# ShifuML/shifu-tensorflow

Measured on NVIDIA H100. Metric: rows/sec tabular-DNN train, higher is better.
Workload: dtype bf16

## Files before the change

include/shifu_b200.h:

```cpp
#ifndef SHIFU_B200_H
#define SHIFU_B200_H

#include <stdint.h>

#ifdef __cplusplus
extern "C" {
#endif

#define SB_MAX_HIDDEN 32

typedef enum {
  SB_OK = 0,
  SB_ERR_INVALID = -1,
  SB_ERR_CUDA = -2,
  SB_ERR_NCCL = -3,
  SB_ERR_IO = -4,
  SB_ERR_STATE = -5,
  SB_ERR_FORMAT = -6
} sb_status;

typedef enum { SB_ACT_SIGMOID = 0, SB_ACT_TANH = 1, SB_ACT_RELU = 2, SB_ACT_LEAKYRELU = 3, SB_ACT_NONE = -1 } sb_act;
typedef enum { SB_LOSS_MSE = 0, SB_LOSS_SIGMOID_CE = 1 } sb_loss;
typedef enum { SB_OPT_ADADELTA = 0, SB_OPT_ADAM = 1, SB_OPT_SGD = 2, SB_OPT_MOMENTUM = 3 } sb_optimizer;
typedef enum { SB_PREC_FP32 = 0, SB_PREC_BF16 = 1, SB_PREC_FP32_TC = 2, SB_PREC_BF16X2 = 3 } sb_precision;

typedef struct {
  int32_t n_features;
  int32_t n_hidden;
  int32_t hidden[SB_MAX_HIDDEN];
  int32_t acts[SB_MAX_HIDDEN];
  int32_t loss;
  int32_t optimizer;
  float learning_rate;
  float rho;
  float epsilon;
  float beta1, beta2;
  float momentum;
  int32_t max_batch;
  int32_t precision;
} sb_net_desc;

typedef struct sb_trainer sb_trainer_t;
typedef struct sb_model sb_model_t;

const char* sb_version(void);
const char* sb_last_error(void);
int sb_device_count(void);
int sb_host_alloc(void** ptr, uint64_t bytes);
int sb_host_free(void* ptr);

#define SB_NCCL_ID_BYTES 128
int sb_nccl_unique_id(void* out128);

int sb_trainer_create(const sb_net_desc* desc, int device, const void* nccl_id, int rank, int world,
                      sb_trainer_t** out);
int sb_trainer_destroy(sb_trainer_t* t);
#define SB_IPC_HANDLE_BYTES 64
int sb_trainer_ipc_handle(sb_trainer_t* t, void* out64);
int sb_trainer_set_peer_handles(sb_trainer_t* t, const void* handles , int32_t n_handles);
int sb_trainer_clear_peer_handles(sb_trainer_t* t);
void* sb_trainer_exchange_base(sb_trainer_t* t);
int sb_trainer_set_peer_pointers(sb_trainer_t* t, void* const* bases, int32_t n);
int64_t sb_trainer_param_count(const sb_trainer_t* t);
int sb_trainer_set_params(sb_trainer_t* t, const float* flat, int64_t n);
int sb_trainer_get_params(sb_trainer_t* t, float* flat, int64_t n);
int sb_trainer_init_xavier(sb_trainer_t* t, uint64_t seed);
int sb_trainer_get_grads(sb_trainer_t* t, float* flat, int64_t n);

int sb_trainer_step(sb_trainer_t* t, const float* X, const float* y, const float* w, int32_t rows,
                    float* loss_out);

int sb_trainer_set_sparse(sb_trainer_t* t, int32_t n_dense, int32_t n_onehot, int32_t n_cat);
int sb_trainer_step_sparse(sb_trainer_t* t, const float* Xd, const int32_t* idx, const float* y, const float* w,
                           int32_t rows, float* loss_out);
int sb_trainer_predict_sparse(sb_trainer_t* t, const float* Xd, const int32_t* idx, int64_t rows, float* out);
int sb_trainer_eval_loss_sparse(sb_trainer_t* t, const float* Xd, const int32_t* idx, const float* y, const float* w,
                                int64_t rows, float* loss_out);

int sb_trainer_step_async(sb_trainer_t* t, const float* X, const float* y, const float* w, int32_t rows);

int sb_trainer_accumulate(sb_trainer_t* t, const float* X, const float* y, const float* w, int32_t rows,
                          float* loss_out);
int sb_trainer_apply_accumulated(sb_trainer_t* t);
int sb_trainer_apply_accumulated_mean(sb_trainer_t* t, int64_t total_pushes);

int sb_trainer_load_dataset(sb_trainer_t* t, const float* X, const float* y, const float* w, int64_t n_rows);
int sb_trainer_step_resident(sb_trainer_t* t, int64_t row_offset, int32_t rows, float* loss_out);
int sb_trainer_step_resident_async(sb_trainer_t* t, int64_t row_offset, int32_t rows);
int sb_trainer_run_resident(sb_trainer_t* t, const int64_t* row_offsets, int32_t n_steps, int32_t rows);
int sb_trainer_accumulate_resident(sb_trainer_t* t, int64_t row_offset, int32_t rows, float* loss_out);
int sb_trainer_loss_resident(sb_trainer_t* t, int64_t row_offset, int32_t rows, float* loss_out);
int sb_trainer_last_loss(sb_trainer_t* t, float* loss_out);
int sb_trainer_loss_history(sb_trainer_t* t, int64_t first_step, int32_t n, float* out);
int sb_trainer_sync(sb_trainer_t* t);
int sb_trainer_broadcast_state(sb_trainer_t* t, int32_t root);
void* sb_trainer_stream(sb_trainer_t* t);
int sb_trainer_kernels_per_step(sb_trainer_t* t, int32_t rows);

int sb_trainer_eval_loss(sb_trainer_t* t, const float* X, const float* y, const float* w, int64_t rows,
                         float* loss_out);
int sb_trainer_predict(sb_trainer_t* t, const float* X, int64_t rows, float* out);

int sb_trainer_save_checkpoint(sb_trainer_t* t, const char* path);
int sb_trainer_load_checkpoint(sb_trainer_t* t, const char* path);
int64_t sb_trainer_global_step(const sb_trainer_t* t);

int sb_trainer_export_savedmodel(sb_trainer_t* t, const char* export_dir);

int sb_model_load(const char* saved_model_dir, const char* input_name, const char* output_name,
                  const char* tag, int device, int precision, sb_model_t** out);
int sb_model_create(const sb_net_desc* desc, const float* flat_params, int64_t n, int device, sb_model_t** out);
int sb_model_destroy(sb_model_t* m);
int32_t sb_model_n_features(const sb_model_t* m);
int32_t sb_model_n_layers(const sb_model_t* m);
int sb_model_score(sb_model_t* m, const float* X, int64_t rows, float* out);
int sb_model_score_row_f64(sb_model_t* m, const double* row, int32_t n, double* out);
int sb_model_score_device(sb_model_t* m, const float* dX, int64_t rows, float* dOut);
int sb_model_sync(sb_model_t* m);
void* sb_model_stream(sb_model_t* m);

#define SB_COL_SKIP (-1)
#define SB_COL_TARGET (-2)
#define SB_COL_WEIGHT (-3)
typedef struct { int64_t row; int32_t slot; int32_t len; int64_t offset; } sb_cell_flag;
int sb_text_parse(const char* text, int64_t n_bytes, char delim, const int32_t* col_map, int32_t n_map, int32_t n_feat,
                  float* X, float* y, float* w, int64_t max_rows, int64_t* n_rows_out, sb_cell_flag* flags,
                  int64_t flag_cap, int64_t* n_flags_out, int device);
int sb_text_parse_device(const char* text, int64_t n_bytes, char delim, const int32_t* col_map, int32_t n_map, int32_t n_feat,
                         float** dX, float** dy, float** dw, int64_t* n_rows_out, sb_cell_flag* flags, int64_t flag_cap,
                         int64_t* n_flags_out, int device, float* kernel_ms_out);
int sb_device_alloc_f32(float** out, int64_t n, int device);
int sb_device_free(void* p);
int sb_device_patch_f32(float* d_base, int64_t index, float value);
int sb_device_read_f32(const float* d_src, int64_t n, float* host_out);
int sb_device_gather_rows(const float* d_src, int32_t n_cols, const int64_t* rows_host, int64_t n, float* d_dst, int device);

int sb_debug_text_parse_host(const char* text, int64_t n_bytes, char delim, const int32_t* col_map, int32_t n_map,
                             int32_t n_feat, float* X, float* y, float* w, int64_t max_rows, int64_t* n_rows_out,
                             sb_cell_flag* flags, int64_t flag_cap, int64_t* n_flags_out);

int sb_savedmodel_write(const char* export_dir, const sb_net_desc* desc, const float* flat_params, int64_t n);
int sb_savedmodel_read(const char* saved_model_dir, const char* input_name, const char* output_name,
                       const char* tag, sb_net_desc* desc_out, int32_t* out_act, float* flat, int64_t flat_cap,
                       int64_t* n_params);

int sb_debug_gemm_bf16_cfg(const float* A, const float* B, float* D, int32_t M, int32_t N, int32_t K,
                           int32_t split_k, int32_t a_mn, int32_t b_mn, int32_t cfg_cg, int32_t cfg_bn, int device);

int sb_debug_gemm_layer(int32_t kind, int32_t precision, const float* A, const float* W, const float* bias, const float* aux,
                        const float* addend, float* out, float* colsum, float* grad, int32_t* guard, char* route,
                        int32_t route_cap, int32_t M, int32_t N, int32_t K, int32_t a_rows, int32_t row0, int32_t act,
                        int32_t r0, int32_t r1, int32_t sms, int64_t clear_n4, int device);

int sb_debug_step_trace(sb_trainer_t* t, uint64_t* stamps, int32_t cap_kernels, char* names, int32_t names_cap, int32_t* n_kernels);
int sb_debug_gemm_bench(const float* A, const float* B, float* D, int32_t M, int32_t N, int32_t K, int32_t split_k,
                        int32_t a_mn, int32_t b_mn, int32_t cfg_cg, int32_t cfg_bn, int device, int32_t iters,
                        float* ms_out);

int sb_debug_gemm_epilogue(const float* A, const float* W, const float* bias, const float* aux, float* out, float* colsum,
                           int32_t M, int32_t N, int32_t K, int32_t da, int32_t act, int32_t bm_wg, int device,
                           int32_t iters, float* ms_out);

int sb_debug_gemm_fwd_out(const float* A, const float* W, const float* bias, const float* wo, float bo, const float* y,
                          const float* w, float* dZ, float* g_bL, float* g_wo, float* g_bo, float* loss_sum, int32_t* guard,
                          int32_t M, int32_t N, int32_t K, int32_t a_rows, int32_t row0, int32_t act, int32_t loss,
                          int32_t np, int32_t grid, int device);

#ifdef __cplusplus
}
#endif
#endif
```

shifu-tensorflow_b200/_capi.py:

```python
from __future__ import annotations

import ctypes as C
import os
from typing import Optional, Sequence

import numpy as np

os.environ.setdefault("CUDA_DEVICE_MAX_CONNECTIONS", "32")

_HERE = os.path.dirname(os.path.abspath(__file__))
LIB_PATH = os.path.join(_HERE, "lib", "libshifu_b200.so")

SB_MAX_HIDDEN = 32
SB_NCCL_ID_BYTES = 128
ACT_SIGMOID, ACT_TANH, ACT_RELU, ACT_LEAKYRELU, ACT_NONE = 0, 1, 2, 3, -1
LOSS_MSE, LOSS_SIGMOID_CE = 0, 1
OPT_ADADELTA, OPT_ADAM, OPT_SGD, OPT_MOMENTUM = 0, 1, 2, 3
PREC_FP32, PREC_BF16, PREC_FP32_TC, PREC_BF16X2 = 0, 1, 2, 3
SB_OK, SB_ERR_INVALID, SB_ERR_CUDA, SB_ERR_NCCL, SB_ERR_IO, SB_ERR_STATE, SB_ERR_FORMAT = 0, -1, -2, -3, -4, -5, -6


class NetDesc(C.Structure):
    _fields_ = [
        ("n_features", C.c_int32), ("n_hidden", C.c_int32),
        ("hidden", C.c_int32 * SB_MAX_HIDDEN), ("acts", C.c_int32 * SB_MAX_HIDDEN),
        ("loss", C.c_int32), ("optimizer", C.c_int32),
        ("learning_rate", C.c_float), ("rho", C.c_float), ("epsilon", C.c_float),
        ("beta1", C.c_float), ("beta2", C.c_float), ("momentum", C.c_float),
        ("max_batch", C.c_int32), ("precision", C.c_int32),
    ]


def make_desc(n_features: int, hidden: Sequence[int], acts: Sequence[int], loss: int = LOSS_MSE,
              optimizer: int = OPT_ADADELTA, learning_rate: float = 0.001, rho: float = 0.95, epsilon: float = 1e-8,
              beta1: float = 0.9, beta2: float = 0.999, momentum: float = 0.9, max_batch: int = 128,
              precision: int = PREC_FP32) -> NetDesc:
    if len(hidden) != len(acts):
        raise ValueError("hidden and acts must have the same length")
    if len(hidden) > SB_MAX_HIDDEN:
        raise ValueError("at most %d hidden layers" % SB_MAX_HIDDEN)
    d = NetDesc()
    d.n_features, d.n_hidden = int(n_features), len(hidden)
    for i, (h, a) in enumerate(zip(hidden, acts)):
        d.hidden[i], d.acts[i] = int(h), int(a)
    d.loss, d.optimizer = int(loss), int(optimizer)
    d.learning_rate, d.rho, d.epsilon = learning_rate, rho, epsilon
    d.beta1, d.beta2, d.momentum = beta1, beta2, momentum
    d.max_batch, d.precision = int(max_batch), int(precision)
    return d


class CellFlag(C.Structure):
    _fields_ = [("row", C.c_int64), ("slot", C.c_int32), ("len", C.c_int32), ("offset", C.c_int64)]


COL_SKIP, COL_TARGET, COL_WEIGHT = -1, -2, -3


class ShifuB200Error(RuntimeError):
    def __init__(self, code: int, msg: str):
        super().__init__("[%d] %s" % (code, msg))
        self.code = code


_lib = None

_P = C.POINTER
_f32p, _f64p, _vp, _cp = _P(C.c_float), _P(C.c_double), C.c_void_p, C.c_char_p
PROTOTYPES = {
    "sb_version": (C.c_char_p, []),
    "sb_last_error": (C.c_char_p, []),
    "sb_device_count": (C.c_int, []),
    "sb_host_alloc": (C.c_int, [_P(_vp), C.c_uint64]),
    "sb_host_free": (C.c_int, [_vp]),
    "sb_nccl_unique_id": (C.c_int, [_vp]),
    "sb_trainer_create": (C.c_int, [_P(NetDesc), C.c_int, _vp, C.c_int, C.c_int, _P(_vp)]),
    "sb_trainer_destroy": (C.c_int, [_vp]),
    "sb_trainer_ipc_handle": (C.c_int, [_vp, _vp]),
    "sb_trainer_set_peer_handles": (C.c_int, [_vp, _vp, C.c_int32]),
    "sb_trainer_clear_peer_handles": (C.c_int, [_vp]),
    "sb_trainer_exchange_base": (C.c_void_p, [_vp]),
    "sb_trainer_set_peer_pointers": (C.c_int, [_vp, _P(_vp), C.c_int32]),
    "sb_trainer_param_count": (C.c_int64, [_vp]),
    "sb_trainer_set_params": (C.c_int, [_vp, _f32p, C.c_int64]),
    "sb_trainer_get_params": (C.c_int, [_vp, _f32p, C.c_int64]),
    "sb_trainer_init_xavier": (C.c_int, [_vp, C.c_uint64]),
    "sb_trainer_get_grads": (C.c_int, [_vp, _f32p, C.c_int64]),
    "sb_trainer_step": (C.c_int, [_vp, _f32p, _f32p, _f32p, C.c_int32, _f32p]),
    "sb_trainer_set_sparse": (C.c_int, [_vp, C.c_int32, C.c_int32, C.c_int32]),
    "sb_trainer_step_sparse": (C.c_int, [_vp, _f32p, _P(C.c_int32), _f32p, _f32p, C.c_int32, _f32p]),
    "sb_trainer_predict_sparse": (C.c_int, [_vp, _f32p, _P(C.c_int32), C.c_int64, _f32p]),
    "sb_trainer_eval_loss_sparse": (C.c_int, [_vp, _f32p, _P(C.c_int32), _f32p, _f32p, C.c_int64, _f32p]),
    "sb_trainer_step_async": (C.c_int, [_vp, _f32p, _f32p, _f32p, C.c_int32]),
    "sb_trainer_accumulate": (C.c_int, [_vp, _f32p, _f32p, _f32p, C.c_int32, _f32p]),
    "sb_trainer_apply_accumulated": (C.c_int, [_vp]),
    "sb_trainer_apply_accumulated_mean": (C.c_int, [_vp, C.c_int64]),
    "sb_trainer_loss_resident": (C.c_int, [_vp, C.c_int64, C.c_int32, _f32p]),
    "sb_trainer_broadcast_state": (C.c_int, [_vp, C.c_int32]),
    "sb_trainer_load_dataset": (C.c_int, [_vp, _f32p, _f32p, _f32p, C.c_int64]),
    "sb_trainer_step_resident": (C.c_int, [_vp, C.c_int64, C.c_int32, _f32p]),
    "sb_trainer_step_resident_async": (C.c_int, [_vp, C.c_int64, C.c_int32]),
    "sb_trainer_run_resident": (C.c_int, [_vp, C.POINTER(C.c_int64), C.c_int32, C.c_int32]),
    "sb_trainer_accumulate_resident": (C.c_int, [_vp, C.c_int64, C.c_int32, _f32p]),
    "sb_trainer_last_loss": (C.c_int, [_vp, _f32p]),
    "sb_trainer_loss_history": (C.c_int, [_vp, C.c_int64, C.c_int32, _f32p]),
    "sb_trainer_sync": (C.c_int, [_vp]),
    "sb_trainer_stream": (C.c_void_p, [_vp]),
    "sb_trainer_kernels_per_step": (C.c_int, [_vp, C.c_int32]),
    "sb_trainer_eval_loss": (C.c_int, [_vp, _f32p, _f32p, _f32p, C.c_int64, _f32p]),
    "sb_trainer_predict": (C.c_int, [_vp, _f32p, C.c_int64, _f32p]),
    "sb_trainer_save_checkpoint": (C.c_int, [_vp, _cp]),
    "sb_trainer_load_checkpoint": (C.c_int, [_vp, _cp]),
    "sb_trainer_global_step": (C.c_int64, [_vp]),
    "sb_trainer_export_savedmodel": (C.c_int, [_vp, _cp]),
    "sb_model_load": (C.c_int, [_cp, _cp, _cp, _cp, C.c_int, C.c_int, _P(_vp)]),
    "sb_model_create": (C.c_int, [_P(NetDesc), _f32p, C.c_int64, C.c_int, _P(_vp)]),
    "sb_model_destroy": (C.c_int, [_vp]),
    "sb_model_n_features": (C.c_int32, [_vp]),
    "sb_model_n_layers": (C.c_int32, [_vp]),
    "sb_model_score": (C.c_int, [_vp, _f32p, C.c_int64, _f32p]),
    "sb_model_score_row_f64": (C.c_int, [_vp, _f64p, C.c_int32, _f64p]),
    "sb_model_score_device": (C.c_int, [_vp, _vp, C.c_int64, _vp]),
    "sb_model_sync": (C.c_int, [_vp]),
    "sb_model_stream": (C.c_void_p, [_vp]),
    "sb_text_parse": (C.c_int, [_cp, C.c_int64, C.c_char, _P(C.c_int32), C.c_int32, C.c_int32, _f32p, _f32p, _f32p, C.c_int64,
                                _P(C.c_int64), _P(CellFlag), C.c_int64, _P(C.c_int64), C.c_int]),
    "sb_text_parse_device": (C.c_int, [_cp, C.c_int64, C.c_char, _P(C.c_int32), C.c_int32, C.c_int32, _P(_f32p), _P(_f32p), _P(_f32p),
                                       _P(C.c_int64), _P(CellFlag), C.c_int64, _P(C.c_int64), C.c_int, _f32p]),
    "sb_device_alloc_f32": (C.c_int, [_P(_f32p), C.c_int64, C.c_int]),
    "sb_device_free": (C.c_int, [_vp]),
    "sb_device_patch_f32": (C.c_int, [_f32p, C.c_int64, C.c_float]),
    "sb_device_read_f32": (C.c_int, [_f32p, C.c_int64, _f32p]),
    "sb_device_gather_rows": (C.c_int, [_f32p, C.c_int32, _P(C.c_int64), C.c_int64, _f32p, C.c_int]),
    "sb_debug_text_parse_host": (C.c_int, [_cp, C.c_int64, C.c_char, _P(C.c_int32), C.c_int32, C.c_int32, _f32p, _f32p, _f32p,
                                           C.c_int64, _P(C.c_int64), _P(CellFlag), C.c_int64, _P(C.c_int64)]),
    "sb_savedmodel_write": (C.c_int, [_cp, _P(NetDesc), _f32p, C.c_int64]),
    "sb_savedmodel_read": (C.c_int, [_cp, _cp, _cp, _cp, _P(NetDesc), _P(C.c_int32), _f32p, C.c_int64, _P(C.c_int64)]),
    "sb_debug_gemm_layer": (C.c_int, [C.c_int32, C.c_int32, _f32p, _f32p, _f32p, _f32p, _f32p, _f32p, _f32p, _f32p, _P(C.c_int32),
                                      C.c_char_p, C.c_int32, C.c_int32, C.c_int32, C.c_int32, C.c_int32, C.c_int32, C.c_int32,
                                      C.c_int32, C.c_int32, C.c_int32, C.c_int64, C.c_int]),
    "sb_debug_step_trace": (C.c_int, [_vp, C.POINTER(C.c_uint64), C.c_int32, C.c_char_p, C.c_int32, C.POINTER(C.c_int32)]),
    "sb_debug_gemm_bench": (C.c_int, [_f32p, _f32p, _f32p, C.c_int32, C.c_int32, C.c_int32, C.c_int32, C.c_int32, C.c_int32,
                                      C.c_int32, C.c_int32, C.c_int, C.c_int32, _f32p]),
    "sb_debug_gemm_bf16_cfg": (C.c_int, [_f32p, _f32p, _f32p, C.c_int32, C.c_int32, C.c_int32, C.c_int32, C.c_int32, C.c_int32,
                                         C.c_int32, C.c_int32, C.c_int]),
    "sb_debug_gemm_epilogue": (C.c_int, [_f32p, _f32p, _f32p, _f32p, _f32p, _f32p, C.c_int32, C.c_int32, C.c_int32, C.c_int32,
                                         C.c_int32, C.c_int32, C.c_int, C.c_int32, _f32p]),
    "sb_debug_gemm_fwd_out": (C.c_int, [_f32p, _f32p, _f32p, _f32p, C.c_float, _f32p, _f32p, _f32p, _f32p, _f32p, _f32p, _f32p,
                                        _P(C.c_int32), C.c_int32, C.c_int32, C.c_int32, C.c_int32, C.c_int32, C.c_int32,
                                        C.c_int32, C.c_int32, C.c_int32, C.c_int]),
}


def lib():
    global _lib
    if _lib is not None:
        return _lib
    if not os.path.exists(LIB_PATH):
        raise ImportError(
            "libshifu_b200.so is missing (%s). Build it with `python -c 'import __graft_entry__ as g; g.build()'` "
            "or `python shifu-tensorflow_b200/build.py`. There is no CPU fallback." % LIB_PATH)
    L = C.CDLL(LIB_PATH, mode=C.RTLD_GLOBAL)
    for name, (res, args) in PROTOTYPES.items():
        fn = getattr(L, name)
        fn.restype, fn.argtypes = res, args
    _lib = L
    return L


def check(status: int) -> None:
    if status != SB_OK:
        raise ShifuB200Error(status, lib().sb_last_error().decode("utf-8", "replace"))


def _f32(a, shape=None) -> np.ndarray:
    a = np.ascontiguousarray(a, dtype=np.float32)
    if shape is not None and a.shape != shape:
        a = a.reshape(shape)
    return a


def _ptr(a):
    if a is None:
        return None
    if hasattr(a, "ptr") and not isinstance(a, np.ndarray):
        return a.ptr
    return a.ctypes.data_as(_f32p)


class DeviceArray:

    def __init__(self, ptr, shape, device: int = 0, owner: bool = True):
        self.ptr, self.shape, self.device, self._own = ptr, tuple(shape), device, owner

    @classmethod
    def empty(cls, shape, device: int = 0) -> "DeviceArray":
        p = _f32p()
        n = int(np.prod(shape))
        check(lib().sb_device_alloc_f32(C.byref(p), max(n, 1), device))
        return cls(p, shape, device)

    def __len__(self):
        return self.shape[0]

    @property
    def size(self) -> int:
        return int(np.prod(self.shape))

    def numpy(self) -> np.ndarray:
        out = np.empty(self.shape, np.float32)
        if self.size:
            check(lib().sb_device_read_f32(self.ptr, self.size, _ptr(out)))
        return out

    def patch(self, flat_index: int, value: float):
        check(lib().sb_device_patch_f32(self.ptr, int(flat_index), float(value)))

    def take_rows(self, rows) -> "DeviceArray":
        rows = np.ascontiguousarray(rows, dtype=np.int64)
        n_cols = int(np.prod(self.shape[1:])) if len(self.shape) > 1 else 1
        out = DeviceArray.empty((len(rows),) + self.shape[1:], self.device)
        check(lib().sb_device_gather_rows(self.ptr, n_cols, rows.ctypes.data_as(_P(C.c_int64)), len(rows), out.ptr, self.device))
        return out

    def free(self):
        if self._own and self.ptr:
            lib().sb_device_free(C.cast(self.ptr, _vp))
        self.ptr = None

    __del__ = free


class Trainer:

    def __init__(self, desc: NetDesc, device: int = 0, nccl_id: Optional[bytes] = None, rank: int = 0, world: int = 1):
        self._h = C.c_void_p()
        self.desc = desc
        idbuf = None
        if nccl_id is not None:
            if len(nccl_id) != SB_NCCL_ID_BYTES:
                raise ValueError("nccl_id must be %d bytes" % SB_NCCL_ID_BYTES)
            idbuf = C.create_string_buffer(bytes(nccl_id), SB_NCCL_ID_BYTES)
        check(lib().sb_trainer_create(C.byref(desc), device, C.cast(idbuf, _vp) if idbuf is not None else None,
                                      rank, world, C.byref(self._h)))
        self.n_params = int(lib().sb_trainer_param_count(self._h))
        self.n_features = int(desc.n_features)

    def close(self):
        if getattr(self, "_h", None) is not None and self._h:
            lib().sb_trainer_destroy(self._h)
            self._h = None

    __del__ = close

    def __enter__(self):
        return self

    def __exit__(self, *exc):
        self.close()

    def ipc_handle(self) -> bytes:
        buf = C.create_string_buffer(64)
        check(lib().sb_trainer_ipc_handle(self._h, C.cast(buf, _vp)))
        return buf.raw

    def set_peer_handles(self, handles: Sequence[bytes]):
        blob = b"".join(handles)
        buf = C.create_string_buffer(blob, len(blob))
        check(lib().sb_trainer_set_peer_handles(self._h, C.cast(buf, _vp), len(handles)))

    def clear_peer_handles(self):
        check(lib().sb_trainer_clear_peer_handles(self._h))

    @property
    def exchange_base(self) -> int:
        return int(lib().sb_trainer_exchange_base(self._h) or 0)

    def set_peer_pointers(self, bases: Sequence[int]):
        arr = (C.c_void_p * len(bases))(*[C.c_void_p(int(b)) for b in bases])
        check(lib().sb_trainer_set_peer_pointers(self._h, arr, len(bases)))

    def set_params(self, flat):
        flat = _f32(flat).reshape(-1)
        check(lib().sb_trainer_set_params(self._h, _ptr(flat), flat.size))

    def get_params(self) -> np.ndarray:
        out = np.empty(self.n_params, np.float32)
        check(lib().sb_trainer_get_params(self._h, _ptr(out), out.size))
        return out

    def get_grads(self) -> np.ndarray:
        out = np.empty(self.n_params, np.float32)
        check(lib().sb_trainer_get_grads(self._h, _ptr(out), out.size))
        return out

    def init_xavier(self, seed: int):
        check(lib().sb_trainer_init_xavier(self._h, seed))

    def _xyw(self, X, y, w):
        if isinstance(X, DeviceArray):
# ... 110 lines not shown
        return out

    def sync(self):
        check(lib().sb_trainer_sync(self._h))

    @property
    def stream(self) -> int:
        return int(lib().sb_trainer_stream(self._h) or 0)

    def kernels_per_step(self, rows: int) -> int:
        n = lib().sb_trainer_kernels_per_step(self._h, rows)
        if n < 0:
            check(n)
        return n

    def eval_loss(self, X, y, w=None) -> float:
        X, y, w, rows = self._xyw(X, y, w)
        loss = C.c_float()
        check(lib().sb_trainer_eval_loss(self._h, _ptr(X), _ptr(y), _ptr(w), rows, C.byref(loss)))
        return float(loss.value)

    def predict(self, X) -> np.ndarray:
        X = _f32(X)
        out = np.empty(X.shape[0], np.float32)
        check(lib().sb_trainer_predict(self._h, _ptr(X), X.shape[0], _ptr(out)))
        return out

    def debug_step_trace(self):
        buf = np.zeros((32, 16), np.uint64)
        names = C.create_string_buffer(4096)
        k = C.c_int32()
        check(lib().sb_debug_step_trace(self._h, buf.ctypes.data_as(C.POINTER(C.c_uint64)), 32, names, 4096, C.byref(k)))
        return names.value.decode().split(","), buf[:k.value].copy()

    @property
    def global_step(self) -> int:
        return int(lib().sb_trainer_global_step(self._h))

    def save_checkpoint(self, path: str):
        check(lib().sb_trainer_save_checkpoint(self._h, path.encode()))

    def load_checkpoint(self, path: str):
        check(lib().sb_trainer_load_checkpoint(self._h, path.encode()))

    def export_savedmodel(self, export_dir: str):
        check(lib().sb_trainer_export_savedmodel(self._h, export_dir.encode()))


class Model:

    def __init__(self, handle):
        self._h = handle
        self.n_features = int(lib().sb_model_n_features(self._h))

    @classmethod
    def load(cls, saved_model_dir: str, input_name: str, output_name: str, tag: str = "serve", device: int = 0,
             precision: int = PREC_FP32) -> "Model":
        h = C.c_void_p()
        enc = lambda s: None if s is None else s.encode()
        check(lib().sb_model_load(enc(saved_model_dir), enc(input_name), enc(output_name), enc(tag), device, precision,
                                  C.byref(h)))
        return cls(h)

    @classmethod
    def create(cls, desc: NetDesc, flat_params, device: int = 0) -> "Model":
        h = C.c_void_p()
        flat = _f32(flat_params).reshape(-1)
        check(lib().sb_model_create(C.byref(desc), _ptr(flat), flat.size, device, C.byref(h)))
        return cls(h)

    def close(self):
        if getattr(self, "_h", None) is not None and self._h:
            lib().sb_model_destroy(self._h)
            self._h = None

    __del__ = close

    def __enter__(self):
        return self

    def __exit__(self, *exc):
        self.close()

    def score(self, X) -> np.ndarray:
        X = _f32(X)
        if X.ndim != 2 or X.shape[1] != self.n_features:
            raise ValueError("X must be [rows, %d]" % self.n_features)
        out = np.empty(X.shape[0], np.float32)
        check(lib().sb_model_score(self._h, _ptr(X), X.shape[0], _ptr(out)))
        return out

    def score_row_f64(self, row) -> float:
        row = np.ascontiguousarray(row, dtype=np.float64).reshape(-1)
        out = C.c_double()
        check(lib().sb_model_score_row_f64(self._h, row.ctypes.data_as(_f64p), row.size, C.byref(out)))
        return float(out.value)

    def score_device(self, dX_ptr: int, rows: int, dOut_ptr: int):
        check(lib().sb_model_score_device(self._h, C.c_void_p(dX_ptr), rows, C.c_void_p(dOut_ptr)))

    def sync(self):
        check(lib().sb_model_sync(self._h))

    @property
    def stream(self) -> int:
        return int(lib().sb_model_stream(self._h) or 0)


def nccl_unique_id() -> bytes:
    buf = C.create_string_buffer(SB_NCCL_ID_BYTES)
    check(lib().sb_nccl_unique_id(C.cast(buf, _vp)))
    return buf.raw


def device_count() -> int:
    return int(lib().sb_device_count())


def savedmodel_write(export_dir: str, desc: NetDesc, flat_params) -> None:
    flat = _f32(flat_params).reshape(-1)
    check(lib().sb_savedmodel_write(export_dir.encode(), C.byref(desc), _ptr(flat), flat.size))


def savedmodel_read(saved_model_dir: str, input_name: str, output_name: str, tag: str = "serve"):
    d = NetDesc()
    out_act = C.c_int32(0)
    n = C.c_int64(0)
    args = (saved_model_dir.encode(), input_name.encode(), output_name.encode(), tag.encode())
    check(lib().sb_savedmodel_read(*args, C.byref(d), C.byref(out_act), None, 0, C.byref(n)))
    flat = np.empty(n.value, np.float32)
    check(lib().sb_savedmodel_read(*args, C.byref(d), C.byref(out_act), _ptr(flat), flat.size, C.byref(n)))
    return int(d.n_features), [int(d.hidden[i]) for i in range(d.n_hidden)], [int(d.acts[i]) for i in range(d.n_hidden)], \
        int(out_act.value), flat


def debug_gemm_bf16(A: np.ndarray, B: np.ndarray, split_k: int = 1, device: int = 0, a_mn: bool = False,
                    b_mn: bool = False, cg: int = 0, bn: int = 0) -> np.ndarray:
    A, B = _f32(A), _f32(B)
    (K, M) = A.shape if a_mn else A.shape[::-1]
    (K2, N) = B.shape if b_mn else B.shape[::-1]
    assert K == K2
    D = np.zeros((M, N), np.float32)
    check(lib().sb_debug_gemm_bf16_cfg(_ptr(A), _ptr(B), _ptr(D), M, N, K, split_k, int(a_mn), int(b_mn), cg, bn, device))
    return D


GEMM_FWD, GEMM_DA, GEMM_DW = 0, 1, 2
PARTS = {PREC_FP32: 1, PREC_BF16: 1, PREC_FP32_TC: 3, PREC_BF16X2: 2}


def debug_gemm_layer(kind: int, precision: int, A: np.ndarray, W: np.ndarray, act: int = ACT_NONE,
                     bias: Optional[np.ndarray] = None, aux: Optional[np.ndarray] = None, addend: Optional[np.ndarray] = None,
                     colsum: Optional[np.ndarray] = None, grad: Optional[np.ndarray] = None, M: Optional[int] = None,
                     row0: int = 0, r0: int = 0, r1: Optional[int] = None, sms: int = 0, clear_n4: int = 0, device: int = 0):
    A, W = _f32(A), _f32(W)
    nparts = PARTS[precision]
    out = cs = g = None
    if kind == GEMM_DW:
        a_rows, Mx = A.shape
        K, N = W.shape
        if row0 + K > a_rows:
            raise ValueError("the batch of K = %d rows at row0 = %d runs past A" % (K, row0))
        g = np.zeros((Mx, N), np.float32) if grad is None else _f32(grad).copy()
        a_rows_arg, M = a_rows, Mx
    elif kind == GEMM_DA:
        M, K = A.shape
        N = W.shape[0]
        assert W.shape == (N, K) and np.shape(aux) == (M, N)
        cs = np.zeros(N, np.float32) if colsum is None else _f32(colsum).copy()
        a_rows_arg = M
    else:
        a_rows_arg, K = A.shape
        N = W.shape[1]
        M = a_rows_arg - row0 if M is None else M
    if kind != GEMM_DW:
        out = np.zeros((nparts, M, N), np.float32)
    bias = None if bias is None else _f32(bias)
    aux = None if aux is None else _f32(aux)
    addend = None if addend is None else _f32(addend)
    guard = C.c_int32(-1)
    route = C.create_string_buffer(64)
    check(lib().sb_debug_gemm_layer(kind, precision, _ptr(A), _ptr(W), _ptr(bias), _ptr(aux), _ptr(addend), _ptr(out), _ptr(cs),
                                    _ptr(g), C.byref(guard), route, 64, M, N, K, a_rows_arg, row0, act, r0,
                                    M if r1 is None else r1, sms, clear_n4, device))
    return out, cs, g, int(guard.value), route.value.decode()


def debug_gemm_split(A: np.ndarray, B: np.ndarray, np_parts: int, device: int = 0) -> np.ndarray:
    prec = {1: PREC_BF16, 2: PREC_BF16X2, 3: PREC_FP32_TC}.get(np_parts)
    if prec is None:
        raise ShifuB200Error(SB_ERR_INVALID, "np_parts=%r outside 1..3" % (np_parts,))
    A, B = _f32(A), _f32(B)
    assert A.shape[1] == B.shape[1]
    out, _, _, guard, _ = debug_gemm_layer(GEMM_FWD, prec, A, B.T.copy(), ACT_NONE, bias=np.zeros(B.shape[0], np.float32),
                                           device=device)
    if guard != 0:
        raise ShifuB200Error(SB_ERR_STATE, "%d sentinel elements around the output changed" % guard)
    return out.astype(np.float64).sum(axis=0)


def debug_gemm_bench(M: int, N: int, K: int, split_k: int = 1, a_mn: bool = False, b_mn: bool = False, cg: int = 0,
                     bn: int = 0, iters: int = 50, device: int = 0) -> float:
    rng = np.random.default_rng(0)
    A = rng.standard_normal((K, M) if a_mn else (M, K), dtype=np.float32)
    B = rng.standard_normal((K, N) if b_mn else (N, K), dtype=np.float32)
    D = np.zeros((M, N), np.float32)
    ms = C.c_float()
    check(lib().sb_debug_gemm_bench(_ptr(A), _ptr(B), _ptr(D), M, N, K, split_k, int(a_mn), int(b_mn), cg, bn, device,
                                    iters, C.byref(ms)))
    return float(ms.value)


def debug_gemm_epilogue(A: np.ndarray, W: np.ndarray, act: int, bias: Optional[np.ndarray] = None,
                        aux: Optional[np.ndarray] = None, bm_wg: int = 0, iters: int = 0, device: int = 0):
    A, W = _f32(A), _f32(W)
    M, K = A.shape
    da = aux is not None
    N = W.shape[0] if da else W.shape[1]
    assert W.shape == ((N, K) if da else (K, N))
    bias = _f32(bias) if bias is not None else None
    aux = _f32(aux) if da else None
    out = np.zeros((M, N), np.float32)
    cs = np.zeros(N, np.float32) if da else None
    ms = C.c_float()
    check(lib().sb_debug_gemm_epilogue(_ptr(A), _ptr(W), _ptr(bias) if bias is not None else None,
                                       _ptr(aux) if da else None, _ptr(out), _ptr(cs) if da else None, M, N, K, int(da),
                                       act, bm_wg, device, iters, C.byref(ms)))
    return out, cs, (float(ms.value) if iters > 0 else None)


def debug_gemm_fwd_out(A: np.ndarray, W: np.ndarray, bias: np.ndarray, wo: np.ndarray, bo: float, y: np.ndarray,
                       w: np.ndarray, act: int, loss: int, np_parts: int = 1, row0: int = 0, M: Optional[int] = None,
                       grid: int = 0, g_bL: Optional[np.ndarray] = None, g_wo: Optional[np.ndarray] = None, g_bo: float = 0.0,
                       loss_sum: float = 0.0, device: int = 0):
    A, W, bias, wo = _f32(A), _f32(W), _f32(bias), _f32(wo)
    a_rows, K = A.shape
    K2, N = W.shape
    assert K == K2
    M = a_rows - row0 if M is None else M
    y, w = _f32(y).reshape(-1), _f32(w).reshape(-1)
    assert y.size == M and w.size == M
    g_bL = _f32(g_bL).copy() if g_bL is not None else np.zeros(N, np.float32)
    g_wo = _f32(g_wo).copy() if g_wo is not None else np.zeros(N, np.float32)
    gbo, ls, guard = C.c_float(g_bo), C.c_float(loss_sum), C.c_int32(-1)
    dZ = np.zeros((max(np_parts, 1), max(M, 0), N), np.float32)
    check(lib().sb_debug_gemm_fwd_out(_ptr(A), _ptr(W), _ptr(bias), _ptr(wo), float(bo), _ptr(y), _ptr(w), _ptr(dZ),
                                      _ptr(g_bL), _ptr(g_wo), C.byref(gbo), C.byref(ls), C.byref(guard), M, N, K, a_rows, row0,
                                      act, loss, np_parts, grid, device))
    return dZ, g_bL, g_wo, float(gbo.value), float(ls.value), int(guard.value)


def text_parse_device(text: bytes, col_map: Sequence[int], n_feat: int, delim: str = "|", device: int = 0, flag_cap: int = 65536):
    if not text.endswith(b"\n"):
        text = text + b"\n"
    cm = (C.c_int32 * len(col_map))(*[int(c) for c in col_map])
    dX, dy, dw = _f32p(), _f32p(), _f32p()
    flags = (CellFlag * flag_cap)()
    n_rows, n_flags, kms = C.c_int64(0), C.c_int64(0), C.c_float(0)
    check(lib().sb_text_parse_device(text, len(text), delim.encode()[:1], cm, len(col_map), n_feat, C.byref(dX), C.byref(dy), C.byref(dw),
                                     C.byref(n_rows), flags, flag_cap, C.byref(n_flags), device, C.byref(kms)))
    if n_flags.value > flag_cap:
        raise ShifuB200Error(SB_ERR_FORMAT, "%d cells need the slow path, more than flag_cap=%d" % (n_flags.value, flag_cap))
    fl = [(int(flags[i].row), int(flags[i].slot), int(flags[i].offset), int(flags[i].len)) for i in range(n_flags.value)]
    n = n_rows.value
    return DeviceArray(dX, (n, n_feat), device), DeviceArray(dy, (n,), device), DeviceArray(dw, (n,), device), fl, text, float(kms.value)


def text_parse(text: bytes, col_map: Sequence[int], n_feat: int, delim: str = "|", device: int = 0, host_debug: bool = False,
               flag_cap: int = 65536):
    if not text.endswith(b"\n"):
        text = text + b"\n"
    max_rows = text.count(b"\n")
    cm = (C.c_int32 * len(col_map))(*[int(c) for c in col_map])
    X = np.zeros((max_rows, n_feat), np.float32)
    y = np.zeros(max_rows, np.float32)
    w = np.ones(max_rows, np.float32)
    flags = (CellFlag * flag_cap)()
    n_rows, n_flags = C.c_int64(0), C.c_int64(0)
    args = [text, len(text), delim.encode()[:1], cm, len(col_map), n_feat, _ptr(X), _ptr(y), _ptr(w), max_rows, C.byref(n_rows),
            flags, flag_cap, C.byref(n_flags)]
    if host_debug:
        check(lib().sb_debug_text_parse_host(*args))
    else:
        check(lib().sb_text_parse(*args, device))
    if n_flags.value > flag_cap:
        raise ShifuB200Error(SB_ERR_FORMAT, "%d cells need the slow path, more than flag_cap=%d" % (n_flags.value, flag_cap))
    fl = [(int(flags[i].row), int(flags[i].slot), int(flags[i].offset), int(flags[i].len)) for i in range(n_flags.value)]
    n = n_rows.value
    return X[:n], y[:n], w[:n], fl, text
```

shifu-tensorflow_b200/csrc/capi.cu:

```cuda
#include <math.h>
#include <stdlib.h>
#include <string.h>
#include <algorithm>
#include <memory>
#include <random>
#include "net.cuh"
#include "savedmodel.h"
#include "xchg_p2p.cuh"

using namespace sb;

enum { G_STEP = 0, G_ACC = 1, G_KINDS = 2 };

struct sb_trainer {
  Net net;
  sb_net_desc desc;
  OptHyper hyper;
  float lr = 0.f;
  int rank = 0, world = 1;
  NcclComm comm = nullptr;
  float *grad = nullptr, *s1 = nullptr, *s2 = nullptr, *acc = nullptr;
  int n_acc = 0;
  float grad_out_scale = 1.f;
  long long global_step = 0;
// ... 114 lines not shown
}

static int enqueue_allreduce(sb_trainer* t, float* buf) {
  if (t->world <= 1) return SB_OK;
  NcclApi* api = nccl_api();
  SB_CHECK(api && t->comm, SB_ERR_NCCL, "no gradient exchange configured: world = %d but neither an NCCL communicator (nccl_id) nor a "
           "peer table (sb_trainer_set_peer_handles / _pointers) exists", t->world);
  int r = api->AllReduce(buf, buf, static_cast<size_t>(t->net.n_params), NCCL_FLOAT32, NCCL_SUM, t->comm, t->net.stream);
  SB_CHECK(r == 0, SB_ERR_NCCL, "ncclAllReduce failed: %s", api->GetErrorString(r));
  return SB_OK;
}

static int enqueue_optimizer(sb_trainer* t, const StepIn& in, const float* g, int w0 = 0, int w1 = -1, cudaStream_t st = nullptr,
                             bool publish_scalars = false, bool pdl = false) {
  Net& n = t->net;
  if (w1 < 0) w1 = n.n_work;
  if (!st) st = n.stream;
  if (w1 <= w0) return SB_OK;
  SB_TRY(launch_kernel(optimizer_kernel, dim3(static_cast<unsigned>(w1 - w0)), dim3(256), 0, st, pdl, n.work + w0, in.desc, t->hyper,
                       n.theta, g, n.s1, n.s2, in.scal, publish_scalars ? t->d_hscal : static_cast<float*>(nullptr),
                       n.next_trace(st == n.stream ? "opt" : "opt_side")));
  n.mark("optimizer");
  return SB_OK;
}

enum { XSEG_A = 1 };
static int xseg_all(const sb_trainer* t) { return (1 << t->x_slots) - 1; }

static XchgParams xchg_params(sb_trainer* t, const BatchDesc* desc) {
  Net& n = t->net;
  XchgParams p;
  memset(&p, 0, sizeof(p));
  p.peers = t->d_peers;
  p.rank = t->rank; p.world = t->world;
  p.s1_off = static_cast<long long>(n.s1_off); p.s2_off = static_cast<long long>(n.s2_off);
  p.grad_off = t->grad_off; p.flags_off = t->flags_off;
  p.work = n.work;
  p.n_slots = t->x_slots;
  for (int sl = 0; sl < t->x_slots; ++sl) { p.slot_begin[sl] = t->x_begin[sl]; p.slot_end[sl] = t->x_end[sl]; }
  p.desc = desc;
  p.hyper = t->hyper;
  p.host_err = t->d_herr;
  p.timeout_ns = t->xchg_timeout_ns;
  static const bool fence_sys = getenv("SB_XCHG_FENCE_SYS") != nullptr;
  p.fence_gpu = fence_sys ? 0 : 1;
  return p;
}

static int enqueue_xchg(sb_trainer* t, const StepIn& in, int slot_mask, cudaStream_t st, bool publish_scalars, bool pdl,
                        bool alone = false) {
  Net& n = t->net;
  XchgParams p = xchg_params(t, in.desc);
  p.slot_mask = slot_mask;
  p.scal = publish_scalars ? in.scal : nullptr;
  p.host_scal = publish_scalars ? t->d_hscal : nullptr;
  char nm[24];
  if (slot_mask == XSEG_A) snprintf(nm, sizeof(nm), "xchg_A");
  else if ((slot_mask & (slot_mask - 1)) == 0) snprintf(nm, sizeof(nm), "xchg_B%d", __builtin_ctz(slot_mask) - 1);
  else snprintf(nm, sizeof(nm), "xchg");
  p.trace = n.next_trace(nm);
  int runs = 0, all_runs = 0;
  for (int sl = 0; sl < t->x_slots; ++sl)
    if ((slot_mask >> sl) & 1) {
      runs += (p.slot_end[sl] - p.slot_begin[sl] + t->world - 1) / t->world;
      all_runs += p.slot_end[sl] - p.slot_begin[sl];
    }
  const int U = t->world <= 2 ? 2 : 1;
  const int want = std::max((runs + U - 1) / U, (all_runs - runs + 3) / 4);
  int grid = t->xchg_blocks > 0 ? t->xchg_blocks : (alone ? 2 : 1) * n.num_sms;
  if (t->peers_share_device && grid > 32) grid = 32;
  if (grid > want) grid = want;
  if (grid < 1) grid = 1;
  const dim3 g(static_cast<unsigned>(grid)), b(256);
  if (t->ll_ready) {
    LLParams lp;
    lp.x = p; lp.llg_off = t->llg_off; lp.lls_off = t->lls_off; lp.n4 = t->xch_n4;
    if (t->world <= 2) SB_TRY(launch_kernel(xchg_ll_kernel<2>, g, b, 0, st, pdl, lp));
    else if (t->world <= 4) SB_TRY(launch_kernel(xchg_ll_kernel<4>, g, b, 0, st, pdl, lp));
    else if (t->world <= 8) SB_TRY(launch_kernel(xchg_ll_kernel<8>, g, b, 0, st, pdl, lp));
    else SB_TRY(launch_kernel(xchg_ll_kernel<16>, g, b, 0, st, pdl, lp));
  } else
  if (t->world <= 2) SB_TRY(launch_kernel(xchg_update_kernel<2>, g, b, 0, st, pdl, p));
  else if (t->world <= 4) SB_TRY(launch_kernel(xchg_update_kernel<4>, g, b, 0, st, pdl, p));
  else if (t->world <= 8) SB_TRY(launch_kernel(xchg_update_kernel<8>, g, b, 0, st, pdl, p));
  else SB_TRY(launch_kernel(xchg_update_kernel<16>, g, b, 0, st, pdl, p));
  n.mark("xchg_update");
  t->master_stale = true;
  t->grad_sharded = true;
  return SB_OK;
}

static int gather_master(sb_trainer* t) {
  if (!t->p2p_ready || !t->master_stale || t->world <= 1) return SB_OK;
  Net& n = t->net;
  SB_CUDA(cudaStreamSynchronize(n.stream));
  XchgParams p = xchg_params(t, n.desc);
  gather_master_kernel<<<n.n_work, 256, 0, n.stream>>>(p, 0);
  SB_CUDA(cudaGetLastError());
  SB_CUDA(cudaStreamSynchronize(n.stream));
  t->master_stale = false;
  return SB_OK;
}

static int join_streams(cudaStream_t to, cudaStream_t from, cudaEvent_t e) {
  SB_CUDA(cudaEventRecord(e, from));
  SB_CUDA(cudaStreamWaitEvent(to, e, 0));
  return SB_OK;
}

enum Dw1At { DW1_BESIDE, DW1_FRONT, DW1_BEHIND };
struct Dw1Plan {
  Dw1At at;
  int sms[2];
};

static Dw1Plan plan_dw1(const sb_trainer* t, int rows, bool split_tail, bool xsched) {
  const Net& n = t->net;
  const int S = n.num_sms;
  Dw1Plan d = {DW1_BESIDE, {S, S}};
  if (xsched) {
    d.at = t->peers_share_device ? DW1_BEHIND : DW1_FRONT;
    return d;
  }
  const Layer& l0 = n.layers[0];
  const Layer& l1 = n.layers[1];
  const int kx = round_up(rows, 64) * pairs_of(n.nparts);
  const GemmPlan n0 = plan_gemm(l0.in, l0.out, kx, S, true);
  const GemmPlan n1 = plan_gemm(l1.in, l1.out, kx, S, true);
  if (n0.grid + n1.grid <= S) return d;
  if (split_tail && (n0.grid == S || n0.bn == 256)) {
    d.at = DW1_FRONT;
    return d;
  }
  const GemmPlan b1 = plan_gemm(l1.in, l1.out, kx, S / 3, true);
  const GemmPlan b0 = plan_gemm(l0.in, l0.out, kx, S - b1.grid, true);
  auto waves = [&](const GemmPlan& pl, const Layer& ly, int sms) {
    const int tiles = ((ly.in + 127) / 128) * ((ly.out + pl.bn - 1) / pl.bn) * pl.split_k;
    return ((tiles + sms - 1) / sms) * pl.kb_per_split;
  };
  const int t_nat = waves(n0, l0, S) + waves(n1, l1, S);
  const int t0 = waves(b0, l0, S - b1.grid);
  const int t1 = waves(b1, l1, S / 3);
  if ((t0 > t1 ? t0 : t1) < t_nat) { d.sms[1] = S / 3; d.sms[0] = S - b1.grid; }
  return d;
}

static int enqueue_step_backward(sb_trainer* t, const StepIn& in, int rows, int kind) {
  Net& n = t->net;
  float* g = t->grad;
  const int L = n.L, S = n.num_sms;
  if (!n.tc()) {
    for (int l = L - 1; l >= 0; --l) {
      SB_TRY(n.enqueue_dw(in, l, rows, g, n.stream, false, S));
      if (l > 0) SB_TRY(n.enqueue_da(l, rows, g));
    }
  } else {
    const bool split_tail = kind == G_STEP && (t->world == 1 || t->p2p_ready) && L > 1;
    const bool xsched = split_tail && t->world > 1;
    const Dw1Plan d1 = L > 1 ? plan_dw1(t, rows, split_tail, xsched) : Dw1Plan{DW1_BESIDE, {S, S}};
    for (int l = L - 1; l >= 1; --l) {
      if (l > 1 || d1.at == DW1_BESIDE) {
        SB_TRY(join_streams(t->side, n.stream, t->ev_dz[l]));
        SB_TRY(n.enqueue_dw(in, l, rows, g, t->side, false, l == 1 ? d1.sms[1] : S));
      }
      SB_TRY(n.enqueue_da(l, rows, g));
    }
    if (split_tail) SB_CUDA(cudaEventRecord(t->ev_da_done, n.stream));
    if (L == 1) {
      SB_TRY(join_streams(t->side, n.stream, t->ev_dz[0]));
      SB_TRY(n.enqueue_dw(in, 0, rows, g, t->side, false, S));
    } else {
      if (d1.at == DW1_FRONT) {
        SB_TRY(n.enqueue_dw(in, 1, rows, g, n.stream, true, d1.sms[1]));
        SB_TRY(join_streams(t->side, n.stream, t->ev_c[0]));
        if (xsched) {
          SB_TRY(enqueue_xchg(t, in, XSEG_A, t->side, false, false));
          SB_CUDA(cudaEventRecord(t->ev_x[0], t->side));
        }
      }
      if (xsched && !in.sparse) {
        for (int c = 0; c < t->x_chunks; ++c) {
          const int r0 = c * t->x_chunk_rows, r1 = std::min(r0 + t->x_chunk_rows, n.layers[0].in);
          SB_TRY(n.enqueue_dw(in, 0, rows, g, n.stream, true, d1.sms[0], r0, r1, t->x_chunks > 1 ? c : -1));
          cudaStream_t cs = t->xstream[c & 1];
          SB_TRY(join_streams(cs, n.stream, t->ev_c[1 + c]));
          const bool last = c == t->x_chunks - 1;
          SB_TRY(enqueue_xchg(t, in, 1 << (1 + c), cs, last, false, last && d1.at != DW1_BEHIND));
          SB_CUDA(cudaEventRecord(t->ev_x[1 + c], cs));
        }
      } else {
        SB_TRY(n.enqueue_dw(in, 0, rows, g, n.stream, true, d1.sms[0]));
      }
      if (d1.at == DW1_BEHIND) {
        SB_TRY(n.enqueue_dw(in, 1, rows, g, n.stream, true, d1.sms[1]));
        SB_TRY(join_streams(t->side, n.stream, t->ev_c[0]));
        SB_TRY(enqueue_xchg(t, in, XSEG_A, t->side, false, false));
        SB_CUDA(cudaEventRecord(t->ev_x[0], t->side));
      }
    }
    if (xsched) {
      if (in.sparse) SB_TRY(enqueue_xchg(t, in, xseg_all(t) & ~XSEG_A, n.stream, true, false));
      else
        for (int c = 0; c < t->x_chunks; ++c) SB_CUDA(cudaStreamWaitEvent(n.stream, t->ev_x[1 + c], 0));
      SB_CUDA(cudaStreamWaitEvent(n.stream, t->ev_x[0], 0));
      return SB_OK;
    }
    if (split_tail) {
      SB_TRY(enqueue_optimizer(t, in, g, n.work_begin[0], n.work_end[0], n.stream, true, true));
      SB_CUDA(cudaStreamWaitEvent(t->side, t->ev_da_done, 0));
      SB_TRY(enqueue_optimizer(t, in, g, n.work_end[0], n.n_work, t->side));
      return join_streams(n.stream, t->side, t->ev_join);
    }
    SB_TRY(join_streams(n.stream, t->side, t->ev_join));
  }
  if (kind == G_STEP) {
    if (t->world > 1 && t->p2p_ready) {
      SB_TRY(enqueue_xchg(t, in, xseg_all(t), n.stream, true, false));
    } else {
      SB_TRY(enqueue_allreduce(t, g));
      SB_TRY(enqueue_optimizer(t, in, g, 0, -1, nullptr, true, false));
    }
  } else {
    const long long np = n.n_params;
    axpy_kernel<<<static_cast<unsigned>((np + 255) / 256), 256, 0, n.stream>>>(t->acc, g, np, in.scal, t->d_hscal);
    SB_CUDA(cudaGetLastError());
    n.mark("accumulate");
  }
  return SB_OK;
}

static int enqueue_step_body(sb_trainer* t, const StepIn& in, int rows, int kind) {
  Net& n = t->net;
  n.trace_k = 0;
  float4* clear = nullptr;
  long long clear_n4 = 0;
  if (in.resident) {
    if (n.L > 1) {
      clear = reinterpret_cast<float4*>(t->grad);
      clear_n4 = t->xch_n4;
    } else {
      SB_CUDA(cudaMemsetAsync(t->grad, 0, sizeof(float) * n.n_params, n.stream));
    }
  } else {
    SB_TRY(n.enqueue_load(in, rows, t->grad, n.n_params));
  }
  bool fused_out = false;
  SB_TRY(n.enqueue_hidden_forward(in, rows, t->grad, &fused_out, clear, clear_n4));
  if (!fused_out) SB_TRY(n.enqueue_out(in, rows, true, true, nullptr, t->grad));
  return enqueue_step_backward(t, in, rows, kind);
}

static int get_graph(sb_trainer* t, const StepIn& in, int rows, int kind, int pair, cudaGraphExec_t* out) {
  auto key = std::make_pair(rows, kind * 8 + (in.sparse ? 4 : 0) + (in.resident ? 2 : 0) + pair);
  auto it = t->graphs.find(key);
  if (it != t->graphs.end()) { *out = it->second; return SB_OK; }
  Net& n = t->net;
  n.launches = 0;
  cudaGraph_t g = nullptr;
  SB_CUDA(cudaStreamBeginCapture(n.stream, cudaStreamCaptureModeThreadLocal));
  int s = enqueue_step_body(t, in, rows, kind);
  cudaError_t e = cudaStreamEndCapture(n.stream, &g);
  if (s != SB_OK) { if (g) cudaGraphDestroy(g); return s; }
  SB_CHECK(e == cudaSuccess, SB_ERR_CUDA, "cudaStreamEndCapture failed: %s", cudaGetErrorString(e));
  cudaGraphExec_t ge = nullptr;
  SB_CUDA(cudaGraphInstantiate(&ge, g, 0));
  cudaGraphDestroy(g);
  t->graphs[key] = ge;
  if (kind == G_STEP && !in.sparse && (in.resident || !t->dsXb)) t->kernels_per_step[rows] = n.launches + 1;
  *out = ge;
  return SB_OK;
}

static int run_step(sb_trainer* t, const float* X, const float* y, const float* w, int rows, int kind, long long resident_row0 = -1,
                    bool sparse = false) {
  Net& n = t->net;
  SB_CHECK(rows > 0 && rows <= n.max_batch, SB_ERR_INVALID, "rows=%d outside (0, max_batch=%d]", rows, n.max_batch);
  SB_CUDA(cudaSetDevice(n.device));
  const bool resident = resident_row0 >= 0 && t->dsXb != nullptr;
  const bool prep = resident && t->prep != nullptr;
  const int pair = prep ? static_cast<int>(t->prep_steps & 1) : 0;
  const StepIn in{t->descs[pair], t->scals[pair], resident, sparse};
  t->last_pair = pair;
  cudaGraphExec_t ge = nullptr;
  SB_TRY(get_graph(t, in, rows, kind, pair, &ge));
  float lr_t = t->lr, gscale = 1.f / static_cast<float>(t->world);
  if (kind == G_STEP) {
    ++t->global_step;
    lr_t = lr_for_step(t, t->global_step);
  }
  if (kind == G_STEP) ++t->epoch;
  if (prep) {
    if (!t->have_pos) SB_CUDA(cudaEventRecord(t->ev_pos[pair ^ 1], n.stream));
    SB_CUDA(cudaStreamWaitEvent(t->prep, t->ev_pos[pair ^ 1], 0));
    set_batch_kernel<<<1, 1, 0, t->prep>>>(in.desc, nullptr, y, w, lr_t, gscale, t->epoch, static_cast<int>(resident_row0), t->dsP, rows, in.scal,
                                           kind == G_STEP ? t->hist_slot(t->global_step) : nullptr);
    SB_CUDA(cudaGetLastError());
    SB_CUDA(cudaEventRecord(t->ev_prep[pair], t->prep));
    SB_CUDA(cudaEventRecord(t->ev_pos[pair], n.stream));
    SB_CUDA(cudaStreamWaitEvent(n.stream, t->ev_prep[pair], 0));
    t->have_pos = true;
    ++t->prep_steps;
  } else {
    t->have_pos = false;
    if (resident)
      set_batch_kernel<<<1, 1, 0, n.stream>>>(in.desc, nullptr, y, w, lr_t, gscale, t->epoch, static_cast<int>(resident_row0), t->dsP, rows, in.scal,
                                               kind == G_STEP ? t->hist_slot(t->global_step) : nullptr);
    else
      set_batch_kernel<<<1, 1, 0, n.stream>>>(in.desc, X, y, w ? w : n.ones, lr_t, gscale, t->epoch, 0, nullptr, 0, nullptr,
                                               kind == G_STEP ? t->hist_slot(t->global_step) : nullptr);
  }
  SB_CUDA(cudaGetLastError());
  SB_CUDA(cudaGraphLaunch(ge, n.stream));
  if (kind == G_ACC) ++t->n_acc;
  t->grad_out_scale = (kind == G_STEP) ? gscale : 1.f;
  return SB_OK;
}

static int poll_nccl(sb_trainer* t) {
// ... 968 lines not shown
```

shifu-tensorflow_b200/csrc/common.cuh:

```cuda
#pragma once
#include <cuda_runtime.h>
#include <cuda_bf16.h>
#include <stdint.h>
#include <stdio.h>
#include <string>
#include <type_traits>
#include <utility>

#include "../../include/shifu_b200.h"

namespace sb {

std::string& last_error_ref();
int set_error(int code, const char* fmt, ...);

#define SB_CUDA(call)                                                                                       \
  do {                                                                                                      \
    cudaError_t _e = (call);                                                                                \
    if (_e != cudaSuccess)                                                                                  \
      return ::sb::set_error(SB_ERR_CUDA, "%s failed: %s (%s:%d)", #call, cudaGetErrorString(_e), __FILE__, \
                             __LINE__);                                                                     \
  } while (0)

#define SB_CHECK(cond, code, ...)                          \
  do {                                                     \
    if (!(cond)) return ::sb::set_error(code, __VA_ARGS__); \
  } while (0)

#define SB_TRY(expr)          \
  do {                        \
    int _s = (expr);          \
    if (_s != SB_OK) return _s; \
  } while (0)

template <typename T>
struct DevBuf {
  T* p = nullptr;
  DevBuf() = default;
  DevBuf(const DevBuf&) = delete;
  DevBuf& operator=(const DevBuf&) = delete;
  DevBuf(DevBuf&& o) noexcept : p(o.p) { o.p = nullptr; }
  DevBuf& operator=(DevBuf&& o) noexcept { std::swap(p, o.p); return *this; }
  ~DevBuf() { if (p) cudaFree(p); }
  int alloc(size_t n) {
    SB_CHECK(p == nullptr, SB_ERR_STATE, "DevBuf allocated twice");
    void* q = nullptr;
    SB_CUDA(cudaMalloc(&q, n * sizeof(T)));
    p = static_cast<T*>(q);
    return SB_OK;
  }
};

inline int round_up(int x, int m) { return (x + m - 1) / m * m; }
inline int64_t ceil_div64(int64_t a, int64_t b) { return (a + b - 1) / b; }

template <typename... KArgs, typename... Args>
int launch_kernel(void (*kernel)(KArgs...), dim3 grid, dim3 block, size_t smem, cudaStream_t st, bool pdl, Args... args) {
  cudaLaunchConfig_t cfg = {};
  cfg.gridDim = grid; cfg.blockDim = block; cfg.dynamicSmemBytes = smem; cfg.stream = st;
  cudaLaunchAttribute at[1];
  at[0].id = cudaLaunchAttributeProgrammaticStreamSerialization;
  at[0].val.programmaticStreamSerializationAllowed = 1;
  cfg.attrs = at; cfg.numAttrs = pdl ? 1 : 0;
  SB_CUDA(cudaLaunchKernelEx(&cfg, kernel, static_cast<KArgs>(args)...));
  return SB_OK;
}

template <typename... KArgs>
int set_max_smem(void (*kernel)(KArgs...), int bytes) {
  SB_CUDA(cudaFuncSetAttribute(kernel, cudaFuncAttributeMaxDynamicSharedMemorySize, bytes));
  return SB_OK;
}

template <typename F>
int with_act(int act, F&& f) {
  switch (act) {
    case SB_ACT_SIGMOID: return f(std::integral_constant<int, SB_ACT_SIGMOID>());
    case SB_ACT_TANH: return f(std::integral_constant<int, SB_ACT_TANH>());
    case SB_ACT_RELU: return f(std::integral_constant<int, SB_ACT_RELU>());
    case SB_ACT_LEAKYRELU: return f(std::integral_constant<int, SB_ACT_LEAKYRELU>());
    default: return f(std::integral_constant<int, SB_ACT_NONE>());
  }
}

#define SB_LEAKY_ALPHA 0.2f

__device__ __forceinline__ float sigmoidf_stable(float z) {
  if (z >= 0.f) return 1.f / (1.f + expf(-z));
  float e = expf(z);
  return e / (1.f + e);
}

__device__ __forceinline__ float act_apply(float z, int act) {
  switch (act) {
    case SB_ACT_SIGMOID: return sigmoidf_stable(z);
    case SB_ACT_TANH: return tanhf(z);
    case SB_ACT_RELU: return fmaxf(z, 0.f);
    case SB_ACT_LEAKYRELU: return z > 0.f ? z : z * SB_LEAKY_ALPHA;
    default: return z;
  }
}
__device__ __forceinline__ float act_grad_from_out(float a, int act) {
  switch (act) {
    case SB_ACT_SIGMOID: return a * (1.f - a);
    case SB_ACT_TANH: return 1.f - a * a;
    case SB_ACT_RELU: return a > 0.f ? 1.f : 0.f;
    case SB_ACT_LEAKYRELU: return a > 0.f ? 1.f : SB_LEAKY_ALPHA;
    default: return 1.f;
  }
}

__device__ __forceinline__ float warp_sum(float v) {
#pragma unroll
  for (int o = 16; o > 0; o >>= 1) v += __shfl_xor_sync(0xffffffffu, v, o);
  return v;
}

__device__ __forceinline__ float warp_colsum_32x32(float (&v)[32], int lane) {
#pragma unroll
  for (int half = 16; half >= 1; half >>= 1) {
    const bool upper = (lane & half) != 0;
#pragma unroll
    for (int i = 0; i < half; ++i) {
      float send = upper ? v[i] : v[i + half];
      float keep = upper ? v[i + half] : v[i];
      v[i] = keep + __shfl_xor_sync(0xffffffffu, send, half);
    }
  }
  return v[0];
}

template <int LEN, int N_>
__device__ __forceinline__ void colsum_halve(float (&v)[N_], int lane, int m) {
  const bool upper = (lane & m) != 0;
#pragma unroll
  for (int i = 0; i < LEN; ++i) {
    const float send = upper ? v[i] : v[i + LEN];
    const float keep = upper ? v[i + LEN] : v[i];
    v[i] = keep + __shfl_xor_sync(0xffffffffu, send, m);
  }
}
template <int N_>
__device__ __forceinline__ void colsum_row_groups(float (&v)[N_], int lane) {
  static_assert(N_ % 8 == 0, "three halving rounds");
  colsum_halve<N_ / 2>(v, lane, 16);
  colsum_halve<N_ / 4>(v, lane, 8);
  colsum_halve<N_ / 8>(v, lane, 4);
}

}
```

shifu-tensorflow_b200/csrc/gemm_pp.cuh:

```cuda
#pragma once
#include "gemm_tc.cuh"

namespace sb {

struct PpTmaps {
  CUtensorMap a;
  CUtensorMap b;
  CUtensorMap o;
  CUtensorMap x;
};

template <int BM_WG, int BN>
struct GemmPpCfg : RingCfg<BM_WG * 64 * 2, BN * 64 * 2, 1024 + 256 + 2 * BN * 4 + 16 * BN * 4 + 2 * BM_WG * BN * 2> {
  static_assert(BM_WG == 64 || BM_WG == 128, "warpgroup tile rows");
  static_assert(BN == 64 || BN == 128, "tile N");
  static_assert(GemmPpCfg::STAGES >= 4, "operand ring");
  static constexpr int X_TILE = BM_WG * 128;
  static constexpr int X_BYTES = X_TILE * (BN / 64);
};

template <int BM_WG, int BN, int EPI, int ACT>
__global__ void __launch_bounds__(GemmPpCfg<BM_WG, BN>::THREADS, 1)
gemm_pp_kernel(const __grid_constant__ PpTmaps tms, const GemmTcParams p) {
  static_assert(EPI == EPI_FWD || EPI == EPI_DA, "forward or dA");
  using Cfg = GemmPpCfg<BM_WG, BN>;
  constexpr int BK = Cfg::BK, MI = BM_WG / 64;
  constexpr bool B_MN = EPI == EPI_FWD;

  extern __shared__ uint8_t smem_raw[];
  const Ring<Cfg> ring(smem_raw, 2 * Cfg::X_BYTES);
  const uint32_t xs_base = ring.end();
  const uint32_t sm_bias = ring.bars + 256u;
  const uint32_t sm_col = sm_bias + 2u * BN * 4u;
  auto aux_bar = [&](int g) { return ring.bar(g); };

  const int warp = threadIdx.x >> 5;
  const int lane = threadIdx.x & 31;
  const bool tracing = ring_enter(ring, 1, 2, &tms.a, &tms.b, p);

  const int tiles_m = (p.M + BM_WG - 1) / BM_WG;
  const int tiles_n = (p.N + BN - 1) / BN;
  const int n_tiles = tiles_m * tiles_n;
  const int kb_n = (p.K + BK - 1) / BK;

  if (warp >= Cfg::PRODUCER_WARP) {
    asm volatile("setmaxnreg.dec.sync.aligned.u32 %0;" ::"n"(Cfg::PRODUCER_REGS));
    if (warp == Cfg::PRODUCER_WARP && lane == 0) {
      RingPos<Cfg::STAGES> pos;
      const int a_row0 = (p.a_rows != nullptr) ? p.a_rows->row0 : 0;
      for (int t = blockIdx.x; t < n_tiles; t += gridDim.x) {
        const int m0 = (t / tiles_n) * BM_WG, n0 = (t % tiles_n) * BN;
        for (int kb = 0; kb < kb_n; ++kb) {
          ring_issue(ring, pos, [&](uint32_t fb, uint32_t sa, uint32_t sb) {
            tma_load_2d(sa, &tms.a, fb, kb * BK, m0 + a_row0);
            if constexpr (B_MN) {
#pragma unroll
              for (int j = 0; j < BN / 64; ++j) tma_load_2d(sb + j * 8192, &tms.b, fb, n0 + j * 64, kb * BK);
            } else {
              tma_load_2d(sb, &tms.b, fb, kb * BK, n0);
            }
          });
          if (kb == 0 && t == static_cast<int>(blockIdx.x)) ring_stamp(p, tracing, 3);
        }
      }
    }
    ring_producer_tail<Cfg>(p);
  } else {
    asm volatile("setmaxnreg.inc.sync.aligned.u32 %0;" ::"n"(Cfg::CONSUMER_REGS));
    const int g = warp >> 2;
    const int gt = static_cast<int>(threadIdx.x) & 127;
    const bool xthread = gt == 0;
    auto bar_wg = [&]() { asm volatile("bar.sync %0, 128;" ::"r"(2 + g) : "memory"); };
    const uint32_t xs = xs_base + static_cast<uint32_t>(g) * Cfg::X_BYTES;
    const uint32_t bias_s = sm_bias + static_cast<uint32_t>(g) * BN * 4u;
    const uint32_t col_w = sm_col + static_cast<uint32_t>(g * 8 + (warp & 3)) * BN * 4u;
    const int r0 = (warp & 3) * 16 + (lane >> 2);
    const int c0 = 2 * (lane & 3);
    auto xaddr = [&](int r, int c) {
      return xs + static_cast<uint32_t>((c >> 6) * Cfg::X_TILE + r * 128 + ((((c & 63) >> 3) ^ (r & 7)) << 4) + (c & 7) * 2);
    };
    const bool do_cols = EPI == EPI_DA && p.colsum != nullptr;

    float acc[MI][BN / 2];
    for (int lt = g;; lt += 2) {
      const int t = static_cast<int>(blockIdx.x) + lt * static_cast<int>(gridDim.x);
      if (t >= n_tiles) break;
      const int it = lt >> 1;
      const int m0 = (t / tiles_n) * BM_WG, n0 = (t % tiles_n) * BN;
      const int nx = min(BN / 64, (p.N - n0 + 63) / 64);

      if (xthread) tma_store_wait_read<0>();
      if constexpr (EPI == EPI_FWD) {
        for (int j = gt; j < BN; j += 128) {
          const float bv = (n0 + j < p.N) ? __ldg(p.bias + n0 + j) : 0.f;
          asm volatile("st.shared.f32 [%0], %1;" ::"r"(bias_s + j * 4u), "f"(bv) : "memory");
        }
        bar_wg();
      } else {
        if (xthread) {
          mbar_arrive_expect_tx(aux_bar(g), static_cast<uint32_t>(nx * Cfg::X_TILE));
          for (int x = 0; x < nx; ++x) tma_load_2d(xs + x * Cfg::X_TILE, &tms.x, aux_bar(g), n0 + x * 64, m0);
        }
      }

      if (lt >= 1) asm volatile("bar.sync %0, 256;" ::"r"(4 + g) : "memory");
      RingPos<Cfg::STAGES> pos = RingPos<Cfg::STAGES>::at(lt * kb_n);
      ring_mma<BN, false, B_MN>(ring, pos, kb_n, acc, 0u, 0u, xthread, lt == 0, p, tracing, [&] {
        if (t + static_cast<int>(gridDim.x) < n_tiles) asm volatile("bar.arrive %0, 256;" ::"r"(4 + (g ^ 1)) : "memory");
      });

      if constexpr (EPI == EPI_FWD) {
#pragma unroll
        for (int i = 0; i < BN / 8; ++i) {
          const int c = c0 + 8 * i;
          float2 b;
          asm volatile("ld.shared.v2.f32 {%0, %1}, [%2];" : "=f"(b.x), "=f"(b.y) : "r"(bias_s + c * 4u) : "memory");
#pragma unroll
          for (int mi = 0; mi < MI; ++mi) {
#pragma unroll
            for (int h = 0; h < 2; ++h) {
              const float v0 = act_apply(acc[mi][4 * i + 2 * h] + b.x, ACT);
              const float v1 = act_apply(acc[mi][4 * i + 2 * h + 1] + b.y, ACT);
              asm volatile("st.shared.b32 [%0], %1;" ::"r"(xaddr(64 * mi + r0 + 8 * h, c)), "r"(pack_bf16x2(v0, v1)) : "memory");
            }
          }
        }
      } else {
        mbar_wait(aux_bar(g), static_cast<uint32_t>(it) & 1u);
        const uint32_t cb = col_w + static_cast<uint32_t>(it & 1) * 4u * BN * 4u;
#pragma unroll
        for (int x = 0; x < BN / 64; ++x) {
          float cs[16];
#pragma unroll
          for (int i = 0; i < 8; ++i) {
            const int c = 64 * x + c0 + 8 * i;
            float s0 = 0.f, s1 = 0.f;
#pragma unroll
            for (int mi = 0; mi < MI; ++mi) {
#pragma unroll
              for (int h = 0; h < 2; ++h) {
                const uint32_t a = xaddr(64 * mi + r0 + 8 * h, c);
                uint32_t raw;
                asm volatile("ld.shared.b32 %0, [%1];" : "=r"(raw) : "r"(a) : "memory");
                const float x0 = __uint_as_float(raw << 16), x1 = __uint_as_float(raw & 0xFFFF0000u);
                const float v0 = acc[mi][32 * x + 4 * i + 2 * h] * act_grad_from_out(x0, ACT);
                const float v1 = acc[mi][32 * x + 4 * i + 2 * h + 1] * act_grad_from_out(x1, ACT);
                asm volatile("st.shared.b32 [%0], %1;" ::"r"(a), "r"(pack_bf16x2(v0, v1)) : "memory");
                s0 += v0;
                s1 += v1;
              }
            }
            cs[2 * i] = s0;
            cs[2 * i + 1] = s1;
          }
          if (do_cols) {
            colsum_row_groups(cs, lane);
            const uint32_t col = static_cast<uint32_t>(64 * x + c0 + 8 * (lane >> 2));
            asm volatile("st.shared.v2.f32 [%0], {%1, %2};" ::"r"(cb + col * 4u), "f"(cs[0]), "f"(cs[1]) : "memory");
          }
        }
      }
      fence_proxy_async();
      bar_wg();
      if (xthread) {
        for (int x = 0; x < nx; ++x) tma_store_2d(&tms.o, xs + x * Cfg::X_TILE, n0 + x * 64, m0);
        tma_store_commit();
      }
      if (do_cols) {
        const uint32_t cb = col_w + static_cast<uint32_t>((it & 1) * 4 - (warp & 3)) * BN * 4u;
        for (int j = gt; j < BN; j += 128) {
          float v = 0.f;
#pragma unroll
          for (int w = 0; w < 4; ++w) {
            float x;
            asm volatile("ld.shared.f32 %0, [%1];" : "=f"(x) : "r"(cb + (w * BN + j) * 4u) : "memory");
            v += x;
          }
          if (n0 + j < p.N && v != 0.f) red_add_f32(p.colsum + n0 + j, v);
        }
      }
      if (lt == 0 && threadIdx.x == 0) ring_stamp(p, tracing, 7);
    }
    if (xthread) asm volatile("cp.async.bulk.wait_group 0;" ::: "memory");
  }
  ring_exit(p, tracing);
}

struct PpPlan {
  int bm_wg;
  int bn;
  int grid;
};

constexpr int PP_TILE_WIDE = 256;

static inline PpPlan plan_gemm_pp(int M, int N, int K, int num_sms, bool fwd, int tile = 0) {
  PpPlan pl = {};
  const int tiles_m = (M + 127) / 128, kb = (K + 63) / 64;
  const int wide_tiles = tiles_m * ((N + 255) / 256), narrow_tiles = tiles_m * ((N + 127) / 128);
  const bool wide = fwd && N > 128 && 8 * wide_tiles >= 7 * num_sms && kb >= 16 &&
                    2 * ((wide_tiles + num_sms - 1) / num_sms) <= (narrow_tiles + num_sms - 1) / num_sms;
  if (tile == PP_TILE_WIDE || (tile == 0 && wide)) {
    pl.bm_wg = 128;
    pl.bn = 256;
    pl.grid = wide_tiles < num_sms ? wide_tiles : num_sms;
    return pl;
  }
  pl.bn = N <= 64 ? 64 : 128;
  const int tiles_n = (N + pl.bn - 1) / pl.bn;
  const int tiles128 = tiles_m * tiles_n;
  const bool tall = tiles128 > num_sms || (8 * tiles128 >= 7 * num_sms && kb >= 8);
  pl.bm_wg = tile > 0 ? tile : (tall ? 128 : 64);
  const int tiles = ((M + pl.bm_wg - 1) / pl.bm_wg) * tiles_n;
  pl.grid = tiles < num_sms ? tiles : num_sms;
  return pl;
}

template <typename F>
static int with_pp_shape(int bm_wg, int bn, F&& f) {
  using std::integral_constant;
  if (bm_wg == 128 && bn == 128) return f(integral_constant<int, 128>(), integral_constant<int, 128>());
  if (bm_wg == 128 && bn == 64) return f(integral_constant<int, 128>(), integral_constant<int, 64>());
  if (bm_wg == 64 && bn == 128) return f(integral_constant<int, 64>(), integral_constant<int, 128>());
  if (bm_wg == 64 && bn == 64) return f(integral_constant<int, 64>(), integral_constant<int, 64>());
  return set_error(SB_ERR_INVALID, "no gemm_pp instantiation for bm_wg=%d bn=%d", bm_wg, bn);
}

template <int EPI>
static int launch_gemm_pp(const PpPlan& pl, const PpTmaps& tms, const GemmTcParams& p, cudaStream_t st, bool pdl) {
  return with_pp_shape(pl.bm_wg, pl.bn, [&](auto BM_WG, auto BN) {
    return with_act(p.act, [&](auto ACT) {
      using Cfg = GemmPpCfg<BM_WG, BN>;
      return launch_kernel(gemm_pp_kernel<BM_WG, BN, EPI, ACT>, pl.grid, Cfg::THREADS, Cfg::SMEM_BYTES, st, pdl, tms, p);
    });
  });
}

static int set_gemm_pp_attrs() {
  for (int bm_wg : {64, 128})
    for (int bn : {64, 128})
      for (int act = SB_ACT_NONE; act <= SB_ACT_LEAKYRELU; ++act)
        SB_TRY(with_pp_shape(bm_wg, bn, [&](auto BM_WG, auto BN) {
          return with_act(act, [&](auto ACT) {
            const int bytes = GemmPpCfg<BM_WG, BN>::SMEM_BYTES;
            SB_TRY(set_max_smem(gemm_pp_kernel<BM_WG, BN, EPI_FWD, ACT>, bytes));
            return set_max_smem(gemm_pp_kernel<BM_WG, BN, EPI_DA, ACT>, bytes);
          });
        }));
  return SB_OK;
}

}
```

shifu-tensorflow_b200/csrc/gemm_ring.cuh:

```cuda
#pragma once
#include <cuda.h>
#include "common.cuh"
#include "ptx.cuh"
#include "kernels.cuh"

namespace sb {

struct GemmTcParams {
  int M, N, K;
  int kb_per_split;
  int split_k;
  const float* bias;
  int act;
  __nv_bfloat16* out;
  int ld_out;
  const __nv_bfloat16* aux;
  int ld_aux;
  float* colsum;
  float* accum;
  int ld_acc;
  int acc_vec4;
  const float* wo;
  const float* bo;
  const BatchDesc* desc;
  float* scal;
  int loss;
  float *g_wo, *g_bo, *g_bL;
  const BatchDesc* a_rows;
  float4* zero_buf;
  long long zero_n4;
  unsigned long long* trace;
  int np;
  int n_pairs;
  unsigned char pair_a[6], pair_b[6];
  long long out_ps, aux_ps;
  const float* addend;
  int ld_add;
};

template <int A_BYTES_, int B_BYTES_, int FIXED_BYTES_>
struct RingCfg {
  static constexpr int BK = 64;
  static constexpr int THREADS = 384;
  static constexpr int PRODUCER_WARP = 8;
  static constexpr int CONSUMER_REGS = 232;
  static constexpr int PRODUCER_REGS = 40;
  static constexpr int A_BYTES = A_BYTES_, B_BYTES = B_BYTES_, FIXED_BYTES = FIXED_BYTES_;
  static constexpr int STAGE_BYTES = A_BYTES + B_BYTES;
  static constexpr int RING_BUDGET = 232448 - FIXED_BYTES;
  static constexpr int STAGES = RING_BUDGET / STAGE_BYTES > 8 ? 8 : RING_BUDGET / STAGE_BYTES;
  static constexpr int SMEM_BYTES = STAGES * STAGE_BYTES + FIXED_BYTES;
};

template <class Cfg>
struct Ring {
  uint32_t base, bars;
  __device__ __forceinline__ Ring(const uint8_t* smem, uint32_t bar_offset)
      : base((smem_u32(smem) + 1023u) & ~1023u), bars(base + Cfg::STAGES * Cfg::STAGE_BYTES + bar_offset) {}
  __device__ __forceinline__ uint32_t end() const { return base + Cfg::STAGES * Cfg::STAGE_BYTES; }
  __device__ __forceinline__ uint32_t a(int s) const { return base + s * Cfg::STAGE_BYTES; }
  __device__ __forceinline__ uint32_t b(int s) const { return a(s) + Cfg::A_BYTES; }
  __device__ __forceinline__ uint32_t full(int s) const { return bars + 8u * s; }
  __device__ __forceinline__ uint32_t empty(int s) const { return bars + 8u * (Cfg::STAGES + s); }
  __device__ __forceinline__ uint32_t bar(int i) const { return bars + 8u * (2 * Cfg::STAGES + i); }
};

template <int STAGES>
struct RingPos {
  int stage = 0;
  uint32_t phase = 0;
  __device__ __forceinline__ void advance() {
    if (++stage == STAGES) { stage = 0; phase ^= 1u; }
  }
  __device__ __forceinline__ static RingPos at(int n) {
    RingPos r;
    r.stage = n % STAGES;
    r.phase = static_cast<uint32_t>(n / STAGES) & 1u;
    return r;
  }
};

__device__ __forceinline__ void ring_stamp(const GemmTcParams& p, bool tracing, int slot) {
  if (tracing) p.trace[slot] = globaltimer_ns();
}

template <class Cfg>
__device__ __forceinline__ bool ring_enter(const Ring<Cfg>& ring, uint32_t empty_arrivals, int n_own_bars, const void* tm_a,
                                           const void* tm_b, const GemmTcParams& p) {
  const bool tracing = p.trace != nullptr && blockIdx.x == 0;
  if (threadIdx.x == 0) ring_stamp(p, tracing, 0);
  if (threadIdx.x == 0) {
    tma_prefetch_desc(tm_a);
    tma_prefetch_desc(tm_b);
    for (int s = 0; s < Cfg::STAGES; ++s) {
      mbar_init(ring.full(s), 1);
      mbar_init(ring.empty(s), empty_arrivals);
    }
    for (int i = 0; i < n_own_bars; ++i) mbar_init(ring.bar(i), 1);
    fence_barrier_init();
  }
  __syncthreads();
  if (threadIdx.x == 0) ring_stamp(p, tracing, 1);
  pdl_wait();
  pdl_launch_dependents();
  if (threadIdx.x == 0) ring_stamp(p, tracing, 2);
  return tracing;
}

__device__ __forceinline__ void ring_exit(const GemmTcParams& p, bool tracing) {
  __syncthreads();
  if (threadIdx.x == 0) {
    ring_stamp(p, tracing, 8);
    if (p.trace != nullptr) atomicMax(p.trace + 10, static_cast<unsigned long long>(globaltimer_ns()));
  }
}

template <class Cfg, class Boxes>
__device__ __forceinline__ void ring_issue(const Ring<Cfg>& ring, RingPos<Cfg::STAGES>& pos, Boxes&& boxes) {
  mbar_wait(ring.empty(pos.stage), pos.phase ^ 1u);
  const uint32_t fb = ring.full(pos.stage);
  mbar_arrive_expect_tx(fb, Cfg::STAGE_BYTES);
  boxes(fb, ring.a(pos.stage), ring.b(pos.stage));
  pos.advance();
}

template <class Cfg>
__device__ __forceinline__ void ring_producer_tail(const GemmTcParams& p) {
  if ((threadIdx.x >> 5) > Cfg::PRODUCER_WARP && p.zero_buf != nullptr) {
    const float4 z4 = make_float4(0.f, 0.f, 0.f, 0.f);
    const long long zt = static_cast<long long>(threadIdx.x) - 32 * (Cfg::PRODUCER_WARP + 1), zn = 32 * 3;
    for (long long i = static_cast<long long>(blockIdx.x) * zn + zt; i < p.zero_n4; i += static_cast<long long>(gridDim.x) * zn)
      p.zero_buf[i] = z4;
  }
  __syncwarp();
}

struct RingNoOp {
  __device__ __forceinline__ void operator()() const {}
};

template <int N, bool A_MN, bool B_MN, class Cfg, int MI, class Issued = RingNoOp>
__device__ __forceinline__ void ring_mma(const Ring<Cfg>& ring, RingPos<Cfg::STAGES>& pos, int n_kb, float (&acc)[MI][N / 2],
                                         uint32_t a_off, uint32_t b_off, bool releaser, bool first_tile,
                                         const GemmTcParams& p, bool tracing, Issued&& issued = Issued()) {
  constexpr uint32_t a_kstep = A_MN ? (2048u >> 4) : (32u >> 4);
  constexpr uint32_t b_kstep = B_MN ? (2048u >> 4) : (32u >> 4);
  int prev_stage = -1;
  for (int kb = 0; kb < n_kb; ++kb) {
    mbar_wait(ring.full(pos.stage), pos.phase);
    if (kb == 0 && first_tile && threadIdx.x == 0) ring_stamp(p, tracing, 4);
    const uint32_t sa = ring.a(pos.stage) + a_off, sb = ring.b(pos.stage) + b_off;
    const uint64_t da = A_MN ? make_mnmajor_sw128_desc(sa, 8192u) : make_kmajor_sw128_desc(sa);
    const uint64_t db = B_MN ? make_mnmajor_sw128_desc(sb, 8192u) : make_kmajor_sw128_desc(sb);
    wgmma_fence();
#pragma unroll
    for (int k = 0; k < Cfg::BK / 16; ++k) {
#pragma unroll
      for (int mi = 0; mi < MI; ++mi)
        wgmma_bf16<N, A_MN ? 1 : 0, B_MN ? 1 : 0>(acc[mi], da + (8192u >> 4) * mi + a_kstep * k, db + b_kstep * k,
                                                  (kb > 0 || k > 0) ? 1u : 0u);
    }
    wgmma_commit();
    wgmma_wait<1>();
    if (prev_stage >= 0 && releaser) mbar_arrive(ring.empty(prev_stage));
    prev_stage = pos.stage;
    pos.advance();
  }
  issued();
  wgmma_wait<0>();
  if (prev_stage >= 0 && releaser) mbar_arrive(ring.empty(prev_stage));
  if (first_tile && threadIdx.x == 0) { ring_stamp(p, tracing, 5); ring_stamp(p, tracing, 6); }
// ... 4 lines not shown
```

shifu-tensorflow_b200/csrc/gemm_wide.cuh:

```cuda
#pragma once
#include "gemm_pp.cuh"

namespace sb {

struct GemmWideCfg : RingCfg<128 * 64 * 2, 256 * 64 * 2, 1024 + 256 + 256 * 4 + 128 * 256 * 2> {
  static constexpr int BM = 128, BN = 256;
  static constexpr int X_TILE = BM * 128;
};
static_assert(GemmWideCfg::STAGES >= 3, "operand ring");

template <int ACT>
__global__ void __launch_bounds__(GemmWideCfg::THREADS, 1)
gemm_wide_kernel(const __grid_constant__ PpTmaps tms, const GemmTcParams p) {
  using Cfg = GemmWideCfg;
  constexpr int BM = Cfg::BM, BN = Cfg::BN, BK = Cfg::BK;

  extern __shared__ uint8_t smem_raw[];
  const Ring<Cfg> ring(smem_raw, Cfg::BN * Cfg::BM * 2);
  const uint32_t xs = ring.end();
  const uint32_t bias_s = ring.bars + 256u;

  const int warp = threadIdx.x >> 5;
  const int lane = threadIdx.x & 31;
  const bool tracing = ring_enter(ring, 2, 0, &tms.a, &tms.b, p);

  const int tiles_m = (p.M + BM - 1) / BM;
  const int tiles_n = (p.N + BN - 1) / BN;
  const int n_tiles = tiles_m * tiles_n;
  const int kb_n = (p.K + BK - 1) / BK;

  if (warp >= Cfg::PRODUCER_WARP) {
    asm volatile("setmaxnreg.dec.sync.aligned.u32 %0;" ::"n"(Cfg::PRODUCER_REGS));
    if (warp == Cfg::PRODUCER_WARP && lane == 0) {
      RingPos<Cfg::STAGES> pos;
      const int a_row0 = (p.a_rows != nullptr) ? p.a_rows->row0 : 0;
      for (int t = blockIdx.x; t < n_tiles; t += gridDim.x) {
        const int m0 = (t / tiles_n) * BM, n0 = (t % tiles_n) * BN;
        for (int kb = 0; kb < kb_n; ++kb) {
          ring_issue(ring, pos, [&](uint32_t fb, uint32_t sa, uint32_t sb) {
            tma_load_2d(sa, &tms.a, fb, kb * BK, m0 + a_row0);
#pragma unroll
            for (int j = 0; j < BN / 64; ++j) tma_load_2d(sb + j * 8192, &tms.b, fb, n0 + j * 64, kb * BK);
          });
          if (kb == 0 && t == static_cast<int>(blockIdx.x)) ring_stamp(p, tracing, 3);
        }
      }
    }
    ring_producer_tail<Cfg>(p);
  } else {
    asm volatile("setmaxnreg.inc.sync.aligned.u32 %0;" ::"n"(Cfg::CONSUMER_REGS));
    const int g = warp >> 2;
    const int ct = static_cast<int>(threadIdx.x);
    auto bar_consumers = [&]() { asm volatile("bar.sync 2, 256;" ::: "memory"); };
    const int r0 = 64 * g + (warp & 3) * 16 + (lane >> 2);
    const int c0 = 2 * (lane & 3);
    auto xaddr = [&](int r, int c) {
      return xs + static_cast<uint32_t>((c >> 6) * Cfg::X_TILE + r * 128 + ((((c & 63) >> 3) ^ (r & 7)) << 4) + (c & 7) * 2);
    };

    float acc_mi[1][BN / 2];
    float (&acc)[BN / 2] = acc_mi[0];
    RingPos<Cfg::STAGES> pos;
    for (int t = blockIdx.x; t < n_tiles; t += gridDim.x) {
      const bool first = t == static_cast<int>(blockIdx.x);
      const int m0 = (t / tiles_n) * BM, n0 = (t % tiles_n) * BN;
      const int nx = min(BN / 64, (p.N - n0 + 63) / 64);
      const float bv = (n0 + ct < p.N) ? __ldg(p.bias + n0 + ct) : 0.f;

      ring_mma<BN, false, true>(ring, pos, kb_n, acc_mi, static_cast<uint32_t>(g) * 8192u, 0u, (ct & 127) == 0, first, p,
                                tracing);

      asm volatile("st.shared.f32 [%0], %1;" ::"r"(bias_s + ct * 4u), "f"(bv) : "memory");
      if (ct == 0) tma_store_wait_read<0>();
      bar_consumers();
#pragma unroll
      for (int i = 0; i < BN / 8; ++i) {
        const int c = c0 + 8 * i;
        float2 b;
        asm volatile("ld.shared.v2.f32 {%0, %1}, [%2];" : "=f"(b.x), "=f"(b.y) : "r"(bias_s + c * 4u) : "memory");
#pragma unroll
        for (int h = 0; h < 2; ++h) {
          const float v0 = act_apply(acc[4 * i + 2 * h] + b.x, ACT);
          const float v1 = act_apply(acc[4 * i + 2 * h + 1] + b.y, ACT);
          asm volatile("st.shared.b32 [%0], %1;" ::"r"(xaddr(r0 + 8 * h, c)), "r"(pack_bf16x2(v0, v1)) : "memory");
        }
      }
      fence_proxy_async();
      bar_consumers();
      if (ct == 0) {
        for (int x = 0; x < nx; ++x) tma_store_2d(&tms.o, xs + x * Cfg::X_TILE, n0 + x * 64, m0);
        tma_store_commit();
      }
      if (first && ct == 0) ring_stamp(p, tracing, 7);
    }
    if (ct == 0) asm volatile("cp.async.bulk.wait_group 0;" ::: "memory");
  }
  ring_exit(p, tracing);
}

static int launch_gemm_wide(const PpPlan& pl, const PpTmaps& tms, const GemmTcParams& p, cudaStream_t st, bool pdl) {
  if (pl.bm_wg != GemmWideCfg::BM || pl.bn != GemmWideCfg::BN)
    return set_error(SB_ERR_INVALID, "gemm_wide has 128 x 256 tiles only (bm_wg=%d bn=%d)", pl.bm_wg, pl.bn);
  return with_act(p.act, [&](auto ACT) {
    return launch_kernel(gemm_wide_kernel<ACT>, pl.grid, GemmWideCfg::THREADS, GemmWideCfg::SMEM_BYTES, st, pdl, tms, p);
  });
}

static int set_gemm_wide_attrs() {
  for (int act = SB_ACT_NONE; act <= SB_ACT_LEAKYRELU; ++act)
    SB_TRY(with_act(act, [&](auto ACT) { return set_max_smem(gemm_wide_kernel<ACT>, GemmWideCfg::SMEM_BYTES); }));
  return SB_OK;
}

}
```

shifu-tensorflow_b200/csrc/net.cu:

```cuda
#include <stdarg.h>
#include <stdlib.h>
#include <string.h>
#include <algorithm>
#include "net.cuh"
#include "gemm_dw.cuh"
#include "gemm_fwd_out.cuh"
#include "gemm_pp.cuh"
#include "gemm_wide.cuh"

namespace sb {

std::string& last_error_ref() {
  thread_local std::string e;
  return e;
}
int set_error(int code, const char* fmt, ...) {
  char buf[1024];
  va_list ap;
  va_start(ap, fmt);
  vsnprintf(buf, sizeof(buf), fmt, ap);
  va_end(ap);
  last_error_ref() = buf;
  return code;
}
// ... 34 lines not shown
  cuuint32_t box[2] = {64u, static_cast<cuuint32_t>(box_rows)};
  cuuint32_t estr[2] = {1u, 1u};
  CUresult r = enc(out, CU_TENSOR_MAP_DATA_TYPE_BFLOAT16, 2, const_cast<void*>(base), gdim, gstr, box, estr,
                   CU_TENSOR_MAP_INTERLEAVE_NONE, CU_TENSOR_MAP_SWIZZLE_128B, CU_TENSOR_MAP_L2_PROMOTION_L2_256B,
                   CU_TENSOR_MAP_FLOAT_OOB_FILL_NONE);
  SB_CHECK(r == CUDA_SUCCESS, SB_ERR_CUDA, "cuTensorMapEncodeTiled failed (%d) rows=%d cols=%d ld=%d box_rows=%d",
           static_cast<int>(r), rows, cols, ld, box_rows);
  return SB_OK;
}

GemmPlan plan_gemm(int M, int N, int K, int num_sms, bool allow_split) {
  const int total_kb = (K + 63) / 64;
  auto tiles_of = [&](int bn) { return ((M + 127) / 128) * ((N + bn - 1) / bn); };
  auto plan = [&](int bn) {
    const int tiles = tiles_of(bn);
    int split = 1;
    if (allow_split) {
      split = num_sms / tiles;
      const int cap = total_kb / 8;
      if (split > cap) split = cap;
      if (split < 1) split = 1;
    }
    if (split > total_kb) split = total_kb;
    GemmPlan pl = {};
    pl.bn = bn;
    pl.kb_per_split = (total_kb + split - 1) / split;
    pl.split_k = (total_kb + pl.kb_per_split - 1) / pl.kb_per_split;
    const int work = tiles * pl.split_k;
    pl.grid = work < num_sms ? work : num_sms;
    return pl;
  };
  auto cost = [&](const GemmPlan& pl) {
    const long long work = static_cast<long long>(tiles_of(pl.bn)) * pl.split_k;
    return (work + pl.grid - 1) / pl.grid * pl.kb_per_split * pl.bn;
  };
  const GemmPlan pl = plan(N <= 64 ? 64 : 128);
  if (allow_split && N > 128) {
    const GemmPlan wide = plan(256);
    if (wide.grid == pl.grid && cost(wide) <= cost(pl) && wide.kb_per_split >= 32) return wide;
  }
  return pl;
}

int validate_desc(const sb_net_desc* d) {
  SB_CHECK(d != nullptr, SB_ERR_INVALID, "net desc is null");
  SB_CHECK(d->n_features > 0, SB_ERR_INVALID, "n_features must be > 0 (got %d)", d->n_features);
  SB_CHECK(d->n_hidden >= 1 && d->n_hidden <= SB_MAX_HIDDEN, SB_ERR_INVALID, "n_hidden must be in [1,%d] (got %d)",
           SB_MAX_HIDDEN, d->n_hidden);
  for (int l = 0; l < d->n_hidden; ++l) {
    SB_CHECK(d->hidden[l] > 0, SB_ERR_INVALID, "hidden[%d] must be > 0", l);
    SB_CHECK(d->acts[l] >= SB_ACT_NONE && d->acts[l] <= SB_ACT_LEAKYRELU, SB_ERR_INVALID, "acts[%d] invalid", l);
  }
  SB_CHECK(d->max_batch > 0, SB_ERR_INVALID, "max_batch must be > 0");
  SB_CHECK(d->precision >= SB_PREC_FP32 && d->precision <= SB_PREC_BF16X2, SB_ERR_INVALID, "precision invalid");
  SB_CHECK(d->loss == SB_LOSS_MSE || d->loss == SB_LOSS_SIGMOID_CE, SB_ERR_INVALID, "loss invalid");
  SB_CHECK(d->optimizer >= SB_OPT_ADADELTA && d->optimizer <= SB_OPT_MOMENTUM, SB_ERR_INVALID, "optimizer invalid");
  return SB_OK;
}

static int check_device(int device, int* num_sms) {
  int n = 0;
  cudaError_t e = cudaGetDeviceCount(&n);
  SB_CHECK(e == cudaSuccess && n > 0, SB_ERR_CUDA, "no CUDA device available (%s); this library has no CPU fallback",
           cudaGetErrorString(e));
  SB_CHECK(device >= 0 && device < n, SB_ERR_INVALID, "device %d out of range [0,%d)", device, n);
  cudaDeviceProp prop;
  SB_CUDA(cudaGetDeviceProperties(&prop, device));
  SB_CHECK(prop.major == 9 && prop.minor == 0, SB_ERR_CUDA, "device %d is sm_%d%d; this library is built for sm_90a only",
           device, prop.major, prop.minor);
  *num_sms = prop.multiProcessorCount;
  SB_CUDA(cudaSetDevice(device));
  return SB_OK;
}

int Net::init(const sb_net_desc* d, int device_, bool training_) {
  SB_TRY(validate_desc(d));
  SB_TRY(check_device(device_, &num_sms));
  device = device_;
  training = training_;
  const bool want_trace = getenv("SB_STEP_TRACE") != nullptr;
  int prio_least = 0, prio_greatest = 0;
  SB_CUDA(cudaDeviceGetStreamPriorityRange(&prio_least, &prio_greatest));
  SB_CUDA(cudaStreamCreateWithPriority(&stream, cudaStreamNonBlocking, prio_greatest));
  F = d->n_features;
  L = d->n_hidden;
  precision = d->precision;
  nparts = precision == SB_PREC_FP32_TC ? 3 : (precision == SB_PREC_BF16X2 ? 2 : 1);
  loss = d->loss;
  max_batch = d->max_batch;
  ldB = round_up(max_batch, 8);
  ldF = round_up(F, 8);
  layers.resize(L + 1);
  long long off = 0;
  int prev = F;
  for (int l = 0; l <= L; ++l) {
    Layer& ly = layers[l];
    ly.in = prev;
    ly.out = (l < L) ? d->hidden[l] : 1;
    ly.act = (l < L) ? d->acts[l] : SB_ACT_SIGMOID;
    ly.w_off = off; off += static_cast<long long>(ly.in) * ly.out;
    ly.b_off = off; off += ly.out;
    ly.ld_in = round_up(ly.in, 8);
    ly.ld_out = round_up(ly.out, 8);
    prev = ly.out;
  }
  n_params = off;
  const bool bf = tc();
  {
    auto align256 = [](size_t b) { return (b + 255) & ~static_cast<size_t>(255); };
    const size_t vec_bytes = align256(static_cast<size_t>(n_params) * sizeof(float) + 64);
    size_t at = vec_bytes;
    if (training) { s1_off = at; at += vec_bytes; s2_off = at; at += vec_bytes; }
    shadow_off = at;
    std::vector<size_t> wn_off(L, 0);
    Wn_ps.assign(L, 0);
    if (bf)
      for (int l = 0; l < L; ++l) {
        const size_t part = align256(static_cast<size_t>(layers[l].in) * layers[l].ld_out * sizeof(__nv_bfloat16));
        wn_off[l] = at; at += part * nparts;
        Wn_ps[l] = static_cast<long long>(part / sizeof(__nv_bfloat16));
      }
    extra_off = at;
    at += align256(arena_extra_bytes);
    arena_bytes = at;
    void* q = nullptr;
    SB_CUDA(cudaMalloc(&q, arena_bytes));
    allocs.push_back(q);
    SB_CUDA(cudaMemsetAsync(q, 0, arena_bytes, stream));
    arena = static_cast<char*>(q);
    theta = reinterpret_cast<float*>(arena);
    if (training) { s1 = reinterpret_cast<float*>(arena + s1_off); s2 = reinterpret_cast<float*>(arena + s2_off); }
    if (bf)
      for (int l = 0; l < L; ++l) layers[l].Wn = reinterpret_cast<__nv_bfloat16*>(arena + wn_off[l]);
  }
  SB_TRY(dalloc(&scal, SCAL_COUNT));
  SB_TRY(dalloc(&desc, 1));
  if (want_trace) SB_TRY(dalloc(&step_trace, 32 * 16));
  SB_TRY(dalloc(&yhat, max_batch));
  SB_TRY(dalloc(&ones, max_batch));
  SB_TRY(dalloc(&stX, static_cast<size_t>(max_batch) * F));
  SB_TRY(dalloc(&stY, max_batch));
  SB_TRY(dalloc(&stW, max_batch));
  fill_kernel<<<(max_batch + 255) / 256, 256, 0, stream>>>(ones, 1.f, max_batch);

  if (bf) {
    Xb_ps = static_cast<long long>(max_batch) * ldF;
    SB_TRY(dalloc(&Xb, static_cast<size_t>(Xb_ps) * nparts));
    A.assign(L, nullptr); dZ.assign(L, nullptr); A_ps.assign(L, 0);
    for (int l = 0; l < L; ++l) {
      Layer& ly = layers[l];
      A_ps[l] = static_cast<long long>(max_batch) * ly.ld_out;
      SB_TRY(dalloc(&A[l], static_cast<size_t>(A_ps[l]) * nparts));
      if (training) SB_TRY(dalloc(&dZ[l], static_cast<size_t>(A_ps[l]) * nparts));
    }
  } else {
    SB_TRY(dalloc(&Xf, static_cast<size_t>(max_batch) * F));
    Af.assign(L, nullptr); dZf.assign(L, nullptr);
    for (int l = 0; l < L; ++l) {
      SB_TRY(dalloc(&Af[l], static_cast<size_t>(max_batch) * layers[l].out));
      if (training) SB_TRY(dalloc(&dZf[l], static_cast<size_t>(max_batch) * layers[l].out));
    }
  }

  std::vector<OptWork> wk;
  auto add_runs = [&](long long o, long long n, const Layer* mat) {
    for (long long s = 0; s < n; s += 1024) {
      OptWork w = {};
      w.off = o + s; w.count = static_cast<int>(n - s < 1024 ? n - s : 1024);
      w.np = 1;
      if (mat) {
        w.out_dim = mat->out; w.mat_off = mat->w_off; w.Wn = mat->Wn; w.ld_out = mat->ld_out;
        w.np = nparts; w.part_stride = Wn_ps[static_cast<size_t>(mat - layers.data())];
      }
      wk.push_back(w);
    }
  };
  work_begin.assign(L + 1, 0); work_end.assign(L + 1, 0);
  for (int l = 0; l <= L; ++l) {
    Layer& ly = layers[l];
    work_begin[l] = static_cast<int>(wk.size());
    if (bf && l < L) {
      add_runs(ly.w_off, static_cast<long long>(ly.in) * ly.out, &ly);
      add_runs(ly.b_off, ly.out, nullptr);
    } else {
      add_runs(ly.w_off, static_cast<long long>(ly.in) * ly.out + ly.out, nullptr);
    }
    work_end[l] = static_cast<int>(wk.size());
  }
  n_work = static_cast<int>(wk.size());
  SB_TRY(dalloc(&work, wk.size()));
  SB_CUDA(cudaMemcpyAsync(work, wk.data(), wk.size() * sizeof(OptWork), cudaMemcpyHostToDevice, stream));
  SB_CUDA(cudaStreamSynchronize(stream));

  if (bf) {
    SB_TRY((set_gemm_tc_attrs<EPI_FWD, false, true>()));
    SB_TRY(set_gemm_fwd_out_attrs());
    SB_TRY(set_gemm_pp_attrs());
    SB_TRY(set_gemm_wide_attrs());
    SB_TRY((set_gemm_tc_attrs<EPI_DA, false, false>()));
    SB_TRY((set_gemm_tc_attrs<EPI_DW, true, true>()));
    SB_TRY(set_gemm_dw_attrs());
    const int co = cudaSharedmemCarveoutMaxShared;
    cudaFuncSetAttribute(load_batch_kernel<true>, cudaFuncAttributePreferredSharedMemoryCarveout, co);
    cudaFuncSetAttribute(out_layer_kernel<__nv_bfloat16>, cudaFuncAttributePreferredSharedMemoryCarveout, co);
  }
  return SB_OK;
}

Net::~Net() {
  if (!stream && allocs.empty()) return;
  cudaSetDevice(device);
  if (stream) cudaStreamSynchronize(stream);
  for (void* p : allocs) cudaFree(p);
  if (stream) cudaStreamDestroy(stream);
}

int Net::set_sparse(int n_dense_, int n_onehot_, int n_cat_) {
  SB_CHECK(n_dense_ >= 1 && n_onehot_ >= 1 && n_cat_ >= 1, SB_ERR_INVALID, "wide+deep needs >= 1 dense, one-hot and categorical column");
  SB_CHECK(n_dense_ + n_onehot_ == F, SB_ERR_INVALID, "n_dense (%d) + n_onehot (%d) must equal n_features (%d): the sparse path evaluates "
           "the SAME first layer", n_dense_, n_onehot_, F);
  SB_CUDA(cudaSetDevice(device));
  n_dense = n_dense_; n_onehot = n_onehot_; n_cat = n_cat_;
  ldD = round_up(n_dense, 8);
  if (!idx) SB_TRY(dalloc(&idx, static_cast<size_t>(max_batch) * n_cat));
  if (!E) SB_TRY(dalloc(&E, static_cast<size_t>(max_batch) * layers[0].ld_out));
  SB_CUDA(cudaStreamSynchronize(stream));
  return SB_OK;
}

int Net::enqueue_embed(int rows, bool scatter, float* grad, cudaStream_t st) {
  const Layer& l0 = layers[0];
  EmbedParams p = {};
  p.rows = rows; p.n_cat = n_cat; p.H = l0.out;
  p.idx = idx;
  p.np = nparts; p.ldW = tc() ? l0.ld_out : l0.out;
  if (tc()) { p.We = l0.Wn + static_cast<size_t>(n_dense) * l0.ld_out; p.We_ps = Wn_ps[0]; }
  else p.We32 = theta + l0.w_off + static_cast<long long>(n_dense) * l0.out;
  p.E = E; p.ldE = l0.ld_out;
  if (scatter) {
    if (tc()) { p.dZ = dZ[0]; p.dZ_ps = A_ps[0]; p.ld_dZ = l0.ld_out; }
    else { p.dZ32 = dZf[0]; p.ld_dZ = l0.out; }
    p.gWe = grad + l0.w_off + static_cast<long long>(n_dense) * l0.out;
    SB_TRY(launch_kernel(embed_scatter_kernel, dim3((rows + 7) / 8), dim3(256), 0, st, false, p));
    mark("embed_scatter");
  } else {
    SB_TRY(launch_kernel(embed_gather_kernel, dim3((rows + 7) / 8), dim3(256), 0, st, false, p));
    mark("embed_gather");
  }
  return SB_OK;
}

int Net::refresh_shadows() {
  if (!tc()) return SB_OK;
  shadow_refresh_kernel<<<n_work, 256, 0, stream>>>(work, theta);
  SB_CUDA(cudaGetLastError());
  return SB_OK;
}

int Net::enqueue_load(const StepIn& in, int rows, float* clear, long long clear_n) {
  const int Fx = in.sparse ? n_dense : F;
  const int ldx = in.sparse ? ldD : ldF;
  const long long units = static_cast<long long>(rows) * (ldx / 8);
  long long blocks = (units + 255) / 256;
  const long long cap = static_cast<long long>(num_sms) * 16;
  if (blocks > cap) blocks = cap;
  if (blocks < 1) blocks = 1;
  if (tc())
    SB_TRY(launch_kernel(load_batch_kernel<true>, dim3(static_cast<unsigned>(blocks)), dim3(256), 0, stream, true,
                         static_cast<const BatchDesc*>(in.desc), rows, Fx, Xb, ldx, static_cast<float*>(nullptr), in.scal, clear,
                         clear_n, nparts, Xb_ps));
  else
    SB_TRY(launch_kernel(load_batch_kernel<false>, dim3(static_cast<unsigned>(blocks)), dim3(256), 0, stream, true,
                         static_cast<const BatchDesc*>(in.desc), rows, Fx, static_cast<__nv_bfloat16*>(nullptr), ldx, Xf, in.scal,
                         clear, clear_n, 1, 0ll));
  mark("load_batch");
  if (in.sparse) SB_TRY(enqueue_embed(rows, false, nullptr, stream));
  return SB_OK;
}

int Net::enqueue_hidden_forward(const StepIn& in, int rows, float* grad, bool* fused_out, float4* clear, long long clear_n4) {
  if (fused_out) *fused_out = false;
  for (int l = 0; l < L; ++l) {
    Layer& ly = layers[l];
    const bool sp0 = (l == 0) && in.sparse;
    const int k_in = sp0 ? n_dense : ly.in;
    const int ld_k = sp0 ? ldD : ly.ld_in;
    if (tc()) {
      TmapSet tm;
      const bool res0 = (l == 0) && in.resident;
      const __nv_bfloat16* src = (l == 0) ? (res0 ? resident_Xb : Xb) : A[l - 1];
      const long long src_ps = (l == 0) ? (res0 ? resident_ps : Xb_ps) : A_ps[l - 1];
      const int src_rows = res0 ? static_cast<int>(resident_rows) : rows;
      SB_TRY(make_tmaps_bf16(tm.b, ly.Wn, Wn_ps[l], nparts, k_in, ly.out, ly.ld_out, 64));
      GemmTcParams p = {};
      set_part_pairs(&p, nparts);
      p.M = rows; p.N = ly.out; p.K = k_in;
      if (sp0) { p.addend = E; p.ld_add = ly.ld_out; }
      p.bias = theta + ly.b_off; p.act = ly.act;
      p.out = A[l]; p.ld_out = ly.ld_out; p.out_ps = A_ps[l];
      p.a_rows = res0 ? in.desc : nullptr;
      if (l == L - 1 && grad != nullptr && training && ly.out <= FWD_OUT_MAX_N && p.addend == nullptr) {
        FwdOutTmaps ft;
        SB_TRY(make_tmaps_bf16(ft.a, src, src_ps, nparts, src_rows, k_in, ld_k, 64));
        for (int i = 0; i < 3; ++i) ft.b[i] = tm.b[i];
        SB_TRY(make_tmaps_bf16(ft.o, dZ[l], A_ps[l], nparts, rows, ly.out, ly.ld_out, 64));
        const int tiles = (rows + 63) / 64;
        const int grid = tiles < num_sms ? tiles : num_sms;
        Layer& ol = layers[L];
        p.wo = theta + ol.w_off; p.bo = theta + ol.b_off;
        p.desc = in.desc; p.scal = in.scal; p.loss = loss;
        p.g_wo = grad + ol.w_off; p.g_bo = grad + ol.b_off; p.g_bL = grad + ly.b_off;
        p.trace = next_trace("fwd_out", l, rows, ly.out, k_in);
        SB_TRY(launch_gemm_fwd_out(grid, ft, p, stream, true));
        if (fused_out) *fused_out = true;
        mark("gemm_fwd_out");
        continue;
      }
      if (l == 0) { p.zero_buf = clear; p.zero_n4 = clear_n4; }
      p.trace = next_trace("fwd", l, rows, ly.out, k_in);
      if (nparts == 1 && p.addend == nullptr) {
        const PpPlan pp = plan_gemm_pp(rows, ly.out, k_in, num_sms, true);
        PpTmaps pt;
        SB_TRY(make_tmap_bf16(&pt.a, src, src_rows, k_in, ld_k, pp.bm_wg));
        pt.b = tm.b[0];
        SB_TRY(make_tmap_bf16(&pt.o, A[l], rows, ly.out, ly.ld_out, pp.bm_wg));
        if (pp.bn == 256) {
          SB_TRY(launch_gemm_wide(pp, pt, p, stream, true));
          mark("gemm_wide");
        } else {
          SB_TRY(launch_gemm_pp<EPI_FWD>(pp, pt, p, stream, true));
          mark("gemm_pp<FWD>");
        }
      } else {
        const GemmPlan pl = plan_gemm(rows, ly.out, round_up(k_in, 64) * pairs_of(nparts), num_sms, false);
        SB_TRY(make_tmaps_bf16(tm.a, src, src_ps, nparts, src_rows, k_in, ld_k, 128));
        SB_TRY((launch_gemm_tc<EPI_FWD, false, true>(pl, tm, p, stream, true)));
        mark(pl.bn == 64 ? "gemm_tc<64,FWD,GENERIC>" : "gemm_tc<128,FWD,GENERIC>");
      }
    } else {
      GemmF32Params p = {};
      p.M = rows; p.N = ly.out; p.K = k_in;
      p.A = (l == 0) ? Xf : Af[l - 1]; p.sAm = k_in; p.sAk = 1;
      if (sp0) { p.addend = E; p.ld_add = ly.ld_out; }
      p.B = theta + ly.w_off; p.sBk = ly.out; p.sBn = 1;
      p.bias = theta + ly.b_off; p.act = ly.act;
      p.out = Af[l]; p.ld_out = ly.out;
      SB_TRY(launch_gemm_f32<EPI_FWD>(p, 1, stream));
      mark("gemm_f32<FWD>");
    }
  }
  return SB_OK;
}

int Net::enqueue_out(const StepIn& in, int rows, bool do_loss, bool do_bwd, float* yhat_dst, float* grad) {
  Layer& hl = layers[L - 1];
  Layer& ol = layers[L];
  OutLayerParams p = {};
  p.rows = rows; p.H = hl.out;
  p.wo = theta + ol.w_off; p.bo = theta + ol.b_off;
  p.desc = in.desc; p.scal = in.scal; p.loss = loss; p.act = hl.act;
  p.do_bwd = do_bwd ? 1 : 0; p.do_loss = do_loss ? 1 : 0;
  p.yhat = yhat_dst;
  p.trace = next_trace("out_layer");
  if (do_bwd) {
    p.g_wo = grad + ol.w_off; p.g_bo = grad + ol.b_off; p.g_bL = grad + hl.b_off;
  }
  const int grid = (rows + 31) / 32;
  if (tc()) {
    p.A = A[L - 1]; p.ldA = hl.ld_out;
    p.np = nparts; p.a_ps = A_ps[L - 1]; p.dz_ps = A_ps[L - 1];
    if (do_bwd) { p.dZ = dZ[L - 1]; p.ld_dZ = hl.ld_out; }
    if (hl.out <= 1024) {
      int rpb = (rows + 2 * num_sms - 1) / (2 * num_sms);
      rpb = ((rpb + 7) / 8) * 8;
      if (rpb < 8) rpb = 8;
      const dim3 g((rows + rpb - 1) / rpb);
      if (hl.out <= 256) SB_TRY(launch_kernel(out_layer_rows_kernel<1>, g, dim3(256), 0, stream, true, p, rpb));
      else if (hl.out <= 512) SB_TRY(launch_kernel(out_layer_rows_kernel<2>, g, dim3(256), 0, stream, true, p, rpb));
      else SB_TRY(launch_kernel(out_layer_rows_kernel<4>, g, dim3(256), 0, stream, true, p, rpb));
    } else {
      SB_TRY(launch_kernel(out_layer_kernel<__nv_bfloat16>, dim3(grid), dim3(256), 0, stream, true, p));
    }
  } else {
    p.A = Af[L - 1]; p.ldA = hl.out;
    if (do_bwd) { p.dZ = dZf[L - 1]; p.ld_dZ = hl.out; }
    SB_TRY(launch_kernel(out_layer_kernel<float>, dim3(grid), dim3(256), 0, stream, true, p));
  }
  SB_CUDA(cudaGetLastError());
  mark("out_layer");
  return SB_OK;
}

int Net::enqueue_dw(const StepIn& in, int l, int rows, float* grad, cudaStream_t st, bool pdl, int sms, int r0, int r1, int chunk) {
  Layer& ly = layers[l];
  const bool sp0 = (l == 0) && in.sparse;
  const int in_rows = sp0 ? n_dense : ly.in;
  if (r1 < 0) r1 = in_rows;
  if (sp0) SB_TRY(enqueue_embed(rows, true, grad, st));
  if (!tc()) {
    GemmF32Params p = {};
    p.M = in_rows; p.N = ly.out; p.K = rows;
    p.A = (l == 0) ? Xf : Af[l - 1]; p.sAm = 1; p.sAk = in_rows;
    p.B = dZf[l]; p.sBk = ly.out; p.sBn = 1;
    p.accum = grad + ly.w_off; p.ld_acc = ly.out;
    const int tiles = ((p.M + 63) / 64) * ((p.N + 63) / 64);
    int split = (2 * num_sms) / (tiles > 0 ? tiles : 1);
    const int cap = (rows + 63) / 64;
    if (split > cap) split = cap;
    SB_TRY(launch_gemm_f32<EPI_DW>(p, split, st));
    mark("gemm_f32<DW>");
    return SB_OK;
  }
  const bool res0 = (l == 0) && in.resident;
  const int ld_k = sp0 ? ldD : ly.ld_in;
  const __nv_bfloat16* ap = (l == 0) ? (res0 ? resident_Xb : Xb) : A[l - 1];
  const long long ap_ps = (l == 0) ? (res0 ? resident_ps : Xb_ps) : A_ps[l - 1];
  const GemmPlan pl = plan_gemm(r1 - r0, ly.out, round_up(rows, 64) * pairs_of(nparts), sms, true);
  TmapSet tm;
  SB_TRY(make_tmaps_bf16(tm.a, ap + r0, ap_ps, nparts, res0 ? static_cast<int>(resident_rows) : rows, r1 - r0, ld_k, 64));
  SB_TRY(make_tmaps_bf16(tm.b, dZ[l], A_ps[l], nparts, rows, ly.out, ly.ld_out, 64));
  GemmTcParams p = {};
  set_part_pairs(&p, nparts);
  p.M = r1 - r0; p.N = ly.out; p.K = rows;
  p.a_rows = res0 ? in.desc : nullptr;
  p.accum = grad + ly.w_off + static_cast<long long>(r0) * ly.out; p.ld_acc = ly.out;
  p.acc_vec4 = (ly.out % 4 == 0 && ly.w_off % 4 == 0) ? 1 : 0;
  p.trace = next_trace("dW", l, r1 - r0, ly.out, rows, chunk);
  if (pl.bn == 256) {
    SB_TRY(launch_gemm_dw(pl, tm, p, st, pdl));
    mark("gemm_dw");
  } else {
    SB_TRY((launch_gemm_tc<EPI_DW, true, true>(pl, tm, p, st, pdl)));
    mark(pl.bn == 64 ? "gemm_tc<64,DW>" : "gemm_tc<128,DW>");
  }
  return SB_OK;
}

int Net::enqueue_da(int l, int rows, float* grad) {
  Layer& ly = layers[l];
  Layer& pl = layers[l - 1];
  if (!tc()) {
    GemmF32Params p = {};
    p.M = rows; p.N = ly.in; p.K = ly.out;
    p.A = dZf[l]; p.sAm = ly.out; p.sAk = 1;
    p.B = theta + ly.w_off; p.sBk = 1; p.sBn = ly.out;
    p.act = pl.act;
    p.aux = Af[l - 1]; p.ld_aux = pl.out;
    p.out = dZf[l - 1]; p.ld_out = pl.out;
    p.colsum = grad + pl.b_off;
    SB_TRY(launch_gemm_f32<EPI_DA>(p, 1, stream));
    mark("gemm_f32<DA>");
    return SB_OK;
  }
  GemmTcParams p = {};
  set_part_pairs(&p, nparts);
  p.M = rows; p.N = ly.in; p.K = ly.out;
  p.act = pl.act;
  p.aux = A[l - 1]; p.ld_aux = pl.ld_out; p.aux_ps = A_ps[l - 1];
  p.out = dZ[l - 1]; p.ld_out = pl.ld_out; p.out_ps = A_ps[l - 1];
  p.colsum = grad + pl.b_off;
  p.trace = next_trace("dA", l, rows, ly.in, ly.out);
  if (nparts == 1) {
    const PpPlan pp = plan_gemm_pp(rows, ly.in, ly.out, num_sms, false);
    PpTmaps pt;
    SB_TRY(make_tmap_bf16(&pt.a, dZ[l], rows, ly.out, ly.ld_out, pp.bm_wg));
    SB_TRY(make_tmap_bf16(&pt.b, ly.Wn, ly.in, ly.out, ly.ld_out, pp.bn));
    SB_TRY(make_tmap_bf16(&pt.o, dZ[l - 1], rows, ly.in, pl.ld_out, pp.bm_wg));
    SB_TRY(make_tmap_bf16(&pt.x, A[l - 1], rows, ly.in, pl.ld_out, pp.bm_wg));
    SB_TRY(launch_gemm_pp<EPI_DA>(pp, pt, p, stream, true));
    mark("gemm_pp<DA>");
  } else {
    const GemmPlan gp = plan_gemm(rows, ly.in, round_up(ly.out, 64) * pairs_of(nparts), num_sms, false);
    TmapSet tm;
    SB_TRY(make_tmaps_bf16(tm.a, dZ[l], A_ps[l], nparts, rows, ly.out, ly.ld_out, 128));
    SB_TRY(make_tmaps_bf16(tm.b, ly.Wn, Wn_ps[l], nparts, ly.in, ly.out, ly.ld_out, gp.bn));
    SB_TRY((launch_gemm_tc<EPI_DA, false, false>(gp, tm, p, stream, true)));
    mark(gp.bn == 64 ? "gemm_tc<64,DA,GENERIC>" : "gemm_tc<128,DA,GENERIC>");
  }
  return SB_OK;
}

template <typename T>
static int alloc_filled(DevBuf<T>* b, size_t n, int byte = 0) {
  SB_TRY(b->alloc(n));
  SB_CUDA(cudaMemset(b->p, byte, sizeof(T) * n));
  return SB_OK;
}

static int upload_parts(__nv_bfloat16* dst, const float* src, int rows, int cols, int ld, int np, long long ps) {
  const long long n = static_cast<long long>(rows) * cols;
  DevBuf<float> f32;
  SB_TRY(f32.alloc(n));
  SB_CUDA(cudaMemcpy(f32.p, src, sizeof(float) * n, cudaMemcpyHostToDevice));
  cast_bf16_kernel<<<static_cast<unsigned>((n + 255) / 256), 256>>>(f32.p, rows, cols, dst, ld, np, ps);
  SB_CUDA(cudaGetLastError());
  return SB_OK;
}

static int upload_bf16(DevBuf<__nv_bfloat16>* dst, const float* src, int rows, int cols, int np = 1) {
  const int ld = round_up(cols, 8);
  const long long ps = static_cast<long long>(rows) * ld;
  SB_TRY(alloc_filled(dst, static_cast<size_t>(ps) * np));
  return upload_parts(dst->p, src, rows, cols, ld, np, ps);
}

static int download_bf16(float* dst, const __nv_bfloat16* src, int rows, int cols, int np, long long part_stride,
                         std::vector<uint16_t>& raw) {
  const int ld = round_up(cols, 8);
  raw.resize(static_cast<size_t>(part_stride) * np);
  SB_CUDA(cudaMemcpy(raw.data(), src, sizeof(uint16_t) * raw.size(), cudaMemcpyDeviceToHost));
  for (int k = 0; k < np; ++k)
    for (int r = 0; r < rows; ++r)
      for (int c = 0; c < cols; ++c) {
        const uint32_t u = static_cast<uint32_t>(raw[static_cast<size_t>(k * part_stride) + static_cast<size_t>(r) * ld + c]) << 16;
        memcpy(dst + (static_cast<size_t>(k) * rows + r) * cols + c, &u, 4);
      }
  return SB_OK;
}

static int sync_hook(const char* kernel) {
  const cudaError_t e = cudaDeviceSynchronize();
  SB_CHECK(e == cudaSuccess, SB_ERR_CUDA, "%s failed: %s", kernel, cudaGetErrorString(e));
  return SB_OK;
}

template <typename Launch>
static int time_launches(Launch&& launch, int warmup, int iters, float* ms_out) {
  struct Events {
    cudaEvent_t e[2] = {};
    ~Events() { for (cudaEvent_t x : e) if (x) cudaEventDestroy(x); }
  } ev;
  SB_CUDA(cudaEventCreate(&ev.e[0]));
  SB_CUDA(cudaEventCreate(&ev.e[1]));
  for (int i = 0; i < warmup; ++i) SB_TRY(launch());
  SB_CUDA(cudaEventRecord(ev.e[0], 0));
  for (int i = 0; i < iters; ++i) SB_TRY(launch());
  SB_CUDA(cudaEventRecord(ev.e[1], 0));
  SB_CUDA(cudaEventSynchronize(ev.e[1]));
  float ms = 0.f;
  SB_CUDA(cudaEventElapsedTime(&ms, ev.e[0], ev.e[1]));
  *ms_out = ms / iters;
  return SB_OK;
}

static int debug_gemm_impl(const float* A, const float* B, float* D, int32_t M, int32_t N, int32_t K, int32_t split_k,
                           int32_t a_mn, int32_t b_mn, int32_t cfg_cg, int32_t cfg_bn, int device, int iters, float* ms_out) {
  SB_CHECK(cfg_cg == 0 || (cfg_cg == 1 && (cfg_bn == 64 || cfg_bn == 128 || (cfg_bn == 256 && a_mn && b_mn))), SB_ERR_INVALID,
           "tile configuration cg=%d bn=%d not instantiated for this layout (bn=256: MM only)", cfg_cg, cfg_bn);
  SB_CHECK(A && B && D && M > 0 && N > 0 && K > 0, SB_ERR_INVALID, "bad argument");
  SB_CHECK((a_mn == 0 && b_mn == 0) || (a_mn == 0 && b_mn == 1) || (a_mn == 1 && b_mn == 1), SB_ERR_INVALID,
           "layout combination not instantiated (use KK, KM or MM)");
  int sms = 0;
  SB_TRY(check_device(device, &sms));
  const int a_rows = a_mn ? K : M, a_cols = a_mn ? M : K;
  const int b_rows = b_mn ? K : N, b_cols = b_mn ? N : K;
  const int lda = round_up(a_cols, 8), ldb = round_up(b_cols, 8);
  DevBuf<__nv_bfloat16> dA, dB;
  DevBuf<float> dD;
  SB_TRY(upload_bf16(&dA, A, a_rows, a_cols));
  SB_TRY(upload_bf16(&dB, B, b_rows, b_cols));
  SB_TRY(alloc_filled(&dD, static_cast<size_t>(M) * N));
  GemmPlan pl = plan_gemm(M, N, K, sms, false);
  if (cfg_cg > 0) pl.bn = cfg_bn;
  {
    const int total_kb = (K + 63) / 64;
    int want = split_k < 1 ? 1 : (split_k > total_kb ? total_kb : split_k);
    pl.kb_per_split = (total_kb + want - 1) / want;
    pl.split_k = (total_kb + pl.kb_per_split - 1) / pl.kb_per_split;
    const int work = ((M + 127) / 128) * ((N + pl.bn - 1) / pl.bn) * pl.split_k;
    pl.grid = work < sms ? work : sms;
  }
  TmapSet tms;
  SB_TRY(make_tmap_bf16(&tms.a[0], dA.p, a_rows, a_cols, lda, a_mn ? 64 : 128));
  SB_TRY(make_tmap_bf16(&tms.b[0], dB.p, b_rows, b_cols, ldb, b_mn ? 64 : pl.bn));
  GemmTcParams p = {};
  p.M = M; p.N = N; p.K = K;
  p.accum = dD.p; p.ld_acc = N;
  p.acc_vec4 = (N % 4 == 0) ? 1 : 0;
  if (pl.bn == 256) {
    SB_TRY(set_gemm_dw_attrs());
    SB_TRY(launch_gemm_dw(pl, tms, p, 0));
  } else if (!a_mn && !b_mn) {
    SB_TRY((set_gemm_tc_attrs<EPI_F32, false, false>()));
    SB_TRY((launch_gemm_tc<EPI_F32, false, false>(pl, tms, p, 0)));
  } else if (!a_mn) {
    SB_TRY((set_gemm_tc_attrs<EPI_F32, false, true>()));
    SB_TRY((launch_gemm_tc<EPI_F32, false, true>(pl, tms, p, 0)));
  } else {
    SB_TRY((set_gemm_tc_attrs<EPI_F32, true, true>()));
    SB_TRY((launch_gemm_tc<EPI_F32, true, true>(pl, tms, p, 0)));
  }
  if (iters > 0) {
    const int ldn = round_up(N, 8);
    DevBuf<float> d_bias, d_colsum;
    DevBuf<__nv_bfloat16> d_out, d_aux;
    SB_TRY(alloc_filled(&d_bias, N));
    SB_TRY(alloc_filled(&d_colsum, N));
    SB_TRY(d_out.alloc(static_cast<size_t>(M) * ldn));
    SB_TRY(alloc_filled(&d_aux, static_cast<size_t>(M) * ldn, 0x3f));
    GemmTcParams q = p;
    q.bias = d_bias.p; q.act = SB_ACT_RELU; q.out = d_out.p; q.ld_out = ldn; q.aux = d_aux.p; q.ld_aux = ldn; q.colsum = d_colsum.p;
    const PpPlan pp = plan_gemm_pp(M, N, K, sms, !a_mn && b_mn);
    PpTmaps pt;
    if (!a_mn) {
      SB_TRY(make_tmap_bf16(&pt.a, dA.p, a_rows, a_cols, lda, pp.bm_wg));
      SB_TRY(make_tmap_bf16(&pt.b, dB.p, b_rows, b_cols, ldb, b_mn ? 64 : pp.bn));
      SB_TRY(make_tmap_bf16(&pt.o, d_out.p, M, N, ldn, pp.bm_wg));
      SB_TRY(make_tmap_bf16(&pt.x, d_aux.p, M, N, ldn, pp.bm_wg));
    }
    auto real = [&]() -> int {
      if (!a_mn && !b_mn) return launch_gemm_pp<EPI_DA>(pp, pt, q, 0, false);
      if (!a_mn) return pp.bn == 256 ? launch_gemm_wide(pp, pt, q, 0, false) : launch_gemm_pp<EPI_FWD>(pp, pt, q, 0, false);
      if (pl.bn == 256) return launch_gemm_dw(pl, tms, q, 0, false);
      return launch_gemm_tc<EPI_DW, true, true>(pl, tms, q, 0, false);
    };
    SB_TRY((a_mn ? set_gemm_tc_attrs<EPI_DW, true, true>() : set_gemm_pp_attrs()));
    if (pp.bn == 256) SB_TRY(set_gemm_wide_attrs());
    SB_TRY(time_launches(real, 3, iters, ms_out));
    if (getenv("SB_GEMM_TRACE")) {
      DevBuf<unsigned long long> d_tr;
      SB_TRY(alloc_filled(&d_tr, 16));
      q.trace = d_tr.p;
      SB_CUDA(cudaDeviceSynchronize());
      float one = 0.f;
      SB_TRY(time_launches(real, 0, 1, &one));
      unsigned long long h[16];
      SB_CUDA(cudaMemcpy(h, d_tr.p, sizeof(h), cudaMemcpyDeviceToHost));
      if (a_mn)
        fprintf(stderr, "[trace] M=%d N=%d K=%d bn=%d split=%d single-launch %.2f us | ns since entry:", M, N, K, pl.bn, pl.split_k,
                one * 1e3f);
      else
        fprintf(stderr, "[trace] M=%d N=%d K=%d ping-pong bm_wg=%d bn=%d single-launch %.2f us | ns since entry:", M, N, K, pp.bm_wg,
                pp.bn, one * 1e3f);
      const char* nm[9] = {"entry", "setup", "deps", "tma0", "land0", "mma_done", "acc_ready", "epi_done", "exit"};
      for (int i = 1; i < 9; ++i) fprintf(stderr, " %s=%lld", nm[i], (long long)(h[i] - h[0]));
      fprintf(stderr, "\n");
    }
  }
  SB_TRY(sync_hook("gemm_tc_kernel"));
  SB_CUDA(cudaMemcpy(D, dD.p, sizeof(float) * M * N, cudaMemcpyDeviceToHost));
  return SB_OK;
}
}

using namespace sb;

extern "C" {

int sb_debug_gemm_bf16_cfg(const float* A, const float* B, float* D, int32_t M, int32_t N, int32_t K, int32_t split_k,
                           int32_t a_mn, int32_t b_mn, int32_t cfg_cg, int32_t cfg_bn, int device) {
  return debug_gemm_impl(A, B, D, M, N, K, split_k, a_mn, b_mn, cfg_cg, cfg_bn, device, 0, nullptr);
}
int sb_debug_gemm_bench(const float* A, const float* B, float* D, int32_t M, int32_t N, int32_t K, int32_t split_k,
                        int32_t a_mn, int32_t b_mn, int32_t cfg_cg, int32_t cfg_bn, int device, int32_t iters, float* ms_out) {
  SB_CHECK(iters > 0 && ms_out, SB_ERR_INVALID, "iters / ms_out");
  return debug_gemm_impl(A, B, D, M, N, K, split_k, a_mn, b_mn, cfg_cg, cfg_bn, device, iters, ms_out);
}

int sb_debug_gemm_layer(int32_t kind, int32_t precision, const float* A, const float* W, const float* bias, const float* aux,
                        const float* addend, float* out, float* colsum, float* grad, int32_t* guard, char* route,
                        int32_t route_cap, int32_t M, int32_t N, int32_t K, int32_t a_rows, int32_t row0, int32_t act,
                        int32_t r0, int32_t r1, int32_t sms, int64_t clear_n4, int device) {
  enum { FWD = 0, DA = 1, DW = 2 };
  SB_CHECK(kind >= FWD && kind <= DW, SB_ERR_INVALID, "kind=%d (0 forward, 1 dA, 2 dW)", kind);
  SB_CHECK(precision >= SB_PREC_FP32 && precision <= SB_PREC_BF16X2, SB_ERR_INVALID, "precision=%d invalid", precision);
  SB_CHECK(act >= SB_ACT_NONE && act <= SB_ACT_LEAKYRELU, SB_ERR_INVALID, "act=%d invalid", act);
  SB_CHECK(M > 0 && N > 0 && K > 0, SB_ERR_INVALID, "M=%d N=%d K=%d", M, N, K);
  SB_CHECK(A && W && guard && (route == nullptr || route_cap > 0), SB_ERR_INVALID, "null argument");
  SB_CHECK(kind != FWD || (bias && out), SB_ERR_INVALID, "the forward GEMM needs bias and out");
  SB_CHECK(kind != DA || (aux && out && colsum), SB_ERR_INVALID, "the dA GEMM needs aux, out and colsum");
  SB_CHECK(kind != DW || grad, SB_ERR_INVALID, "the dW GEMM needs grad");
  SB_CHECK(addend == nullptr || kind == FWD, SB_ERR_INVALID, "an addend belongs to the forward GEMM only");
  const bool tc = precision != SB_PREC_FP32;
  const int rows = kind == DW ? K : M;
  SB_CHECK(row0 >= 0 && static_cast<long long>(row0) + rows <= a_rows, SB_ERR_INVALID, "rows %d..%d outside the %d rows of A",
           row0, row0 + rows - 1, a_rows);
  const bool resident = row0 != 0 || a_rows != rows;
  SB_CHECK(!resident || (tc && kind != DA && addend == nullptr), SB_ERR_INVALID,
           "a resident batch is read by the layer-0 forward / dW GEMMs of a dense tensor-core step only");
  if (kind == DW) {
    SB_CHECK(r0 >= 0 && r0 < r1 && r1 <= M && r0 % 8 == 0, SB_ERR_INVALID, "rows r0=%d .. r1=%d of the %d-row gradient "
             "(r0 a multiple of 8)", r0, r1, M);
    SB_CHECK(tc || (r0 == 0 && r1 == M), SB_ERR_INVALID, "the fp32 dW GEMM has no row chunks");
  }
  SB_CHECK(clear_n4 >= 0 && (clear_n4 == 0 || (kind == FWD && tc)), SB_ERR_INVALID,
           "clear_n4=%lld: the tensor-core forward GEMM only", static_cast<long long>(clear_n4));
  SB_CHECK(sms >= 0, SB_ERR_INVALID, "sms=%d", sms);
  int dev_sms = 0;
  SB_TRY(check_device(device, &dev_sms));
  SB_CHECK(sms <= dev_sms, SB_ERR_INVALID, "sms=%d above the %d SMs", sms, dev_sms);

  sb_net_desc d = {};
  d.n_features = kind == FWD ? (addend ? K + 1 : K) : (kind == DA ? 8 : M);
  d.n_hidden = kind == DA ? 2 : 1;
  d.hidden[0] = N; d.acts[0] = kind == DW ? SB_ACT_NONE : act;
  d.hidden[1] = K; d.acts[1] = SB_ACT_NONE;
  d.loss = SB_LOSS_MSE; d.optimizer = SB_OPT_SGD;
  d.max_batch = kind == DW ? K : M + 64;
  d.precision = precision;
  constexpr int GUARD = 256;
  const uint32_t S32 = 0x7f7f7f7fu;
  const uint16_t S16 = 0x7f7f;
  DevBuf<__nv_bfloat16> res;
  DevBuf<float> g, clr;
  Net net;
  SB_TRY(net.init(&d, device, true));
  if (sms > 0) net.num_sms = sms;
  const int np = net.nparts;
  if (addend) SB_TRY(net.set_sparse(K, 1, 1));
  const Layer& l0 = net.layers[0];
  std::vector<float> theta(static_cast<size_t>(net.n_params), 0.f);
  if (kind == FWD) {
    std::copy(W, W + static_cast<size_t>(K) * N, theta.begin() + l0.w_off);
    std::copy(bias, bias + N, theta.begin() + l0.b_off);
  } else if (kind == DA) {
    std::copy(W, W + static_cast<size_t>(N) * K, theta.begin() + net.layers[1].w_off);
  }
  SB_CUDA(cudaMemcpy(net.theta, theta.data(), sizeof(float) * theta.size(), cudaMemcpyHostToDevice));
  BatchDesc hd = {};
  hd.row0 = row0;
  SB_CUDA(cudaMemcpy(net.desc, &hd, sizeof(hd), cudaMemcpyHostToDevice));
  if (kind != DA) {
    const int cols = kind == FWD ? K : M;
    if (resident) {
      net.resident_ps = static_cast<long long>(a_rows) * net.ldF;
      net.resident_rows = a_rows;
      SB_TRY(alloc_filled(&res, static_cast<size_t>(net.resident_ps) * np));
      SB_TRY(upload_parts(res.p, A, a_rows, cols, net.ldF, np, net.resident_ps));
      net.resident_Xb = res.p;
    } else if (tc) {
      SB_TRY(upload_parts(net.Xb, A, rows, cols, addend ? net.ldD : net.ldF, np, net.Xb_ps));
    } else {
      SB_CUDA(cudaMemcpy(net.Xf, A, sizeof(float) * rows * cols, cudaMemcpyHostToDevice));
    }
  }
  if (addend)
    SB_CUDA(cudaMemcpy2D(net.E, sizeof(float) * l0.ld_out, addend, sizeof(float) * N, sizeof(float) * N, M, cudaMemcpyHostToDevice));
  if (kind == DA) {
    if (tc) {
      SB_TRY(upload_parts(net.dZ[1], A, M, K, net.layers[1].ld_out, np, net.A_ps[1]));
      SB_TRY(upload_parts(net.A[0], aux, M, N, l0.ld_out, np, net.A_ps[0]));
    } else {
      SB_CUDA(cudaMemcpy(net.dZf[1], A, sizeof(float) * M * K, cudaMemcpyHostToDevice));
      SB_CUDA(cudaMemcpy(net.Af[0], aux, sizeof(float) * M * N, cudaMemcpyHostToDevice));
    }
  }
  if (kind == DW) {
    if (tc) SB_TRY(upload_parts(net.dZ[0], W, K, N, l0.ld_out, np, net.A_ps[0]));
    else SB_CUDA(cudaMemcpy(net.dZf[0], W, sizeof(float) * K * N, cudaMemcpyHostToDevice));
  }
  void* outp = nullptr;
  size_t out_bytes = 0;
  if (kind != DW) {
    outp = tc ? static_cast<void*>(kind == FWD ? net.A[0] : net.dZ[0]) : static_cast<void*>(kind == FWD ? net.Af[0] : net.dZf[0]);
    out_bytes = tc ? sizeof(__nv_bfloat16) * net.A_ps[0] * np : sizeof(float) * static_cast<size_t>(net.max_batch) * N;
    SB_CUDA(cudaMemset(outp, 0x7f, out_bytes));
  }
  const size_t g_n = static_cast<size_t>(net.n_params) + GUARD;
  std::vector<float> hg(g_n);
  {
    float s;
    memcpy(&s, &S32, 4);
    std::fill(hg.begin(), hg.end(), s);
  }
  auto in_region = [&](size_t i) {
    if (kind == DA) return i >= static_cast<size_t>(l0.b_off) && i < static_cast<size_t>(l0.b_off) + N;
    return i >= static_cast<size_t>(r0) * N && i < static_cast<size_t>(r1) * N;
  };
  if (kind == DA) std::copy(colsum, colsum + N, hg.begin() + l0.b_off);
  if (kind == DW) std::copy(grad + static_cast<size_t>(r0) * N, grad + static_cast<size_t>(r1) * N, hg.begin() + static_cast<size_t>(r0) * N);
  if (kind != FWD) {
    SB_TRY(g.alloc(g_n));
    SB_CUDA(cudaMemcpy(g.p, hg.data(), sizeof(float) * g_n, cudaMemcpyHostToDevice));
  }
  const size_t clr_n = clear_n4 > 0 ? static_cast<size_t>(clear_n4) * 4 + GUARD : 0;
  if (clear_n4 > 0) SB_TRY(alloc_filled(&clr, clr_n, 0x7f));
  SB_CUDA(cudaDeviceSynchronize());

  StepIn in;
  in.desc = net.desc; in.scal = net.scal; in.resident = resident; in.sparse = addend != nullptr;
  SB_TRY(net.refresh_shadows());
  net.launches = 0;
  if (kind == FWD) SB_TRY(net.enqueue_hidden_forward(in, M, nullptr, nullptr, reinterpret_cast<float4*>(clr.p), clear_n4));
  else if (kind == DA) SB_TRY(net.enqueue_da(1, M, g.p));
  else SB_TRY(net.enqueue_dw(in, 0, K, g.p, net.stream, false, sms > 0 ? sms : dev_sms, r0, r1));
  SB_CHECK(net.launches == 1 && net.last_kernel != nullptr, SB_ERR_STATE, "%d GEMM launches", net.launches);
  SB_TRY(sync_hook(net.last_kernel));
  if (route) {
    strncpy(route, net.last_kernel, static_cast<size_t>(route_cap) - 1);
    route[route_cap - 1] = '\0';
  }

  int32_t changed = 0;
  if (kind != DW) {
    if (tc) {
      std::vector<uint16_t> h;
      SB_TRY(download_bf16(out, static_cast<const __nv_bfloat16*>(outp), M, N, np, net.A_ps[0], h));
      const uint16_t a0 = kind == FWD && act == SB_ACT_SIGMOID ? 0x3f00 : 0;
      const int ld = l0.ld_out;
      for (int k = 0; k < np; ++k)
        for (int r = 0; r < M + 64; ++r)
          for (int c = (r < M ? N : 0); c < ld; ++c) {
            const uint16_t v = h[static_cast<size_t>(k * net.A_ps[0]) + static_cast<size_t>(r) * ld + c];
            const uint16_t want = k == 0 ? a0 : 0;
            const bool legit = r < M && (v == want || (want == 0 && v == 0x8000));
            if (v != S16 && !legit) ++changed;
          }
    } else {
      std::vector<uint32_t> h(static_cast<size_t>(M + 64) * N);
      SB_CUDA(cudaMemcpy(h.data(), outp, sizeof(uint32_t) * h.size(), cudaMemcpyDeviceToHost));
      memcpy(out, h.data(), sizeof(float) * M * N);
      for (size_t i = static_cast<size_t>(M) * N; i < h.size(); ++i) changed += h[i] != S32;
    }
  }
  if (kind != FWD) {
    SB_CUDA(cudaMemcpy(hg.data(), g.p, sizeof(float) * g_n, cudaMemcpyDeviceToHost));
    for (size_t i = 0; i < g_n; ++i) {
      uint32_t u;
      memcpy(&u, &hg[i], 4);
      if (!in_region(i) && u != S32) ++changed;
    }
    if (kind == DA) std::copy(hg.begin() + l0.b_off, hg.begin() + l0.b_off + N, colsum);
    else std::copy(hg.begin() + static_cast<size_t>(r0) * N, hg.begin() + static_cast<size_t>(r1) * N, grad + static_cast<size_t>(r0) * N);
  }
  if (clear_n4 > 0) {
    std::vector<uint32_t> h(clr_n);
    SB_CUDA(cudaMemcpy(h.data(), clr.p, sizeof(uint32_t) * clr_n, cudaMemcpyDeviceToHost));
    for (size_t i = 0; i < clr_n; ++i) changed += i < clr_n - GUARD ? h[i] != 0u : h[i] != S32;
  }
  *guard = changed;
  return SB_OK;
}

int sb_debug_gemm_epilogue(const float* A, const float* W, const float* bias, const float* aux, float* out, float* colsum,
                           int32_t M, int32_t N, int32_t K, int32_t da, int32_t act, int32_t bm_wg, int device,
                           int32_t iters, float* ms_out) {
  SB_CHECK(A && W && out && M > 0 && N > 0 && K > 0 && (da == 0 || da == 1), SB_ERR_INVALID, "bad argument");
  SB_CHECK(da ? aux != nullptr : bias != nullptr, SB_ERR_INVALID, "the forward GEMM needs a bias, the dA GEMM an aux matrix");
  SB_CHECK(act >= SB_ACT_NONE && act <= SB_ACT_LEAKYRELU, SB_ERR_INVALID, "act invalid");
  SB_CHECK(bm_wg == 0 || bm_wg == 64 || bm_wg == 128 || bm_wg == PP_TILE_WIDE, SB_ERR_INVALID,
           "bm_wg must be 0, 64, 128 or %d (got %d)", PP_TILE_WIDE, bm_wg);
  SB_CHECK(!(da && bm_wg == PP_TILE_WIDE), SB_ERR_INVALID, "the %d-wide tile is for the forward GEMM only", PP_TILE_WIDE);
  SB_CHECK(iters >= 0 && (iters == 0 || ms_out != nullptr), SB_ERR_INVALID, "iters / ms_out");
  int sms = 0;
  SB_TRY(check_device(device, &sms));
  const int w_rows = da ? N : K, w_cols = da ? K : N;
  const int lda = round_up(K, 8), ldw = round_up(w_cols, 8), ldn = round_up(N, 8);
  DevBuf<__nv_bfloat16> dA, dW, d_out, d_aux;
  DevBuf<float> d_bias, d_col;
  SB_TRY(upload_bf16(&dA, A, M, K));
  SB_TRY(upload_bf16(&dW, W, w_rows, w_cols));
  SB_TRY(alloc_filled(&d_out, static_cast<size_t>(M) * ldn));
  SB_TRY(aux ? upload_bf16(&d_aux, aux, M, N) : alloc_filled(&d_aux, static_cast<size_t>(M) * ldn));
  SB_TRY(alloc_filled(&d_bias, N));
  SB_TRY(alloc_filled(&d_col, N));
  if (bias) SB_CUDA(cudaMemcpy(d_bias.p, bias, sizeof(float) * N, cudaMemcpyHostToDevice));
  const PpPlan pp = plan_gemm_pp(M, N, K, sms, da == 0, bm_wg);
  PpTmaps pt;
  SB_TRY(make_tmap_bf16(&pt.a, dA.p, M, K, lda, pp.bm_wg));
  SB_TRY(make_tmap_bf16(&pt.b, dW.p, w_rows, w_cols, ldw, da ? pp.bn : 64));
  SB_TRY(make_tmap_bf16(&pt.o, d_out.p, M, N, ldn, pp.bm_wg));
  SB_TRY(make_tmap_bf16(&pt.x, d_aux.p, M, N, ldn, pp.bm_wg));
  GemmTcParams p = {};
  p.M = M; p.N = N; p.K = K;
  p.act = act; p.bias = d_bias.p; p.colsum = colsum ? d_col.p : nullptr;
  auto launch = [&]() {
    if (da) return launch_gemm_pp<EPI_DA>(pp, pt, p, 0, false);
    return pp.bn == 256 ? launch_gemm_wide(pp, pt, p, 0, false) : launch_gemm_pp<EPI_FWD>(pp, pt, p, 0, false);
  };
  const char* kernel = pp.bn == 256 ? "gemm_wide_kernel" : "gemm_pp_kernel";
  SB_TRY(pp.bn == 256 ? set_gemm_wide_attrs() : set_gemm_pp_attrs());
  SB_TRY(launch());
  SB_TRY(sync_hook(kernel));
  std::vector<uint16_t> h;
  SB_TRY(download_bf16(out, d_out.p, M, N, 1, static_cast<long long>(M) * ldn, h));
  if (colsum) SB_CUDA(cudaMemcpy(colsum, d_col.p, sizeof(float) * N, cudaMemcpyDeviceToHost));
  if (iters > 0) {
    SB_TRY(time_launches(launch, 3, iters, ms_out));
    SB_TRY(sync_hook(kernel));
  }
  return SB_OK;
}

int sb_debug_gemm_fwd_out(const float* A, const float* W, const float* bias, const float* wo, float bo, const float* y,
                          const float* w, float* dZ, float* g_bL, float* g_wo, float* g_bo, float* loss_sum, int32_t* guard,
                          int32_t M, int32_t N, int32_t K, int32_t a_rows, int32_t row0, int32_t act, int32_t loss,
                          int32_t np, int32_t grid, int device) {
  SB_CHECK(A && W && bias && wo && y && w && dZ && g_bL && g_wo && g_bo && loss_sum && guard, SB_ERR_INVALID, "null argument");
  SB_CHECK(M > 0 && K > 0 && N >= 1 && N <= FWD_OUT_MAX_N, SB_ERR_INVALID, "M=%d K=%d N=%d (N must be 1..%d)", M, K, N,
           FWD_OUT_MAX_N);
  SB_CHECK(np >= 1 && np <= 3, SB_ERR_INVALID, "np=%d outside 1..3", np);
  SB_CHECK(loss == SB_LOSS_MSE || loss == SB_LOSS_SIGMOID_CE, SB_ERR_INVALID, "loss invalid");
  SB_CHECK(act >= SB_ACT_NONE && act <= SB_ACT_LEAKYRELU, SB_ERR_INVALID, "act invalid");
  SB_CHECK(grid >= 0, SB_ERR_INVALID, "grid=%d", grid);
  SB_CHECK(row0 >= 0 && static_cast<long long>(row0) + M <= a_rows, SB_ERR_INVALID, "rows %d..%d outside the %d rows of A", row0,
           row0 + M - 1, a_rows);
  int sms = 0;
  SB_TRY(check_device(device, &sms));
  SB_CHECK(grid <= sms, SB_ERR_INVALID, "grid=%d above the %d SMs", grid, sms);
  const int lda = round_up(K, 8), ldn = round_up(N, 8), dz_rows = M + 64;
  const long long a_ps = static_cast<long long>(a_rows) * lda, w_ps = static_cast<long long>(K) * ldn;
  const long long dz_ps = static_cast<long long>(dz_rows) * ldn;
  DevBuf<__nv_bfloat16> dA, dW, d_dz;
  DevBuf<float> d_vec, d_yw;
  DevBuf<BatchDesc> d_desc;
  SB_TRY(upload_bf16(&dA, A, a_rows, K, np));
  SB_TRY(upload_bf16(&dW, W, K, N, np));
  SB_TRY(alloc_filled(&d_dz, static_cast<size_t>(dz_ps) * np, 0x7f));
  float nnz = 0.f;
  for (int r = 0; r < M; ++r) nnz += (w[r] != 0.f) ? 1.f : 0.f;
  std::vector<float> h_vec(4 * N + 2 + SCAL_COUNT, 0.f);
  std::copy(bias, bias + N, h_vec.begin());
  std::copy(wo, wo + N, h_vec.begin() + N);
  std::copy(g_bL, g_bL + N, h_vec.begin() + 2 * N);
  std::copy(g_wo, g_wo + N, h_vec.begin() + 3 * N);
  h_vec[4 * N] = bo;
  h_vec[4 * N + 1] = *g_bo;
  h_vec[4 * N + 2 + SCAL_LOSS_SUM] = *loss_sum;
  h_vec[4 * N + 2 + SCAL_NNZ] = nnz;
  SB_TRY(d_vec.alloc(h_vec.size()));
  SB_CUDA(cudaMemcpy(d_vec.p, h_vec.data(), sizeof(float) * h_vec.size(), cudaMemcpyHostToDevice));
  float* d_bias = d_vec.p;
  float* d_wo = d_vec.p + N;
  float* d_gbL = d_vec.p + 2 * N;
  float* d_gwo = d_vec.p + 3 * N;
  float* d_bo = d_vec.p + 4 * N;
  float* d_gbo = d_bo + 1;
  float* d_scal = d_bo + 2;
  SB_TRY(d_yw.alloc(2 * static_cast<size_t>(M)));
  SB_CUDA(cudaMemcpy(d_yw.p, y, sizeof(float) * M, cudaMemcpyHostToDevice));
  SB_CUDA(cudaMemcpy(d_yw.p + M, w, sizeof(float) * M, cudaMemcpyHostToDevice));
  BatchDesc h_desc = {};
  h_desc.y = d_yw.p; h_desc.w = d_yw.p + M; h_desc.gscale = 1.f; h_desc.row0 = row0;
  SB_TRY(d_desc.alloc(1));
  SB_CUDA(cudaMemcpy(d_desc.p, &h_desc, sizeof(BatchDesc), cudaMemcpyHostToDevice));
  const bool resident = row0 != 0 || a_rows != M;
  FwdOutTmaps ft;
  SB_TRY(make_tmaps_bf16(ft.a, dA.p, a_ps, np, a_rows, K, lda, 64));
  SB_TRY(make_tmaps_bf16(ft.b, dW.p, w_ps, np, K, N, ldn, 64));
  SB_TRY(make_tmaps_bf16(ft.o, d_dz.p, dz_ps, np, M, N, ldn, 64));
  GemmTcParams p = {};
  set_part_pairs(&p, np);
  p.M = M; p.N = N; p.K = K;
  p.bias = d_bias; p.act = act;
  p.a_rows = resident ? d_desc.p : nullptr;
  p.wo = d_wo; p.bo = d_bo;
  p.desc = d_desc.p; p.scal = d_scal; p.loss = loss;
  p.g_wo = d_gwo; p.g_bo = d_gbo; p.g_bL = d_gbL;
  const int tiles = (M + 63) / 64;
  const int step_grid = tiles < sms ? tiles : sms;
  SB_TRY(set_gemm_fwd_out_attrs());
  SB_TRY(launch_gemm_fwd_out(grid > 0 ? grid : step_grid, ft, p, 0, false));
  SB_TRY(sync_hook("gemm_fwd_out_kernel"));
  std::vector<uint16_t> h;
  SB_TRY(download_bf16(dZ, d_dz.p, M, N, np, dz_ps, h));
  SB_CUDA(cudaMemcpy(h_vec.data(), d_vec.p, sizeof(float) * h_vec.size(), cudaMemcpyDeviceToHost));
  int32_t changed = 0;
  for (int k = 0; k < np; ++k)
    for (int r = 0; r < dz_rows; ++r)
      for (int c = 0; c < ldn; ++c) {
        const uint16_t v = h[static_cast<size_t>(k * dz_ps) + static_cast<size_t>(r) * ldn + c];
        if ((r >= M || c >= N) && v != 0x7f7f && (r >= M || (v & 0x7fff) != 0)) ++changed;
      }
  *guard = changed;
  std::copy(h_vec.begin() + 2 * N, h_vec.begin() + 3 * N, g_bL);
  std::copy(h_vec.begin() + 3 * N, h_vec.begin() + 4 * N, g_wo);
  *g_bo = h_vec[4 * N + 1];
  *loss_sum = h_vec[4 * N + 2 + SCAL_LOSS_SUM];
  return SB_OK;
}

}
```

shifu-tensorflow_b200/csrc/net.cuh:

```cuda
#pragma once
#include <vector>
#include <map>
#include <mutex>
#include "common.cuh"
#include "gemm_tc.cuh"
#include "gemm_f32.cuh"
#include "kernels.cuh"
#include "nccl_dyn.h"

namespace sb {

struct Layer {
  int in, out, act;
  long long w_off, b_off;
  __nv_bfloat16* Wn = nullptr;
  int ld_in = 0, ld_out = 0;
};

struct StepIn {
  BatchDesc* desc = nullptr;
  float* scal = nullptr;
  bool resident = false;
  bool sparse = false;
};

inline int pairs_of(int np) { return np == 3 ? 6 : (np == 2 ? 3 : 1); }

struct Net {
  int device = 0, num_sms = 132;
  cudaStream_t stream = nullptr;
  std::vector<int> work_begin, work_end;
  int F = 0, L = 0;
  std::vector<Layer> layers;
  long long n_params = 0;
  int precision = SB_PREC_FP32, loss = SB_LOSS_MSE;
  int nparts = 1;
  bool tc() const { return precision != SB_PREC_FP32; }
  long long Xb_ps = 0;
  std::vector<long long> A_ps, Wn_ps;
  long long resident_ps = 0;
  int max_batch = 0, ldB = 0, ldF = 0;
  bool training = false;

  char* arena = nullptr;
  size_t arena_bytes = 0, arena_extra_bytes = 0;
  size_t s1_off = 0, s2_off = 0, shadow_off = 0, extra_off = 0;
  float* theta = nullptr;
  float *s1 = nullptr, *s2 = nullptr;
  __nv_bfloat16* Xb = nullptr;
  std::vector<__nv_bfloat16*> A, dZ;
  float* Xf = nullptr;
  std::vector<float*> Af, dZf;
  float *yhat = nullptr, *ones = nullptr;
  BatchDesc* desc = nullptr;
  float* scal = nullptr;
  float *stX = nullptr, *stY = nullptr, *stW = nullptr;
  OptWork* work = nullptr;
  int n_work = 0;
  int launches = 0;
  unsigned long long* step_trace = nullptr;
  int trace_k = 0;
  std::vector<std::string> trace_names;
  bool trace_on = true;
  int trace_n = 0;
  unsigned long long* next_trace(const char* name, int layer = -1, int M = 0, int N = 0, int K = 0, int chunk = -1) {
    if (!step_trace || !trace_on || trace_k >= 32) return nullptr;
    if (static_cast<int>(trace_names.size()) <= trace_k) trace_names.resize(trace_k + 1);
    std::string nm = name;
    if (layer >= 0) nm += std::to_string(layer);
    if (chunk >= 0) nm += "." + std::to_string(chunk);
    if (M > 0) nm += "@" + std::to_string(M) + "x" + std::to_string(N) + "x" + std::to_string(K);
    trace_names[trace_k] = nm;
    trace_n = trace_k + 1;
    return step_trace + 16 * (trace_k++);
  }
  const char* last_kernel = nullptr;
  void mark(const char* kernel) { ++launches; last_kernel = kernel; }

  std::vector<void*> allocs;
  template <typename T> int dalloc(T** p, size_t n) {
    void* q = nullptr;
    SB_CUDA(cudaMalloc(&q, n * sizeof(T) + 256));
    allocs.push_back(q);
    SB_CUDA(cudaMemsetAsync(q, 0, n * sizeof(T) + 256, stream));
    *p = reinterpret_cast<T*>(q);
    return SB_OK;
  }

  Net() = default;
  Net(const Net&) = delete;
  Net& operator=(const Net&) = delete;
  ~Net();
  int init(const sb_net_desc* d, int device_, bool training_);
  int refresh_shadows();
  int enqueue_load(const StepIn& in, int rows, float* clear = nullptr, long long clear_n = 0);
  int enqueue_hidden_forward(const StepIn& in, int rows, float* grad = nullptr, bool* fused_out = nullptr, float4* clear = nullptr,
                             long long clear_n4 = 0);
  int n_dense = 0, n_onehot = 0, n_cat = 0, ldD = 0;
  int* idx = nullptr;
  float* E = nullptr;
  int set_sparse(int n_dense_, int n_onehot_, int n_cat_);
  int enqueue_embed(int rows, bool scatter, float* grad, cudaStream_t st);
  const __nv_bfloat16* resident_Xb = nullptr;
  long long resident_rows = 0;
  int enqueue_out(const StepIn& in, int rows, bool do_loss, bool do_bwd, float* yhat_dst, float* grad);
  int enqueue_dw(const StepIn& in, int l, int rows, float* grad, cudaStream_t st, bool pdl, int sms, int r0 = 0, int r1 = -1,
                 int chunk = -1);
  int enqueue_da(int l, int rows, float* grad);
};

int validate_desc(const sb_net_desc* d);

}
```

shifu-tensorflow_b200/csrc/ptx.cuh:

```cuda
#pragma once
#include <cuda_bf16.h>
#include <stdint.h>

namespace sb {

__device__ __forceinline__ uint32_t smem_u32(const void* p) {
  return static_cast<uint32_t>(__cvta_generic_to_shared(p));
}

__device__ __forceinline__ void mbar_init(uint32_t bar, uint32_t count) {
  asm volatile("mbarrier.init.shared::cta.b64 [%0], %1;" ::"r"(bar), "r"(count) : "memory");
}
__device__ __forceinline__ void fence_barrier_init() {
  asm volatile("fence.mbarrier_init.release.cluster;" ::: "memory");
}
__device__ __forceinline__ void fence_proxy_async() {
  asm volatile("fence.proxy.async.shared::cta;" ::: "memory");
}
__device__ __forceinline__ void mbar_arrive(uint32_t bar) {
  asm volatile("mbarrier.arrive.shared::cta.b64 _, [%0];" ::"r"(bar) : "memory");
}
__device__ __forceinline__ void mbar_arrive_expect_tx(uint32_t bar, uint32_t bytes) {
  asm volatile("mbarrier.arrive.expect_tx.shared::cta.b64 _, [%0], %1;" ::"r"(bar), "r"(bytes) : "memory");
}
__device__ __forceinline__ uint64_t globaltimer_ns() {
  uint64_t t;
  asm volatile("mov.u64 %0, %globaltimer;" : "=l"(t));
  return t;
}
__device__ __forceinline__ void mbar_wait(uint32_t bar, uint32_t parity) {
  uint32_t done = 0;
  uint32_t spins = 0;
  uint64_t t0 = 0;
  while (true) {
    asm volatile(
        "{\n\t.reg .pred p;\n\t"
        "mbarrier.try_wait.parity.shared::cta.b64 p, [%1], %2;\n\t"
        "selp.b32 %0, 1, 0, p;\n\t}"
        : "=r"(done)
        : "r"(bar), "r"(parity)
        : "memory");
    if (done) break;
    if ((++spins & 0x3FFu) == 0) {
      uint64_t now = globaltimer_ns();
      if (t0 == 0) t0 = now;
      else if (now - t0 > 4000000000ull) __trap();
    }
  }
}

__device__ __forceinline__ void tma_prefetch_desc(const void* tmap) {
  asm volatile("prefetch.tensormap [%0];" ::"l"(tmap) : "memory");
}
__device__ __forceinline__ void tma_load_2d(uint32_t dst_smem, const void* tmap, uint32_t bar, int c0, int c1) {
  asm volatile(
      "cp.async.bulk.tensor.2d.shared::cluster.global.mbarrier::complete_tx::bytes [%0], [%1, {%3, %4}], [%2];"
      ::"r"(dst_smem), "l"(tmap), "r"(bar), "r"(c0), "r"(c1)
      : "memory");
}
__device__ __forceinline__ void tma_store_2d(const void* tmap, uint32_t src_smem, int c0, int c1) {
  asm volatile("cp.async.bulk.tensor.2d.global.shared::cta.bulk_group [%0, {%2, %3}], [%1];"
               ::"l"(tmap), "r"(src_smem), "r"(c0), "r"(c1)
               : "memory");
}
__device__ __forceinline__ void tma_store_commit() { asm volatile("cp.async.bulk.commit_group;" ::: "memory"); }
template <int N>
__device__ __forceinline__ void tma_store_wait_read() {
  asm volatile("cp.async.bulk.wait_group.read %0;" ::"n"(N) : "memory");
}

__device__ __forceinline__ void wgmma_fence() { asm volatile("wgmma.fence.sync.aligned;" ::: "memory"); }
__device__ __forceinline__ void wgmma_commit() { asm volatile("wgmma.commit_group.sync.aligned;" ::: "memory"); }
template <int N>
__device__ __forceinline__ void wgmma_wait() { asm volatile("wgmma.wait_group.sync.aligned %0;" ::"n"(N) : "memory"); }

#define SB_F8(i) "+f"(d[i]), "+f"(d[i + 1]), "+f"(d[i + 2]), "+f"(d[i + 3]), "+f"(d[i + 4]), "+f"(d[i + 5]), "+f"(d[i + 6]), "+f"(d[i + 7])
template <int N, int TA, int TB>
__device__ __forceinline__ void wgmma_bf16(float (&d)[N / 2], uint64_t desc_a, uint64_t desc_b, uint32_t scale_d) {
  static_assert(N == 32 || N == 64 || N == 128 || N == 256, "wgmma N");
  if constexpr (N == 32) {
    asm volatile(
        "{\n\t.reg .pred p;\n\t"
        "setp.ne.b32 p, %18, 0;\n\t"
        "wgmma.mma_async.sync.aligned.m64n32k16.f32.bf16.bf16 "
        "{%0, %1, %2, %3, %4, %5, %6, %7, %8, %9, %10, %11, %12, %13, %14, %15}, "
        "%16, %17, p, 1, 1, %19, %20;\n\t}"
        : SB_F8(0), SB_F8(8)
        : "l"(desc_a), "l"(desc_b), "r"(scale_d), "n"(TA), "n"(TB));
  }
  if constexpr (N == 64) {
    asm volatile(
        "{\n\t.reg .pred p;\n\t"
        "setp.ne.b32 p, %34, 0;\n\t"
        "wgmma.mma_async.sync.aligned.m64n64k16.f32.bf16.bf16 "
        "{%0, %1, %2, %3, %4, %5, %6, %7, %8, %9, %10, %11, %12, %13, %14, %15, %16, %17, %18, %19, %20, %21, %22, %23, %24, %25, %26, %27, %28, %29, %30, %31}, "
        "%32, %33, p, 1, 1, %35, %36;\n\t}"
        : SB_F8(0), SB_F8(8), SB_F8(16), SB_F8(24)
        : "l"(desc_a), "l"(desc_b), "r"(scale_d), "n"(TA), "n"(TB));
  }
  if constexpr (N == 128) {
    asm volatile(
        "{\n\t.reg .pred p;\n\t"
        "setp.ne.b32 p, %66, 0;\n\t"
        "wgmma.mma_async.sync.aligned.m64n128k16.f32.bf16.bf16 "
        "{%0, %1, %2, %3, %4, %5, %6, %7, %8, %9, %10, %11, %12, %13, %14, %15, %16, %17, %18, %19, %20, %21, %22, %23, %24, %25, %26, %27, %28, %29, %30, %31, %32, %33, %34, %35, %36, %37, %38, %39, %40, %41, %42, %43, %44, %45, %46, %47, %48, %49, %50, %51, %52, %53, %54, %55, %56, %57, %58, %59, %60, %61, %62, %63}, "
        "%64, %65, p, 1, 1, %67, %68;\n\t}"
        : SB_F8(0), SB_F8(8), SB_F8(16), SB_F8(24), SB_F8(32), SB_F8(40), SB_F8(48), SB_F8(56)
        : "l"(desc_a), "l"(desc_b), "r"(scale_d), "n"(TA), "n"(TB));
  }
  if constexpr (N == 256) {
    asm volatile(
        "{\n\t.reg .pred p;\n\t"
        "setp.ne.b32 p, %130, 0;\n\t"
        "wgmma.mma_async.sync.aligned.m64n256k16.f32.bf16.bf16 "
        "{%0, %1, %2, %3, %4, %5, %6, %7, %8, %9, %10, %11, %12, %13, %14, %15, %16, %17, %18, %19, %20, %21, %22, %23, %24, %25, %26, %27, %28, %29, %30, %31, "
        "%32, %33, %34, %35, %36, %37, %38, %39, %40, %41, %42, %43, %44, %45, %46, %47, %48, %49, %50, %51, %52, %53, %54, %55, %56, %57, %58, %59, %60, %61, %62, %63, "
        "%64, %65, %66, %67, %68, %69, %70, %71, %72, %73, %74, %75, %76, %77, %78, %79, %80, %81, %82, %83, %84, %85, %86, %87, %88, %89, %90, %91, %92, %93, %94, %95, "
        "%96, %97, %98, %99, %100, %101, %102, %103, %104, %105, %106, %107, %108, %109, %110, %111, %112, %113, %114, %115, %116, %117, %118, %119, %120, %121, %122, %123, %124, %125, %126, %127}, "
        "%128, %129, p, 1, 1, %131, %132;\n\t}"
        : SB_F8(0), SB_F8(8), SB_F8(16), SB_F8(24), SB_F8(32), SB_F8(40), SB_F8(48), SB_F8(56),
          SB_F8(64), SB_F8(72), SB_F8(80), SB_F8(88), SB_F8(96), SB_F8(104), SB_F8(112), SB_F8(120)
        : "l"(desc_a), "l"(desc_b), "r"(scale_d), "n"(TA), "n"(TB));
  }
}

#undef SB_F8

__device__ __forceinline__ uint64_t make_kmajor_sw128_desc(uint32_t smem_addr) {
  uint64_t d = 0;
  d |= static_cast<uint64_t>((smem_addr >> 4) & 0x3FFFu);
  d |= static_cast<uint64_t>(1024u >> 4) << 32;
  d |= static_cast<uint64_t>(1) << 62;
  return d;
}
__device__ __forceinline__ uint64_t make_mnmajor_sw128_desc(uint32_t smem_addr, uint32_t lbo_bytes) {
  uint64_t d = 0;
  d |= static_cast<uint64_t>((smem_addr >> 4) & 0x3FFFu);
  d |= static_cast<uint64_t>((lbo_bytes >> 4) & 0x3FFFu) << 16;
  d |= static_cast<uint64_t>(1024u >> 4) << 32;
  d |= static_cast<uint64_t>(1) << 62;
  return d;
}

__device__ __forceinline__ void pdl_wait() { asm volatile("griddepcontrol.wait;" ::: "memory"); }
__device__ __forceinline__ void pdl_launch_dependents() { asm volatile("griddepcontrol.launch_dependents;" ::: "memory"); }

__device__ __forceinline__ uint32_t pack_bf16x2(float lo, float hi) {
  __nv_bfloat162 h = __floats2bfloat162_rn(lo, hi);
  return *reinterpret_cast<uint32_t*>(&h);
}
__device__ __forceinline__ void red_add_f32(float* addr, float v) {
  asm volatile("red.global.add.f32 [%0], %1;" ::"l"(addr), "f"(v) : "memory");
}
__device__ __forceinline__ void red_add_v4_f32(float* addr, float a, float b, float c, float d) {
  asm volatile("red.global.add.v4.f32 [%0], {%1, %2, %3, %4};" ::"l"(addr), "f"(a), "f"(b), "f"(c), "f"(d) : "memory");
}

}
```

Measured before the change: 37.38 million.

## Store ReLU activation-gradient bitmask in forward GEMM and use it in dA

The forward GEMM epilogue for ReLU and leaky-ReLU layers now packs a one-bit-per-element positivity mask into shared memory and writes it out. The dA GEMM bulk-loads that compact mask instead of TMA-loading the bf16 activation tile to derive the derivative. Reading one bit per element instead of sixteen cuts the backward epilogue's auxiliary traffic, at the cost of an extra mask write in the forward pass, more shared memory and new mask buffers per layer. Debug APIs are extended so the mask can be inspected.

```diff
diff --git a/include/shifu_b200.h b/include/shifu_b200.h
--- a/include/shifu_b200.h
+++ b/include/shifu_b200.h
@@ -151,6 +151,11 @@
                         const float* addend, float* out, float* colsum, float* grad, int32_t* guard, char* route,
                         int32_t route_cap, int32_t M, int32_t N, int32_t K, int32_t a_rows, int32_t row0, int32_t act,
                         int32_t r0, int32_t r1, int32_t sms, int64_t clear_n4, int device);
+int sb_debug_gemm_layer_mask(int32_t kind, int32_t precision, const float* A, const float* W, const float* bias,
+                             const float* aux, const float* addend, float* out, float* colsum, float* grad, int32_t* guard,
+                             char* route, int32_t route_cap, int32_t M, int32_t N, int32_t K, int32_t a_rows, int32_t row0,
+                             int32_t act, int32_t r0, int32_t r1, int32_t sms, int64_t clear_n4, int device,
+                             uint32_t* mask_out, int64_t mask_cap, int32_t aux_path);
 
 int sb_debug_step_trace(sb_trainer_t* t, uint64_t* stamps, int32_t cap_kernels, char* names, int32_t names_cap, int32_t* n_kernels);
 int sb_debug_gemm_bench(const float* A, const float* B, float* D, int32_t M, int32_t N, int32_t K, int32_t split_k,
@@ -160,6 +165,10 @@
 int sb_debug_gemm_epilogue(const float* A, const float* W, const float* bias, const float* aux, float* out, float* colsum,
                            int32_t M, int32_t N, int32_t K, int32_t da, int32_t act, int32_t bm_wg, int device,
                            int32_t iters, float* ms_out);
+int sb_debug_gemm_epilogue_mask(const float* A, const float* W, const float* bias, const float* aux, float* out,
+                                float* colsum, int32_t M, int32_t N, int32_t K, int32_t da, int32_t act, int32_t bm_wg,
+                                int device, int32_t iters, float* ms_out, uint32_t* mask_out, int64_t mask_cap,
+                                int32_t aux_path);
 
 int sb_debug_gemm_fwd_out(const float* A, const float* W, const float* bias, const float* wo, float bo, const float* y,
                           const float* w, float* dZ, float* g_bL, float* g_wo, float* g_bo, float* loss_sum, int32_t* guard,
diff --git a/shifu-tensorflow_b200/_capi.py b/shifu-tensorflow_b200/_capi.py
--- a/shifu-tensorflow_b200/_capi.py
+++ b/shifu-tensorflow_b200/_capi.py
@@ -139,6 +139,10 @@
     "sb_debug_gemm_layer": (C.c_int, [C.c_int32, C.c_int32, _f32p, _f32p, _f32p, _f32p, _f32p, _f32p, _f32p, _f32p, _P(C.c_int32),
                                       C.c_char_p, C.c_int32, C.c_int32, C.c_int32, C.c_int32, C.c_int32, C.c_int32, C.c_int32,
                                       C.c_int32, C.c_int32, C.c_int32, C.c_int64, C.c_int]),
+    "sb_debug_gemm_layer_mask": (C.c_int, [C.c_int32, C.c_int32, _f32p, _f32p, _f32p, _f32p, _f32p, _f32p, _f32p, _f32p,
+                                           _P(C.c_int32), C.c_char_p, C.c_int32, C.c_int32, C.c_int32, C.c_int32, C.c_int32,
+                                           C.c_int32, C.c_int32, C.c_int32, C.c_int32, C.c_int32, C.c_int64, C.c_int,
+                                           _P(C.c_uint32), C.c_int64, C.c_int32]),
     "sb_debug_step_trace": (C.c_int, [_vp, C.POINTER(C.c_uint64), C.c_int32, C.c_char_p, C.c_int32, C.POINTER(C.c_int32)]),
     "sb_debug_gemm_bench": (C.c_int, [_f32p, _f32p, _f32p, C.c_int32, C.c_int32, C.c_int32, C.c_int32, C.c_int32, C.c_int32,
                                       C.c_int32, C.c_int32, C.c_int, C.c_int32, _f32p]),
@@ -146,6 +150,9 @@
                                          C.c_int32, C.c_int32, C.c_int]),
     "sb_debug_gemm_epilogue": (C.c_int, [_f32p, _f32p, _f32p, _f32p, _f32p, _f32p, C.c_int32, C.c_int32, C.c_int32, C.c_int32,
                                          C.c_int32, C.c_int32, C.c_int, C.c_int32, _f32p]),
+    "sb_debug_gemm_epilogue_mask": (C.c_int, [_f32p, _f32p, _f32p, _f32p, _f32p, _f32p, C.c_int32, C.c_int32, C.c_int32,
+                                              C.c_int32, C.c_int32, C.c_int32, C.c_int, C.c_int32, _f32p, _P(C.c_uint32),
+                                              C.c_int64, C.c_int32]),
     "sb_debug_gemm_fwd_out": (C.c_int, [_f32p, _f32p, _f32p, _f32p, C.c_float, _f32p, _f32p, _f32p, _f32p, _f32p, _f32p, _f32p,
                                         _P(C.c_int32), C.c_int32, C.c_int32, C.c_int32, C.c_int32, C.c_int32, C.c_int32,
                                         C.c_int32, C.c_int32, C.c_int32, C.c_int]),
@@ -562,7 +569,8 @@
 def debug_gemm_layer(kind: int, precision: int, A: np.ndarray, W: np.ndarray, act: int = ACT_NONE,
                      bias: Optional[np.ndarray] = None, aux: Optional[np.ndarray] = None, addend: Optional[np.ndarray] = None,
                      colsum: Optional[np.ndarray] = None, grad: Optional[np.ndarray] = None, M: Optional[int] = None,
-                     row0: int = 0, r0: int = 0, r1: Optional[int] = None, sms: int = 0, clear_n4: int = 0, device: int = 0):
+                     row0: int = 0, r0: int = 0, r1: Optional[int] = None, sms: int = 0, clear_n4: int = 0, device: int = 0,
+                     mask_out: Optional[np.ndarray] = None, aux_path: bool = False):
     A, W = _f32(A), _f32(W)
     nparts = PARTS[precision]
     out = cs = g = None
@@ -590,9 +598,9 @@
     addend = None if addend is None else _f32(addend)
     guard = C.c_int32(-1)
     route = C.create_string_buffer(64)
-    check(lib().sb_debug_gemm_layer(kind, precision, _ptr(A), _ptr(W), _ptr(bias), _ptr(aux), _ptr(addend), _ptr(out), _ptr(cs),
-                                    _ptr(g), C.byref(guard), route, 64, M, N, K, a_rows_arg, row0, act, r0,
-                                    M if r1 is None else r1, sms, clear_n4, device))
+    check(lib().sb_debug_gemm_layer_mask(kind, precision, _ptr(A), _ptr(W), _ptr(bias), _ptr(aux), _ptr(addend), _ptr(out),
+                                         _ptr(cs), _ptr(g), C.byref(guard), route, 64, M, N, K, a_rows_arg, row0, act, r0,
+                                         M if r1 is None else r1, sms, clear_n4, device, *_mask_args(mask_out), int(aux_path)))
     return out, cs, g, int(guard.value), route.value.decode()
 
 
@@ -621,8 +629,30 @@
     return float(ms.value)
 
 
+def act_mask_words(rows: int, N: int) -> int:
+    return (rows + 63) // 64 * ((N + 63) // 64) * 128
+
+
+def act_mask_bits(words: np.ndarray, M: int, N: int) -> np.ndarray:
+    rbs, cbs = (M + 63) // 64, (N + 63) // 64
+    w = np.asarray(words, np.uint32)[:rbs * cbs * 128].reshape(rbs, cbs, 4, 8, 4)
+    bits = (w[..., None] >> np.arange(32, dtype=np.uint32)) & 1
+    bits = bits.reshape(rbs, cbs, 4, 8, 4, 8, 2, 2)
+    full = bits.transpose(0, 2, 6, 3, 1, 5, 4, 7).reshape(rbs * 64, cbs * 64)
+    return full[:M, :N].astype(bool)
+
+
+def _mask_args(mask_out: Optional[np.ndarray]):
+    if mask_out is None:
+        return None, 0
+    if mask_out.dtype != np.uint32 or not mask_out.flags.c_contiguous:
+        raise ValueError("mask_out must be a contiguous uint32 array")
+    return mask_out.ctypes.data_as(_P(C.c_uint32)), mask_out.size
+
+
 def debug_gemm_epilogue(A: np.ndarray, W: np.ndarray, act: int, bias: Optional[np.ndarray] = None,
-                        aux: Optional[np.ndarray] = None, bm_wg: int = 0, iters: int = 0, device: int = 0):
+                        aux: Optional[np.ndarray] = None, bm_wg: int = 0, iters: int = 0, device: int = 0,
+                        mask_out: Optional[np.ndarray] = None, aux_path: bool = False):
     A, W = _f32(A), _f32(W)
     M, K = A.shape
     da = aux is not None
@@ -633,9 +663,9 @@
     out = np.zeros((M, N), np.float32)
     cs = np.zeros(N, np.float32) if da else None
     ms = C.c_float()
-    check(lib().sb_debug_gemm_epilogue(_ptr(A), _ptr(W), _ptr(bias) if bias is not None else None,
-                                       _ptr(aux) if da else None, _ptr(out), _ptr(cs) if da else None, M, N, K, int(da),
-                                       act, bm_wg, device, iters, C.byref(ms)))
+    check(lib().sb_debug_gemm_epilogue_mask(_ptr(A), _ptr(W), _ptr(bias) if bias is not None else None,
+                                            _ptr(aux) if da else None, _ptr(out), _ptr(cs) if da else None, M, N, K, int(da),
+                                            act, bm_wg, device, iters, C.byref(ms), *_mask_args(mask_out), int(aux_path)))
     return out, cs, (float(ms.value) if iters > 0 else None)
 
 
diff --git a/shifu-tensorflow_b200/csrc/capi.cu b/shifu-tensorflow_b200/csrc/capi.cu
--- a/shifu-tensorflow_b200/csrc/capi.cu
+++ b/shifu-tensorflow_b200/csrc/capi.cu
@@ -290,7 +290,7 @@
   if (!n.tc()) {
     for (int l = L - 1; l >= 0; --l) {
       SB_TRY(n.enqueue_dw(in, l, rows, g, n.stream, false, S));
-      if (l > 0) SB_TRY(n.enqueue_da(l, rows, g));
+      if (l > 0) SB_TRY(n.enqueue_da(in, l, rows, g));
     }
   } else {
     const bool split_tail = kind == G_STEP && (t->world == 1 || t->p2p_ready) && L > 1;
@@ -301,7 +301,7 @@
         SB_TRY(join_streams(t->side, n.stream, t->ev_dz[l]));
         SB_TRY(n.enqueue_dw(in, l, rows, g, t->side, false, l == 1 ? d1.sms[1] : S));
       }
-      SB_TRY(n.enqueue_da(l, rows, g));
+      SB_TRY(n.enqueue_da(in, l, rows, g));
     }
     if (split_tail) SB_CUDA(cudaEventRecord(t->ev_da_done, n.stream));
     if (L == 1) {
diff --git a/shifu-tensorflow_b200/csrc/common.cuh b/shifu-tensorflow_b200/csrc/common.cuh
--- a/shifu-tensorflow_b200/csrc/common.cuh
+++ b/shifu-tensorflow_b200/csrc/common.cuh
@@ -110,6 +110,26 @@
   }
 }
 
+inline bool act_has_mask(int act) { return act == SB_ACT_RELU || act == SB_ACT_LEAKYRELU; }
+__host__ __device__ __forceinline__ int act_mask_col_blocks(int N) { return (N + 63) / 64; }
+__host__ __device__ __forceinline__ long long act_mask_word(int rb, int cb, int N, int t) {
+  return (static_cast<long long>(rb) * act_mask_col_blocks(N) + cb) * 128 + t;
+}
+__host__ __device__ __forceinline__ size_t act_mask_words(int rows, int N) {
+  return static_cast<size_t>((rows + 63) / 64) * act_mask_col_blocks(N) * 128;
+}
+__device__ __forceinline__ void act_mask_collect(uint32_t (&acc)[2], uint32_t packed, int k) {
+  const uint32_t gt = __hgt2_mask(*reinterpret_cast<const __nv_bfloat162*>(&packed), __nv_bfloat162(0.f, 0.f));
+  const int j = 2 * (k & 7);
+  acc[k >> 3] |= gt & ((1u << j) | (1u << (17 + j)));
+}
+__device__ __forceinline__ uint32_t act_mask_fold(const uint32_t (&acc)[2]) {
+  return (acc[0] & 0xFFFFu) | (acc[0] >> 16) | (acc[1] << 16) | (acc[1] & 0xFFFF0000u);
+}
+__device__ __forceinline__ float act_grad_from_bit(bool pos, int act) {
+  return pos ? 1.f : (act == SB_ACT_LEAKYRELU ? SB_LEAKY_ALPHA : 0.f);
+}
+
 __device__ __forceinline__ float warp_sum(float v) {
 #pragma unroll
   for (int o = 16; o > 0; o >>= 1) v += __shfl_xor_sync(0xffffffffu, v, o);
diff --git a/shifu-tensorflow_b200/csrc/gemm_pp.cuh b/shifu-tensorflow_b200/csrc/gemm_pp.cuh
--- a/shifu-tensorflow_b200/csrc/gemm_pp.cuh
+++ b/shifu-tensorflow_b200/csrc/gemm_pp.cuh
@@ -11,27 +11,33 @@
 };
 
 template <int BM_WG, int BN>
-struct GemmPpCfg : RingCfg<BM_WG * 64 * 2, BN * 64 * 2, 1024 + 256 + 2 * BN * 4 + 16 * BN * 4 + 2 * BM_WG * BN * 2> {
+struct GemmPpCfg : RingCfg<BM_WG * 64 * 2, BN * 64 * 2,
+                           1024 + 256 + 2 * BN * 4 + 16 * BN * 4 + 2 * BM_WG * BN * 2 + 2 * BM_WG * BN / 8> {
   static_assert(BM_WG == 64 || BM_WG == 128, "warpgroup tile rows");
   static_assert(BN == 64 || BN == 128, "tile N");
   static_assert(GemmPpCfg::STAGES >= 4, "operand ring");
   static constexpr int X_TILE = BM_WG * 128;
   static constexpr int X_BYTES = X_TILE * (BN / 64);
+  static constexpr int M_BLOCK = 512;
+  static constexpr int M_BYTES = M_BLOCK * (BM_WG / 64) * (BN / 64);
 };
 
-template <int BM_WG, int BN, int EPI, int ACT>
+template <int BM_WG, int BN, int EPI, int ACT, bool MASK = false>
 __global__ void __launch_bounds__(GemmPpCfg<BM_WG, BN>::THREADS, 1)
 gemm_pp_kernel(const __grid_constant__ PpTmaps tms, const GemmTcParams p) {
   static_assert(EPI == EPI_FWD || EPI == EPI_DA, "forward or dA");
   using Cfg = GemmPpCfg<BM_WG, BN>;
   constexpr int BK = Cfg::BK, MI = BM_WG / 64;
   constexpr bool B_MN = EPI == EPI_FWD;
+  constexpr bool MASKED = ACT == SB_ACT_RELU || ACT == SB_ACT_LEAKYRELU;
+  static_assert(!MASK || MASKED, "an act' mask for relu / leaky relu only");
 
   extern __shared__ uint8_t smem_raw[];
   const Ring<Cfg> ring(smem_raw, 2 * Cfg::X_BYTES);
   const uint32_t xs_base = ring.end();
   const uint32_t sm_bias = ring.bars + 256u;
   const uint32_t sm_col = sm_bias + 2u * BN * 4u;
+  const uint32_t ms_base = sm_col + 16u * BN * 4u;
   auto aux_bar = [&](int g) { return ring.bar(g); };
 
   const int warp = threadIdx.x >> 5;
@@ -72,6 +78,7 @@
     const bool xthread = gt == 0;
     auto bar_wg = [&]() { asm volatile("bar.sync %0, 128;" ::"r"(2 + g) : "memory"); };
     const uint32_t xs = xs_base + static_cast<uint32_t>(g) * Cfg::X_BYTES;
+    const uint32_t ms = ms_base + static_cast<uint32_t>(g) * Cfg::M_BYTES;
     const uint32_t bias_s = sm_bias + static_cast<uint32_t>(g) * BN * 4u;
     const uint32_t col_w = sm_col + static_cast<uint32_t>(g * 8 + (warp & 3)) * BN * 4u;
     const int r0 = (warp & 3) * 16 + (lane >> 2);
@@ -96,8 +103,14 @@
           asm volatile("st.shared.f32 [%0], %1;" ::"r"(bias_s + j * 4u), "f"(bv) : "memory");
         }
         bar_wg();
-      } else {
-        if (xthread) {
+      } else if (ACT != SB_ACT_NONE && xthread) {
+        if constexpr (MASK) {
+          const int nmi = min(MI, (p.M - m0 + 63) / 64);
+          mbar_arrive_expect_tx(aux_bar(g), static_cast<uint32_t>(nmi * nx * Cfg::M_BLOCK));
+          for (int mi = 0; mi < nmi; ++mi)
+            bulk_load_1d(ms + mi * (BN / 64) * Cfg::M_BLOCK, p.mask + act_mask_word(m0 / 64 + mi, n0 / 64, p.N, 0),
+                         static_cast<uint32_t>(nx * Cfg::M_BLOCK), aux_bar(g));
+        } else {
           mbar_arrive_expect_tx(aux_bar(g), static_cast<uint32_t>(nx * Cfg::X_TILE));
           for (int x = 0; x < nx; ++x) tma_load_2d(xs + x * Cfg::X_TILE, &tms.x, aux_bar(g), n0 + x * 64, m0);
         }
@@ -110,6 +123,7 @@
       });
 
       if constexpr (EPI == EPI_FWD) {
+        uint32_t ma[MI][2];
 #pragma unroll
         for (int i = 0; i < BN / 8; ++i) {
           const int c = c0 + 8 * i;
@@ -117,16 +131,26 @@
           asm volatile("ld.shared.v2.f32 {%0, %1}, [%2];" : "=f"(b.x), "=f"(b.y) : "r"(bias_s + c * 4u) : "memory");
 #pragma unroll
           for (int mi = 0; mi < MI; ++mi) {
+            if (MASK && i % 8 == 0) ma[mi][0] = ma[mi][1] = 0u;
 #pragma unroll
             for (int h = 0; h < 2; ++h) {
               const float v0 = act_apply(acc[mi][4 * i + 2 * h] + b.x, ACT);
               const float v1 = act_apply(acc[mi][4 * i + 2 * h + 1] + b.y, ACT);
-              asm volatile("st.shared.b32 [%0], %1;" ::"r"(xaddr(64 * mi + r0 + 8 * h, c)), "r"(pack_bf16x2(v0, v1)) : "memory");
+              const uint32_t pk = pack_bf16x2(v0, v1);
+              asm volatile("st.shared.b32 [%0], %1;" ::"r"(xaddr(64 * mi + r0 + 8 * h, c)), "r"(pk) : "memory");
+              if (MASK) act_mask_collect(ma[mi], pk, 2 * (i % 8) + h);
+            }
+            if (MASK && i % 8 == 7) {
+              const int row = m0 + 64 * mi + r0;
+              const uint32_t keep = (row < p.M ? 0x33333333u : 0u) | (row + 8 < p.M ? 0xCCCCCCCCu : 0u);
+              asm volatile("st.shared.b32 [%0], %1;"
+                           ::"r"(ms + (mi * (BN / 64) + i / 8) * Cfg::M_BLOCK + gt * 4u), "r"(act_mask_fold(ma[mi]) & keep)
+                           : "memory");
             }
           }
         }
       } else {
-        mbar_wait(aux_bar(g), static_cast<uint32_t>(it) & 1u);
+        if (ACT != SB_ACT_NONE) mbar_wait(aux_bar(g), static_cast<uint32_t>(it) & 1u);
         const uint32_t cb = col_w + static_cast<uint32_t>(it & 1) * 4u * BN * 4u;
 #pragma unroll
         for (int x = 0; x < BN / 64; ++x) {
@@ -137,14 +161,26 @@
             float s0 = 0.f, s1 = 0.f;
 #pragma unroll
             for (int mi = 0; mi < MI; ++mi) {
+              uint32_t mw = 0u;
+              if (MASK)
+                asm volatile("ld.shared.b32 %0, [%1];"
+                             : "=r"(mw) : "r"(ms + (mi * (BN / 64) + x) * Cfg::M_BLOCK + gt * 4u) : "memory");
 #pragma unroll
               for (int h = 0; h < 2; ++h) {
                 const uint32_t a = xaddr(64 * mi + r0 + 8 * h, c);
-                uint32_t raw;
-                asm volatile("ld.shared.b32 %0, [%1];" : "=r"(raw) : "r"(a) : "memory");
-                const float x0 = __uint_as_float(raw << 16), x1 = __uint_as_float(raw & 0xFFFF0000u);
-                const float v0 = acc[mi][32 * x + 4 * i + 2 * h] * act_grad_from_out(x0, ACT);
-                const float v1 = acc[mi][32 * x + 4 * i + 2 * h + 1] * act_grad_from_out(x1, ACT);
+                float g0 = 1.f, g1 = 1.f;
+                if (MASK) {
+                  const int bit = 4 * i + 2 * h;
+                  g0 = act_grad_from_bit((mw >> bit) & 1u, ACT);
+                  g1 = act_grad_from_bit((mw >> (bit + 1)) & 1u, ACT);
+                } else if (ACT != SB_ACT_NONE) {
+                  uint32_t raw;
+                  asm volatile("ld.shared.b32 %0, [%1];" : "=r"(raw) : "r"(a) : "memory");
+                  g0 = act_grad_from_out(__uint_as_float(raw << 16), ACT);
+                  g1 = act_grad_from_out(__uint_as_float(raw & 0xFFFF0000u), ACT);
+                }
+                const float v0 = acc[mi][32 * x + 4 * i + 2 * h] * g0;
+                const float v1 = acc[mi][32 * x + 4 * i + 2 * h + 1] * g1;
                 asm volatile("st.shared.b32 [%0], %1;" ::"r"(a), "r"(pack_bf16x2(v0, v1)) : "memory");
                 s0 += v0;
                 s1 += v1;
@@ -164,6 +200,10 @@
       bar_wg();
       if (xthread) {
         for (int x = 0; x < nx; ++x) tma_store_2d(&tms.o, xs + x * Cfg::X_TILE, n0 + x * 64, m0);
+        if constexpr (EPI == EPI_FWD && MASK)
+          for (int mi = 0; mi < MI && m0 + 64 * mi < p.M; ++mi)
+            bulk_store_1d(p.mask + act_mask_word(m0 / 64 + mi, n0 / 64, p.N, 0), ms + mi * (BN / 64) * Cfg::M_BLOCK,
+                          static_cast<uint32_t>(nx * Cfg::M_BLOCK));
         tma_store_commit();
       }
       if (do_cols) {
@@ -231,6 +271,9 @@
   return with_pp_shape(pl.bm_wg, pl.bn, [&](auto BM_WG, auto BN) {
     return with_act(p.act, [&](auto ACT) {
       using Cfg = GemmPpCfg<BM_WG, BN>;
+      if constexpr (ACT == SB_ACT_RELU || ACT == SB_ACT_LEAKYRELU)
+        if (p.mask != nullptr)
+          return launch_kernel(gemm_pp_kernel<BM_WG, BN, EPI, ACT, true>, pl.grid, Cfg::THREADS, Cfg::SMEM_BYTES, st, pdl, tms, p);
       return launch_kernel(gemm_pp_kernel<BM_WG, BN, EPI, ACT>, pl.grid, Cfg::THREADS, Cfg::SMEM_BYTES, st, pdl, tms, p);
     });
   });
@@ -244,6 +287,10 @@
           return with_act(act, [&](auto ACT) {
             const int bytes = GemmPpCfg<BM_WG, BN>::SMEM_BYTES;
             SB_TRY(set_max_smem(gemm_pp_kernel<BM_WG, BN, EPI_FWD, ACT>, bytes));
+            if constexpr (ACT == SB_ACT_RELU || ACT == SB_ACT_LEAKYRELU) {
+              SB_TRY(set_max_smem(gemm_pp_kernel<BM_WG, BN, EPI_FWD, ACT, true>, bytes));
+              SB_TRY(set_max_smem(gemm_pp_kernel<BM_WG, BN, EPI_DA, ACT, true>, bytes));
+            }
             return set_max_smem(gemm_pp_kernel<BM_WG, BN, EPI_DA, ACT>, bytes);
           });
         }));
diff --git a/shifu-tensorflow_b200/csrc/gemm_ring.cuh b/shifu-tensorflow_b200/csrc/gemm_ring.cuh
--- a/shifu-tensorflow_b200/csrc/gemm_ring.cuh
+++ b/shifu-tensorflow_b200/csrc/gemm_ring.cuh
@@ -17,6 +17,7 @@
   const __nv_bfloat16* aux;
   int ld_aux;
   float* colsum;
+  uint32_t* mask;
   float* accum;
   int ld_acc;
   int acc_vec4;
diff --git a/shifu-tensorflow_b200/csrc/gemm_wide.cuh b/shifu-tensorflow_b200/csrc/gemm_wide.cuh
--- a/shifu-tensorflow_b200/csrc/gemm_wide.cuh
+++ b/shifu-tensorflow_b200/csrc/gemm_wide.cuh
@@ -9,11 +9,12 @@
 };
 static_assert(GemmWideCfg::STAGES >= 3, "operand ring");
 
-template <int ACT>
+template <int ACT, bool MASK = false>
 __global__ void __launch_bounds__(GemmWideCfg::THREADS, 1)
 gemm_wide_kernel(const __grid_constant__ PpTmaps tms, const GemmTcParams p) {
   using Cfg = GemmWideCfg;
   constexpr int BM = Cfg::BM, BN = Cfg::BN, BK = Cfg::BK;
+  static_assert(!MASK || ACT == SB_ACT_RELU || ACT == SB_ACT_LEAKYRELU, "an act' mask for relu / leaky relu only");
 
   extern __shared__ uint8_t smem_raw[];
   const Ring<Cfg> ring(smem_raw, Cfg::BN * Cfg::BM * 2);
@@ -28,6 +29,10 @@
   const int tiles_n = (p.N + BN - 1) / BN;
   const int n_tiles = tiles_m * tiles_n;
   const int kb_n = (p.K + BK - 1) / BK;
+  auto xaddr = [&](int r, int c) {
+    return xs + static_cast<uint32_t>((c >> 6) * Cfg::X_TILE + r * 128 + ((((c & 63) >> 3) ^ (r & 7)) << 4) + (c & 7) * 2);
+  };
+  constexpr int MASK_BAR_THREADS = 256 + 96;
 
   if (warp >= Cfg::PRODUCER_WARP) {
     asm volatile("setmaxnreg.dec.sync.aligned.u32 %0;" ::"n"(Cfg::PRODUCER_REGS));
@@ -47,6 +52,34 @@
       }
     }
     ring_producer_tail<Cfg>(p);
+    if constexpr (MASK) {
+      if (warp > Cfg::PRODUCER_WARP) {
+        const int ht = static_cast<int>(threadIdx.x) - 32 * (Cfg::PRODUCER_WARP + 1);
+        for (int t = blockIdx.x; t < n_tiles; t += gridDim.x) {
+          const int m0 = (t / tiles_n) * BM, n0 = (t % tiles_n) * BN;
+          const int nx = min(BN / 64, (p.N - n0 + 63) / 64);
+          asm volatile("bar.sync 3, %0;" ::"n"(MASK_BAR_THREADS) : "memory");
+          for (int w = ht; w < 8 * 128; w += 96) {
+            const int half = w >> 9, x = (w >> 7) & 3, tt = w & 127;
+            const int rb = m0 / 64 + half;
+            if (x >= nx || 64 * rb >= p.M) continue;
+            const int r0 = 64 * half + 16 * (tt >> 5) + ((tt & 31) >> 2), c0 = 64 * x + 2 * (tt & 3);
+            uint32_t ma[2] = {0u, 0u};
+#pragma unroll
+            for (int i = 0; i < 8; ++i)
+#pragma unroll
+              for (int h = 0; h < 2; ++h) {
+                uint32_t pk;
+                asm volatile("ld.shared.b32 %0, [%1];" : "=r"(pk) : "r"(xaddr(r0 + 8 * h, c0 + 8 * i)) : "memory");
+                act_mask_collect(ma, pk, 2 * i + h);
+              }
+            const uint32_t keep = (m0 + r0 < p.M ? 0x33333333u : 0u) | (m0 + r0 + 8 < p.M ? 0xCCCCCCCCu : 0u);
+            p.mask[act_mask_word(rb, n0 / 64 + x, p.N, tt)] = act_mask_fold(ma) & keep;
+          }
+          if (t + static_cast<int>(gridDim.x) < n_tiles) asm volatile("bar.arrive 4, %0;" ::"n"(MASK_BAR_THREADS) : "memory");
+        }
+      }
+    }
   } else {
     asm volatile("setmaxnreg.inc.sync.aligned.u32 %0;" ::"n"(Cfg::CONSUMER_REGS));
     const int g = warp >> 2;
@@ -54,9 +87,6 @@
     auto bar_consumers = [&]() { asm volatile("bar.sync 2, 256;" ::: "memory"); };
     const int r0 = 64 * g + (warp & 3) * 16 + (lane >> 2);
     const int c0 = 2 * (lane & 3);
-    auto xaddr = [&](int r, int c) {
-      return xs + static_cast<uint32_t>((c >> 6) * Cfg::X_TILE + r * 128 + ((((c & 63) >> 3) ^ (r & 7)) << 4) + (c & 7) * 2);
-    };
 
     float acc_mi[1][BN / 2];
     float (&acc)[BN / 2] = acc_mi[0];
@@ -72,6 +102,7 @@
 
       asm volatile("st.shared.f32 [%0], %1;" ::"r"(bias_s + ct * 4u), "f"(bv) : "memory");
       if (ct == 0) tma_store_wait_read<0>();
+      if (MASK && !first) asm volatile("bar.sync 4, %0;" ::"n"(MASK_BAR_THREADS) : "memory");
       bar_consumers();
 #pragma unroll
       for (int i = 0; i < BN / 8; ++i) {
@@ -87,6 +118,7 @@
       }
       fence_proxy_async();
       bar_consumers();
+      if (MASK) asm volatile("bar.arrive 3, %0;" ::"n"(MASK_BAR_THREADS) : "memory");
       if (ct == 0) {
         for (int x = 0; x < nx; ++x) tma_store_2d(&tms.o, xs + x * Cfg::X_TILE, n0 + x * 64, m0);
         tma_store_commit();
@@ -102,13 +134,20 @@
   if (pl.bm_wg != GemmWideCfg::BM || pl.bn != GemmWideCfg::BN)
     return set_error(SB_ERR_INVALID, "gemm_wide has 128 x 256 tiles only (bm_wg=%d bn=%d)", pl.bm_wg, pl.bn);
   return with_act(p.act, [&](auto ACT) {
+    if constexpr (ACT == SB_ACT_RELU || ACT == SB_ACT_LEAKYRELU)
+      if (p.mask != nullptr)
+        return launch_kernel(gemm_wide_kernel<ACT, true>, pl.grid, GemmWideCfg::THREADS, GemmWideCfg::SMEM_BYTES, st, pdl, tms, p);
     return launch_kernel(gemm_wide_kernel<ACT>, pl.grid, GemmWideCfg::THREADS, GemmWideCfg::SMEM_BYTES, st, pdl, tms, p);
   });
 }
 
 static int set_gemm_wide_attrs() {
   for (int act = SB_ACT_NONE; act <= SB_ACT_LEAKYRELU; ++act)
-    SB_TRY(with_act(act, [&](auto ACT) { return set_max_smem(gemm_wide_kernel<ACT>, GemmWideCfg::SMEM_BYTES); }));
+    SB_TRY(with_act(act, [&](auto ACT) {
+      if constexpr (ACT == SB_ACT_RELU || ACT == SB_ACT_LEAKYRELU)
+        SB_TRY(set_max_smem(gemm_wide_kernel<ACT, true>, GemmWideCfg::SMEM_BYTES));
+      return set_max_smem(gemm_wide_kernel<ACT>, GemmWideCfg::SMEM_BYTES);
+    }));
   return SB_OK;
 }
 
diff --git a/shifu-tensorflow_b200/csrc/net.cu b/shifu-tensorflow_b200/csrc/net.cu
--- a/shifu-tensorflow_b200/csrc/net.cu
+++ b/shifu-tensorflow_b200/csrc/net.cu
@@ -210,6 +210,13 @@
       A_ps[l] = static_cast<long long>(max_batch) * ly.ld_out;
       SB_TRY(dalloc(&A[l], static_cast<size_t>(A_ps[l]) * nparts));
       if (training) SB_TRY(dalloc(&dZ[l], static_cast<size_t>(A_ps[l]) * nparts));
+    }
+    if (training && nparts == 1) {
+      mask.assign(L > 1 ? L - 1 : 0, nullptr);
+      for (int l = 0; l + 1 < L; ++l)
+        if (act_has_mask(layers[l].act) &&
+            plan_gemm_pp(max_batch, layers[l].out, layers[l + 1].out, num_sms, false).bm_wg == 128)
+          SB_TRY(dalloc(&mask[l], act_mask_words(max_batch, layers[l].out)));
     }
   } else {
     SB_TRY(dalloc(&Xf, static_cast<size_t>(max_batch) * F));
@@ -377,6 +384,7 @@
       if (l == 0) { p.zero_buf = clear; p.zero_n4 = clear_n4; }
       p.trace = next_trace("fwd", l, rows, ly.out, k_in);
       if (nparts == 1 && p.addend == nullptr) {
+        p.mask = mask_of(l, in);
         const PpPlan pp = plan_gemm_pp(rows, ly.out, k_in, num_sms, true);
         PpTmaps pt;
         SB_TRY(make_tmap_bf16(&pt.a, src, src_rows, k_in, ld_k, pp.bm_wg));
@@ -494,7 +502,7 @@
   return SB_OK;
 }
 
-int Net::enqueue_da(int l, int rows, float* grad) {
+int Net::enqueue_da(const StepIn& in, int l, int rows, float* grad) {
   Layer& ly = layers[l];
   Layer& pl = layers[l - 1];
   if (!tc()) {
@@ -525,8 +533,9 @@
     SB_TRY(make_tmap_bf16(&pt.b, ly.Wn, ly.in, ly.out, ly.ld_out, pp.bn));
     SB_TRY(make_tmap_bf16(&pt.o, dZ[l - 1], rows, ly.in, pl.ld_out, pp.bm_wg));
     SB_TRY(make_tmap_bf16(&pt.x, A[l - 1], rows, ly.in, pl.ld_out, pp.bm_wg));
+    p.mask = mask_of(l - 1, in);
     SB_TRY(launch_gemm_pp<EPI_DA>(pp, pt, p, stream, true));
-    mark("gemm_pp<DA>");
+    mark(p.mask ? "gemm_pp<DA,mask>" : "gemm_pp<DA>");
   } else {
     const GemmPlan gp = plan_gemm(rows, ly.in, round_up(ly.out, 64) * pairs_of(nparts), num_sms, false);
     TmapSet tm;
@@ -573,6 +582,31 @@
         const uint32_t u = static_cast<uint32_t>(raw[static_cast<size_t>(k * part_stride) + static_cast<size_t>(r) * ld + c]) << 16;
         memcpy(dst + (static_cast<size_t>(k) * rows + r) * cols + c, &u, 4);
       }
+  return SB_OK;
+}
+
+__global__ void act_mask_kernel(const __nv_bfloat16* A, int ld, int M, int N, uint32_t* mask) {
+  const long long w = static_cast<long long>(blockIdx.x) * blockDim.x + threadIdx.x;
+  if (w >= static_cast<long long>(act_mask_words(M, N))) return;
+  const int t = static_cast<int>(w % 128), blk = static_cast<int>(w / 128);
+  const int rb = blk / act_mask_col_blocks(N), cb = blk % act_mask_col_blocks(N);
+  uint32_t acc[2] = {0u, 0u};
+  for (int i = 0; i < 8; ++i)
+    for (int h = 0; h < 2; ++h) {
+      const int r = 64 * rb + 16 * (t / 32) + (t % 32) / 4 + 8 * h, c = 64 * cb + 8 * i + 2 * (t % 4);
+      if (r >= M || c >= N) continue;
+      uint32_t pk = reinterpret_cast<const uint32_t*>(A + static_cast<size_t>(r) * ld + c)[0];
+      if (c + 1 >= N) pk &= 0xFFFFu;
+      act_mask_collect(acc, pk, 2 * i + h);
+    }
+  const uint32_t word = act_mask_fold(acc);
+  mask[act_mask_word(rb, cb, N, t)] = word;
+}
+
+static int build_act_mask(const __nv_bfloat16* A, int ld, int M, int N, uint32_t* mask, cudaStream_t st) {
+  const long long n = static_cast<long long>(act_mask_words(M, N));
+  act_mask_kernel<<<static_cast<unsigned>((n + 255) / 256), 256, 0, st>>>(A, ld, M, N, mask);
+  SB_CUDA(cudaGetLastError());
   return SB_OK;
 }
 
@@ -715,14 +749,20 @@
   return debug_gemm_impl(A, B, D, M, N, K, split_k, a_mn, b_mn, cfg_cg, cfg_bn, device, iters, ms_out);
 }
 
-int sb_debug_gemm_layer(int32_t kind, int32_t precision, const float* A, const float* W, const float* bias, const float* aux,
-                        const float* addend, float* out, float* colsum, float* grad, int32_t* guard, char* route,
-                        int32_t route_cap, int32_t M, int32_t N, int32_t K, int32_t a_rows, int32_t row0, int32_t act,
-                        int32_t r0, int32_t r1, int32_t sms, int64_t clear_n4, int device) {
+static int debug_gemm_layer_impl(int32_t kind, int32_t precision, const float* A, const float* W, const float* bias,
+                                 const float* aux, const float* addend, float* out, float* colsum, float* grad, int32_t* guard,
+                                 char* route, int32_t route_cap, int32_t M, int32_t N, int32_t K, int32_t a_rows, int32_t row0,
+                                 int32_t act, int32_t r0, int32_t r1, int32_t sms, int64_t clear_n4, int device,
+                                 uint32_t* mask_out, int64_t mask_cap, int32_t aux_path) {
   enum { FWD = 0, DA = 1, DW = 2 };
   SB_CHECK(kind >= FWD && kind <= DW, SB_ERR_INVALID, "kind=%d (0 forward, 1 dA, 2 dW)", kind);
   SB_CHECK(precision >= SB_PREC_FP32 && precision <= SB_PREC_BF16X2, SB_ERR_INVALID, "precision=%d invalid", precision);
   SB_CHECK(act >= SB_ACT_NONE && act <= SB_ACT_LEAKYRELU, SB_ERR_INVALID, "act=%d invalid", act);
+  SB_CHECK(mask_out == nullptr || (kind == FWD && precision == SB_PREC_BF16 && act_has_mask(act) && addend == nullptr),
+           SB_ERR_INVALID, "an act' mask is written by the plain-bf16 forward GEMM of a relu / leaky relu layer only");
+  SB_CHECK(mask_out == nullptr || (M > 0 && N > 0 && mask_cap >= static_cast<int64_t>(act_mask_words(M, N))), SB_ERR_INVALID,
+           "mask_cap=%lld below the mask's words", static_cast<long long>(mask_cap));
+  SB_CHECK(aux_path == 0 || kind == DA, SB_ERR_INVALID, "aux_path belongs to the dA GEMM");
   SB_CHECK(M > 0 && N > 0 && K > 0, SB_ERR_INVALID, "M=%d N=%d K=%d", M, N, K);
   SB_CHECK(A && W && guard && (route == nullptr || route_cap > 0), SB_ERR_INVALID, "null argument");
   SB_CHECK(kind != FWD || (bias && out), SB_ERR_INVALID, "the forward GEMM needs bias and out");
@@ -761,6 +801,7 @@
   const uint16_t S16 = 0x7f7f;
   DevBuf<__nv_bfloat16> res;
   DevBuf<float> g, clr;
+  DevBuf<uint32_t> fwd_mask;
   Net net;
   SB_TRY(net.init(&d, device, true));
   if (sms > 0) net.num_sms = sms;
@@ -794,10 +835,18 @@
   }
   if (addend)
     SB_CUDA(cudaMemcpy2D(net.E, sizeof(float) * l0.ld_out, addend, sizeof(float) * N, sizeof(float) * N, M, cudaMemcpyHostToDevice));
+  if (mask_out) {
+    SB_TRY(alloc_filled(&fwd_mask, act_mask_words(M, N), 0xff));
+    net.mask.assign(1, fwd_mask.p);
+  }
   if (kind == DA) {
     if (tc) {
       SB_TRY(upload_parts(net.dZ[1], A, M, K, net.layers[1].ld_out, np, net.A_ps[1]));
       SB_TRY(upload_parts(net.A[0], aux, M, N, l0.ld_out, np, net.A_ps[0]));
+      if (!net.mask.empty() && net.mask[0]) {
+        if (aux_path) net.mask[0] = nullptr;
+        else SB_TRY(build_act_mask(net.A[0], l0.ld_out, M, N, net.mask[0], 0));
+      }
     } else {
       SB_CUDA(cudaMemcpy(net.dZf[1], A, sizeof(float) * M * K, cudaMemcpyHostToDevice));
       SB_CUDA(cudaMemcpy(net.Af[0], aux, sizeof(float) * M * N, cudaMemcpyHostToDevice));
@@ -840,7 +889,7 @@
   SB_TRY(net.refresh_shadows());
   net.launches = 0;
   if (kind == FWD) SB_TRY(net.enqueue_hidden_forward(in, M, nullptr, nullptr, reinterpret_cast<float4*>(clr.p), clear_n4));
-  else if (kind == DA) SB_TRY(net.enqueue_da(1, M, g.p));
+  else if (kind == DA) SB_TRY(net.enqueue_da(in, 1, M, g.p));
   else SB_TRY(net.enqueue_dw(in, 0, K, g.p, net.stream, false, sms > 0 ? sms : dev_sms, r0, r1));
   SB_CHECK(net.launches == 1 && net.last_kernel != nullptr, SB_ERR_STATE, "%d GEMM launches", net.launches);
   SB_TRY(sync_hook(net.last_kernel));
@@ -886,16 +935,40 @@
     SB_CUDA(cudaMemcpy(h.data(), clr.p, sizeof(uint32_t) * clr_n, cudaMemcpyDeviceToHost));
     for (size_t i = 0; i < clr_n; ++i) changed += i < clr_n - GUARD ? h[i] != 0u : h[i] != S32;
   }
+  if (mask_out) SB_CUDA(cudaMemcpy(mask_out, fwd_mask.p, sizeof(uint32_t) * act_mask_words(M, N), cudaMemcpyDeviceToHost));
   *guard = changed;
   return SB_OK;
 }
 
-int sb_debug_gemm_epilogue(const float* A, const float* W, const float* bias, const float* aux, float* out, float* colsum,
-                           int32_t M, int32_t N, int32_t K, int32_t da, int32_t act, int32_t bm_wg, int device,
-                           int32_t iters, float* ms_out) {
+int sb_debug_gemm_layer(int32_t kind, int32_t precision, const float* A, const float* W, const float* bias, const float* aux,
+                        const float* addend, float* out, float* colsum, float* grad, int32_t* guard, char* route,
+                        int32_t route_cap, int32_t M, int32_t N, int32_t K, int32_t a_rows, int32_t row0, int32_t act,
+                        int32_t r0, int32_t r1, int32_t sms, int64_t clear_n4, int device) {
+  return debug_gemm_layer_impl(kind, precision, A, W, bias, aux, addend, out, colsum, grad, guard, route, route_cap, M, N, K,
+                               a_rows, row0, act, r0, r1, sms, clear_n4, device, nullptr, 0, 0);
+}
+
+int sb_debug_gemm_layer_mask(int32_t kind, int32_t precision, const float* A, const float* W, const float* bias,
+                             const float* aux, const float* addend, float* out, float* colsum, float* grad, int32_t* guard,
+                             char* route, int32_t route_cap, int32_t M, int32_t N, int32_t K, int32_t a_rows, int32_t row0,
+                             int32_t act, int32_t r0, int32_t r1, int32_t sms, int64_t clear_n4, int device,
+                             uint32_t* mask_out, int64_t mask_cap, int32_t aux_path) {
+  return debug_gemm_layer_impl(kind, precision, A, W, bias, aux, addend, out, colsum, grad, guard, route, route_cap, M, N, K,
+                               a_rows, row0, act, r0, r1, sms, clear_n4, device, mask_out, mask_cap, aux_path);
+}
+
+static int debug_gemm_epilogue_impl(const float* A, const float* W, const float* bias, const float* aux, float* out,
+                                    float* colsum, int32_t M, int32_t N, int32_t K, int32_t da, int32_t act, int32_t bm_wg,
+                                    int device, int32_t iters, float* ms_out, uint32_t* mask_out, int64_t mask_cap,
+                                    int32_t aux_path) {
   SB_CHECK(A && W && out && M > 0 && N > 0 && K > 0 && (da == 0 || da == 1), SB_ERR_INVALID, "bad argument");
   SB_CHECK(da ? aux != nullptr : bias != nullptr, SB_ERR_INVALID, "the forward GEMM needs a bias, the dA GEMM an aux matrix");
   SB_CHECK(act >= SB_ACT_NONE && act <= SB_ACT_LEAKYRELU, SB_ERR_INVALID, "act invalid");
+  SB_CHECK(mask_out == nullptr || (!da && act_has_mask(act)), SB_ERR_INVALID,
+           "an act' mask is written by the forward GEMM of a relu / leaky relu layer only");
+  SB_CHECK(mask_out == nullptr || mask_cap >= static_cast<int64_t>(act_mask_words(M, N)), SB_ERR_INVALID,
+           "mask_cap=%lld below the mask's words", static_cast<long long>(mask_cap));
+  SB_CHECK(aux_path == 0 || da, SB_ERR_INVALID, "aux_path belongs to the dA GEMM");
   SB_CHECK(bm_wg == 0 || bm_wg == 64 || bm_wg == 128 || bm_wg == PP_TILE_WIDE, SB_ERR_INVALID,
            "bm_wg must be 0, 64, 128 or %d (got %d)", PP_TILE_WIDE, bm_wg);
   SB_CHECK(!(da && bm_wg == PP_TILE_WIDE), SB_ERR_INVALID, "the %d-wide tile is for the forward GEMM only", PP_TILE_WIDE);
@@ -922,6 +995,12 @@
   GemmTcParams p = {};
   p.M = M; p.N = N; p.K = K;
   p.act = act; p.bias = d_bias.p; p.colsum = colsum ? d_col.p : nullptr;
+  DevBuf<uint32_t> d_mask;
+  if (mask_out || (da && act_has_mask(act) && !aux_path)) {
+    SB_TRY(alloc_filled(&d_mask, act_mask_words(M, N), 0xff));
+    if (da) SB_TRY(build_act_mask(d_aux.p, ldn, M, N, d_mask.p, 0));
+    p.mask = d_mask.p;
+  }
   auto launch = [&]() {
     if (da) return launch_gemm_pp<EPI_DA>(pp, pt, p, 0, false);
     return pp.bn == 256 ? launch_gemm_wide(pp, pt, p, 0, false) : launch_gemm_pp<EPI_FWD>(pp, pt, p, 0, false);
@@ -933,11 +1012,26 @@
   std::vector<uint16_t> h;
   SB_TRY(download_bf16(out, d_out.p, M, N, 1, static_cast<long long>(M) * ldn, h));
   if (colsum) SB_CUDA(cudaMemcpy(colsum, d_col.p, sizeof(float) * N, cudaMemcpyDeviceToHost));
+  if (mask_out) SB_CUDA(cudaMemcpy(mask_out, d_mask.p, sizeof(uint32_t) * act_mask_words(M, N), cudaMemcpyDeviceToHost));
   if (iters > 0) {
     SB_TRY(time_launches(launch, 3, iters, ms_out));
     SB_TRY(sync_hook(kernel));
   }
   return SB_OK;
+}
+
+int sb_debug_gemm_epilogue(const float* A, const float* W, const float* bias, const float* aux, float* out, float* colsum,
+                           int32_t M, int32_t N, int32_t K, int32_t da, int32_t act, int32_t bm_wg, int device,
+                           int32_t iters, float* ms_out) {
+  return debug_gemm_epilogue_impl(A, W, bias, aux, out, colsum, M, N, K, da, act, bm_wg, device, iters, ms_out, nullptr, 0, 0);
+}
+
+int sb_debug_gemm_epilogue_mask(const float* A, const float* W, const float* bias, const float* aux, float* out,
+                                float* colsum, int32_t M, int32_t N, int32_t K, int32_t da, int32_t act, int32_t bm_wg,
+                                int device, int32_t iters, float* ms_out, uint32_t* mask_out, int64_t mask_cap,
+                                int32_t aux_path) {
+  return debug_gemm_epilogue_impl(A, W, bias, aux, out, colsum, M, N, K, da, act, bm_wg, device, iters, ms_out, mask_out,
+                                  mask_cap, aux_path);
 }
 
 int sb_debug_gemm_fwd_out(const float* A, const float* W, const float* bias, const float* wo, float bo, const float* y,
diff --git a/shifu-tensorflow_b200/csrc/net.cuh b/shifu-tensorflow_b200/csrc/net.cuh
--- a/shifu-tensorflow_b200/csrc/net.cuh
+++ b/shifu-tensorflow_b200/csrc/net.cuh
@@ -49,6 +49,10 @@
   float *s1 = nullptr, *s2 = nullptr;
   __nv_bfloat16* Xb = nullptr;
   std::vector<__nv_bfloat16*> A, dZ;
+  std::vector<uint32_t*> mask;
+  uint32_t* mask_of(int l, const StepIn& in) const {
+    return (l < static_cast<int>(mask.size()) && !(l == 0 && in.sparse)) ? mask[l] : nullptr;
+  }
   float* Xf = nullptr;
   std::vector<float*> Af, dZf;
   float *yhat = nullptr, *ones = nullptr;
@@ -106,7 +110,7 @@
   int enqueue_out(const StepIn& in, int rows, bool do_loss, bool do_bwd, float* yhat_dst, float* grad);
   int enqueue_dw(const StepIn& in, int l, int rows, float* grad, cudaStream_t st, bool pdl, int sms, int r0 = 0, int r1 = -1,
                  int chunk = -1);
-  int enqueue_da(int l, int rows, float* grad);
+  int enqueue_da(const StepIn& in, int l, int rows, float* grad);
 };
 
 int validate_desc(const sb_net_desc* d);
diff --git a/shifu-tensorflow_b200/csrc/ptx.cuh b/shifu-tensorflow_b200/csrc/ptx.cuh
--- a/shifu-tensorflow_b200/csrc/ptx.cuh
+++ b/shifu-tensorflow_b200/csrc/ptx.cuh
@@ -57,6 +57,14 @@
       "cp.async.bulk.tensor.2d.shared::cluster.global.mbarrier::complete_tx::bytes [%0], [%1, {%3, %4}], [%2];"
       ::"r"(dst_smem), "l"(tmap), "r"(bar), "r"(c0), "r"(c1)
       : "memory");
+}
+__device__ __forceinline__ void bulk_load_1d(uint32_t dst_smem, const void* src, uint32_t bytes, uint32_t bar) {
+  asm volatile("cp.async.bulk.shared::cluster.global.mbarrier::complete_tx::bytes [%0], [%1], %2, [%3];"
+               ::"r"(dst_smem), "l"(src), "r"(bytes), "r"(bar)
+               : "memory");
+}
+__device__ __forceinline__ void bulk_store_1d(void* dst, uint32_t src_smem, uint32_t bytes) {
+  asm volatile("cp.async.bulk.global.shared::cta.bulk_group [%0], [%1], %2;" ::"l"(dst), "r"(src_smem), "r"(bytes) : "memory");
 }
 __device__ __forceinline__ void tma_store_2d(const void* tmap, uint32_t src_smem, int c0, int c1) {
   asm volatile("cp.async.bulk.tensor.2d.global.shared::cta.bulk_group [%0, {%2, %3}], [%1];"
```

Result: faster. 37.80 million (median of 6 runs) (+1.1%).
